# VinAIResearch/LFM

Hardware: AMD Instinct MI355X
Metric: images/sec (higher is better)
Workload: dtype f16; 1 GPU; DiT-L/2 celeb256 f8 (4x32x32 latents), batch 64/GPU, 50-step Euler (torchdiffeq grid) + f8 VAE decode to 256x256 + uint8 NHWC; 2 batches in flight on 2 HIP streams (same weights, own scratch); per_gpu_batch=64, global_batch=64, h2d_of_latents=inside the timed step, nfe=50, batches_in_flight=2

## Files before the change

### include/lfm_hip.h

```cpp
#ifndef LFM_HIP_H
#define LFM_HIP_H
#include <stddef.h>
#include <stdint.h>

#ifdef __cplusplus
extern "C" {
#endif

typedef void* lfm_stream_t;

#define LFM_OK 0
#define LFM_ERR_SHAPE (-1)
#define LFM_ERR_ALIGN (-2)
#define LFM_ERR_WORKSPACE (-3)
#define LFM_ERR_LAUNCH (-4)
#define LFM_ERR_ARG (-5)

const char* lfm_strerror(int code);
#define LFM_ABI_VERSION 4
int lfm_abi_version(void);

typedef struct lfm_dit_shape {
  int depth;
  int hidden;
  int heads;
  int patch;
  int in_ch;
  int res;
  int mlp_hidden;
  int label_rows;
} lfm_dit_shape;

typedef struct lfm_dit_weights {
  const float* pos_embed;
  const float* patch_w;
  const float* patch_b;
  const float* t_w0;
  const float* t_b0;
  const float* t_w2;
  const float* t_b2;
  const float* y_table;
  const void* ada_w;
  const float* ada_b;
  const void* qkv_w;
  const float* qkv_b;
  const void* proj_w;
  const float* proj_b;
  const void* fc1_w;
  const float* fc1_b;
  const void* fc2_w;
  const float* fc2_b;
  const float* final_w;
  const float* final_b;
  const void* patch_w16;
} lfm_dit_weights;

typedef struct lfm_dit_call {
  int batch;
  const float* x;
  const float* t;
  int t_len;
  const int64_t* y;
  int cfg;
  float cfg_scale;
  float* out;
  const float* axpy_base;
  const float* axpy_dt;
  const void* cond_table;
  const int* cond_step;
  int cond_offset;
  int cond_rows;
  int fold_ln;
  int gemm_select;
} lfm_dit_call;
#define LFM_CALL_OFF 1
#define LFM_CALL_ON 2
#define LFM_CALL_GEMM_SELECT(which) ((which) + 1)

size_t lfm_dit_workspace_bytes(const lfm_dit_shape* shape, int max_batch);

#define LFM_DIT_WS_BUFFERS 10
int lfm_dit_workspace_layout(const lfm_dit_shape* shape, int batch, size_t* offsets_out, int n);

int lfm_dit_forward(const lfm_dit_shape* shape, const lfm_dit_weights* w, void* workspace, size_t workspace_bytes,
                    const lfm_dit_call* call, lfm_stream_t stream);

#define LFM_PLAN_FOLDED_LN 1
#define LFM_PLAN_FUSED_QKV_ATTENTION 2
int lfm_dit_plan(const lfm_dit_shape* shape, const lfm_dit_call* call, int* plan_out);

size_t lfm_dit_cond_table_bytes(const lfm_dit_shape* shape, int n_times);
int lfm_dit_cond_table_build(const lfm_dit_shape* shape, const lfm_dit_weights* w, void* workspace, size_t workspace_bytes, int batch, const float* t_values,
                             int n_times, void* table, size_t table_bytes, lfm_stream_t stream);

int lfm_gemm_f16(const void* A, long lda, const void* W, long ldw, void* C, long ldc, int M, int N, int K, const float* bias,
                 int epilogue, const float* gate, long gate_stride, int tokens, lfm_stream_t stream);

int lfm_gemm_qkv_f16(const void* A, long lda, const void* W, long ldw, void* Q, void* K_out, void* Vt, int M, int D, int K,
                     const float* bias, int head_dim, int tokens, lfm_stream_t stream);

int lfm_gemm_select(int which);
int lfm_gemm_plan(int M, int N, int K, int batch, int caps);

int lfm_profile_fc1(int enable);
int lfm_profile_blocks_read(float* host_ms_out, int max_n);
#define LFM_OPT_FOLD_LN 1
#define LFM_OPT_GEMM_V6 2
#define LFM_OPT_SKINNY_GEMM 4
#define LFM_OPT_ATTENTION_STREAM 5
#define LFM_OPT_FUSED_QKV_ATTENTION 6
#define LFM_OPT_UNET_ATTENTION_STREAM 7
#define LFM_OPT_ATTENTION_TILED 8
int lfm_set_option(int key, int value);
int lfm_dit_call_settings(const lfm_dit_call* call, int* gemm_select_out, int* fold_ln_out);

int lfm_clock_probe(int blocks, int iters, unsigned long long* ticks_out, lfm_stream_t stream);

#ifdef LFM_MEASURE
int lfm_gemm_trace_read(unsigned long long* host_out, int n_per_group);
int lfm_attention_trace_read(unsigned long long* host_out, int n);
int lfm_attention_wg_trace_read(unsigned long long* host_out, int n_wg);
int lfm_dit_chk_arm(const void* workspace);
int lfm_dit_chk_read(unsigned long long* host_out, int n);
#endif
int lfm_profile_fc1_read(float* host_ms_out, int max_n);

int lfm_ln_modulate(const float* X, void* A, int M, int D, int tokens, const float* shift, const float* scale, long mod_stride,
                    lfm_stream_t stream);

int lfm_dit_attention(const void* Q, const void* K, const void* Vt, void* O, int batch, int heads, int T, lfm_stream_t stream);
int lfm_dit_attention_hd(const void* Q, const void* K, const void* Vt, void* O, int batch, int heads, int head_dim, int T,
                         lfm_stream_t stream);
int lfm_attention_plan(int batch, int heads, int head_dim, int T);

typedef struct lfm_vae_resnet {
  const float* n1_g; const float* n1_b; const void* c1_w; const float* c1_b;
  const float* n2_g; const float* n2_b; const void* c2_w; const float* c2_b;
  const void* sc_w; const float* sc_b;
  int cin, cout;
} lfm_vae_resnet;

typedef struct lfm_vae_weights {
  const float* pq_w; const float* pq_b;
  const float* cin_w; const float* cin_b;
  lfm_vae_resnet mid[2];
  const float* at_g; const float* at_b;
  const void* q_w; const float* q_b; const void* k_w; const float* k_b;
  const void* v_w; const float* v_b; const void* o_w; const float* o_b;
  lfm_vae_resnet up[4][3];
  const void* ups_w[3]; const float* ups_b[3];
  const float* no_g; const float* no_b;
  const void* cout_w; const float* cout_b;
} lfm_vae_weights;

size_t lfm_vae_workspace_bytes(int R, int chunk);

int lfm_vae_decode(const lfm_vae_weights* w, void* workspace, size_t workspace_bytes, const float* z, float* out, int N, int R,
                   int chunk, lfm_stream_t stream);

typedef struct lfm_vae_enc_weights {
  const float* cin_w; const float* cin_b;
  lfm_vae_resnet down[4][2];
  const void* ds_w[3]; const float* ds_b[3];
  lfm_vae_resnet mid[2];
  const float* at_g; const float* at_b;
  const void* q_w; const float* q_b; const void* k_w; const float* k_b;
  const void* v_w; const float* v_b; const void* o_w; const float* o_b;
  const float* no_g; const float* no_b;
  const void* cout_w; const float* cout_b;
} lfm_vae_enc_weights;

int lfm_vae_encode(const lfm_vae_enc_weights* w, void* workspace, size_t workspace_bytes, const float* x, float* moments, int N, int R,
                   int chunk, lfm_stream_t stream);

int lfm_vae_groupnorm_f16(const void* x, void* y, const float* gamma, const float* beta, void* workspace, size_t workspace_bytes, int n, int HW, int C,
                          int silu, lfm_stream_t stream);
int lfm_vae_groupnorm_plan(int n, int HW, int C, size_t workspace_bytes);
int lfm_vae_conv3x3_gn_f16(const void* in, const void* w, const float* bias, const void* resid, void* conv_out, void* y, const float* gamma,
                           const float* beta, void* workspace, size_t workspace_bytes, int n, int H, int W, int Cin, int Cout, int ups, int silu,
                           int* stat_slabs, int* stat_kernel, lfm_stream_t stream);
size_t lfm_vae_mid_attention_workspace_bytes(int n, int T);
int lfm_vae_mid_attention_f16(const void* x, void* out, const float* gn_gamma, const float* gn_beta, const void* q_w, const float* q_b,
                              const void* k_w, const float* k_b, const void* v_w, const float* v_b, const void* o_w, const float* o_b,
                              void* workspace, size_t workspace_bytes, int n, int T, lfm_stream_t stream);
int lfm_vae_conv_in_f16(const float* pq_w, const float* pq_b, const float* cin_w, const float* cin_b, const float* z, void* out, int n, int R,
                        lfm_stream_t stream);
size_t lfm_vae_downsample_workspace_bytes(int n, int Ho, int Wo, int C);
int lfm_vae_downsample_f16(const void* x, const void* w, const float* bias, void* out, void* workspace, size_t workspace_bytes, int n, int Ho, int Wo,
                           int C, lfm_stream_t stream);
size_t lfm_vae_resnets_workspace_bytes(int n, int H, int W);
int lfm_vae_resnets_f16(const lfm_vae_resnet* r, int n_res, const void* x, void* out, void* workspace, size_t workspace_bytes, int n, int H, int W,
                        int chain_stats, int* last_slabs, lfm_stream_t stream);
size_t lfm_vae_conv_moments_workspace_bytes(int n, int H, int W);
int lfm_vae_conv_moments_f32(const void* in, const void* w8, const float* b8, float* moments, void* workspace, size_t workspace_bytes, int n, int H,
                             int W, lfm_stream_t stream);

int lfm_images_to_uint8(const float* x, uint8_t* out, int N, int H, int W, lfm_stream_t stream);
int lfm_images_to_uint8_mode(const float* x, uint8_t* out, int N, int H, int W, int rounding, lfm_stream_t stream);

int lfm_conv3x3_f16(const void* in, const void* w, const float* bias, const void* resid, void* out, int N, int H, int W, int Cin, int Cout,
                    int mode, lfm_stream_t stream);
size_t lfm_conv3x3_workspace_bytes(int N, int H, int W, int Cin, int Cout);
int lfm_conv3x3_f16_ws(const void* in, const void* w, const float* bias, const void* resid, void* out, int N, int H, int W, int Cin, int Cout,
                       int mode, void* workspace, size_t workspace_bytes, lfm_stream_t stream);
int lfm_conv3x3_scaled_f16_ws(const void* in, const void* w, const float* bias, const void* resid, float scale, void* out, int N, int H, int W, int Cin,
                              int Cout, int mode, void* workspace, size_t workspace_bytes, lfm_stream_t stream);
int lfm_conv3x3_plan(int N, int H, int W, int Cin, int Cout, int mode, size_t workspace_bytes);
int lfm_conv3x3_in_f32(const float* x_nchw, const float* w, const float* bias, void* out_nhwc, int N, int H, int W, int Cin, int Cout,
                       lfm_stream_t stream);
int lfm_conv3x3_out_f32(const void* in, const void* w4, const float* bias4, float* out_nchw, int N, int H, int W, int Cin, int nch,
                        lfm_stream_t stream);
int lfm_linear_f16(const void* A, long lda, const void* W, long ldw, void* C, long ldc, int M, int N, int K, const float* bias,
                   const void* resid, lfm_stream_t stream);
int lfm_linear2_f16(const void* A1, int K1, const void* A2, int K2, const void* W, long ldw, void* C, long ldc, int M, int N, const float* bias,
                    const void* resid, lfm_stream_t stream);
int lfm_linear_scaled_f16(const void* A, long lda, const void* W, long ldw, void* C, long ldc, int M, int N, int K, const float* bias,
                          const void* resid, float scale, lfm_stream_t stream);
int lfm_linear2_scaled_f16(const void* A1, int K1, const void* A2, int K2, const void* W, long ldw, void* C, long ldc, int M, int N,
                           const float* bias, const void* resid, float scale, lfm_stream_t stream);
int lfm_linear_resid_vec_f16(const void* A, long lda, const void* W, long ldw, void* C, long ldc, int M, int N, int K, const float* bias,
                             const void* resid, const float* vec, long vec_stride, int tokens, float scale, lfm_stream_t stream);
int lfm_linear_silu_f16(const void* A, long lda, const void* W, long ldw, void* C, long ldc, int M, int N, int K, const float* bias, lfm_stream_t stream);
int lfm_gather_rows_f32(const float* table, int rows, int cols, const void* y_int64, int N, float* out, long out_stride, lfm_stream_t stream);
size_t lfm_groupnorm_scratch_bytes(int N, int C);
int lfm_groupnorm_f16(const void* x, void* y, const float* gamma, const float* beta, const float* film, long film_stride, void* scratch, int N,
                      int HW, int C, int groups, float eps, int silu, lfm_stream_t stream);
int lfm_groupnorm_plan(int N, int HW, int C, int groups);
int lfm_groupnorm2_f16(const void* xa, int Ca, const void* xb, int Cb, void* y, const float* gamma, const float* beta, const float* film,
                       long film_stride, void* scratch, int N, int HW, int groups, float eps, int silu, lfm_stream_t stream);
int lfm_avgpool2_f16(const void* x, void* y, int N, int Ho, int Wo, int C, lfm_stream_t stream);
int lfm_upsample2_f16(const void* x, void* y, int N, int Ho, int Wo, int C, lfm_stream_t stream);
int lfm_fir_down2_f16(const void* x, void* y, const float* bias, const void* resid, float scale, int N, int Ho, int Wo, int C, int pad,
                      lfm_stream_t stream);
int lfm_fir_up2_f16(const void* x, void* y, int N, int Ho, int Wo, int C, lfm_stream_t stream);
int lfm_zero_border_f16(const void* x, void* y, int N, int H, int W, int C, lfm_stream_t stream);
int lfm_zero_border_f32(const float* x, float* y, int planes, int H, int W, lfm_stream_t stream);
int lfm_concat_channels_f16(const void* a, const void* b, void* out, long pixels, int Ca, int Cb, lfm_stream_t stream);
int lfm_add_image_vec_f16(const void* x, const float* e, long e_stride, void* y, int N, int HW, int C, lfm_stream_t stream);
int lfm_attention_small_f16(const void* qkv, void* out, int N, int T, int heads, int ch, lfm_stream_t stream);
int lfm_unet_attention_plan(int N, int T, int heads, int ch);
int lfm_cross_attention_f16(const void* Q, long ldq, const void* K, const void* V, long ldkv, void* out, long ldo, int N, int Tq, int Tk, int heads,
                            int ch, lfm_stream_t stream);
int lfm_cross_attention_plan(int N, int Tq, int Tk, int heads, int ch);
int lfm_layernorm_f16(const void* x, void* y, const float* gamma, const float* beta, long M, int C, float eps, lfm_stream_t stream);
int lfm_geglu_f16(const void* h, long ldh, void* y, long M, int I, lfm_stream_t stream);
int lfm_token_embed_f16(const float* tok_emb, int vocab, const float* pos_emb, int pos_rows, const void* ids_int64, void* out, int N, int L, int D,
                        lfm_stream_t stream);
int lfm_linear_gelu_f16(const void* A, long lda, const void* W, long ldw, void* C, long ldc, int M, int N, int K, const float* bias, lfm_stream_t stream);
int lfm_label_rescale_f32(const void* labels_int64, const float* w, const float* bias, float* out, int N, int H, int W, int num_cls, int Cout, int n_stages,
                          lfm_stream_t stream);
int lfm_time_embed(const float* t, int t_len, const float* w0, const float* b0, const float* w2, const float* b2, const float* label_table,
                   const int64_t* y, int label_rows, float* scratch_h1, float* emb, void* emb_silu_f16, int N, int F, int E,
                   lfm_stream_t stream);
int lfm_song_embed(const float* t, int t_len, const float* w0, const float* b0, const float* w1, const float* b1, const float* label_table,
                   const float* label_bias, float label_scale, const int64_t* y, int label_rows, float* scratch_h1, float* emb, void* emb_f16, int N,
                   int F, int E, lfm_stream_t stream);
int lfm_fourier_embed(const float* t, int t_len, const float* freqs, const float* w0, const float* b0, const float* w1, const float* b1,
                      const float* label_table, const float* label_bias, float label_scale, const int64_t* y, int label_rows, float* scratch_h1,
                      float* emb, void* emb_f16, int N, int F, int E, lfm_stream_t stream);

int lfm_grid_advance(const float* ts, const float* dts, int* step, float* t_cur, float* t_next, float* dt_cur, lfm_stream_t stream);

int lfm_lincomb(float* out, const float* base, const float* const* k_host_ptrs, const float* coef, const float* scale, int nk, long n,
                lfm_stream_t stream);

int lfm_rk_error_norm(const float* y0, const float* y1, const float* const* k_host_ptrs, const float* e_coef, const float* dt, int nk, long n,
                      float rtol, float atol, float* scratch, float* out, lfm_stream_t stream);

#ifdef __cplusplus
}
#endif
#endif
```

### lfm_amd/csrc/dit.hip

```cpp
#include <mutex>

#include "../../include/lfm_hip.h"
#include "gemm_dispatch.h"
#include "gemm_skinny_kernel.h"
#include "gemm_sq64_kernel.h"
#include "qkv_attention_kernel.h"

typedef std::atomic<int> Opt;
static inline int opt_get(const Opt& o) { return o.load(std::memory_order_relaxed); }
static inline void opt_set(Opt& o, int v) { o.store(v, std::memory_order_relaxed); }
static struct {
  Opt gemm_sel{0}, gemm_dbg{0};
  Opt fold_ln{1};
  Opt v6{0};
  Opt skinny{1};
  Opt stagger{0};
  Opt att_stream{1};
  Opt fused_qkv{1};
  Opt att_tiled{1};
  Opt unet_att_stream{1};
} g_def;
static thread_local int tl_sel_set = 0, tl_gemm_sel = 0, tl_gemm_dbg = 0;
static thread_local int tl_fold = 0;
static inline int gemm_sel() { return tl_sel_set ? tl_gemm_sel : opt_get(g_def.gemm_sel); }
static inline int gemm_dbg() { return tl_sel_set ? tl_gemm_dbg : opt_get(g_def.gemm_dbg); }
static inline int opt_fold_ln() { return tl_fold ? (tl_fold == LFM_CALL_ON ? 1 : 0) : opt_get(g_def.fold_ln); }
int lfm_gemm_selected() { return gemm_sel(); }
int lfm_gemm_debug_flags() { return gemm_dbg(); }
int lfm_gemm_selected_v1_ok() { return gemm_sel() < 2 && !(gemm_dbg() & LFM_DBG_GEMM_NO_SPLITK); }
int lfm_gemm_prefers_v4(int M, int N, int K) {
  (void)M;
  (void)N;
  (void)K;
  if (gemm_dbg() & LFM_DBG_GEMM_NEVER_V4) return 0;
  if (gemm_dbg() & LFM_DBG_GEMM_ALWAYS_V4) return 1;
  return 0;
}
int lfm_gemm_v6_default() { return opt_get(g_def.v6); }
int lfm_stagger_ticks() { return opt_get(g_def.stagger); }
int lfm_attention_stream_enabled() { return opt_get(g_def.att_stream); }
int lfm_attention_tiled_mode() { return opt_get(g_def.att_tiled); }
int lfm_unet_attention_stream_mode() { return opt_get(g_def.unet_att_stream); }
extern "C" int lfm_gemm_plan(int M, int N, int K, int batch, int caps) { return gemm_choose(M, N, K, batch, caps); }
static inline bool gemm_select_valid(int which) {
  const int k = which & 15;
  return which >= 0 && (k == 0 || k == 1 || k == 4 || k == 5 || k == 6 || k == 7 || k == 8);
}
struct CallScope {
  int sel_set, sel, dbg, fold;
  CallScope() : sel_set(tl_sel_set), sel(tl_gemm_sel), dbg(tl_gemm_dbg), fold(tl_fold) {}
  ~CallScope() {
    tl_sel_set = sel_set;
    tl_gemm_sel = sel;
    tl_gemm_dbg = dbg;
    tl_fold = fold;
  }
};

static int call_scope_enter(const lfm_dit_call* c) {
  if (c->fold_ln < 0 || c->fold_ln > LFM_CALL_ON || c->gemm_select < 0 || (c->gemm_select && !gemm_select_valid(c->gemm_select - 1)) || c->cond_rows < 0)
    return LFM_ERR_ARG;
  if (c->fold_ln) tl_fold = c->fold_ln;
  if (c->gemm_select) {
    tl_sel_set = 1;
    tl_gemm_sel = (c->gemm_select - 1) & 15;
    tl_gemm_dbg = (c->gemm_select - 1) >> 4;
  }
  return LFM_OK;
}
extern "C" int lfm_dit_call_settings(const lfm_dit_call* call, int* gemm_select_out, int* fold_ln_out) {
  if (!call || !gemm_select_out || !fold_ln_out) return LFM_ERR_ARG;
  CallScope scope;
  const int rc = call_scope_enter(call);
  if (rc) return rc;
  *gemm_select_out = gemm_sel() | (gemm_dbg() << 4);
  *fold_ln_out = opt_fold_ln();
  return LFM_OK;
}

extern "C" int lfm_set_option(int key, int value) {
  switch (key) {
    case 1: opt_set(g_def.fold_ln, value != 0); break;
    case 2: opt_set(g_def.v6, value != 0); break;
#ifdef LFM_MEASURE
    case 3: opt_set(g_def.stagger, value > 0 ? value : 0); break;
#endif
    case 4: opt_set(g_def.skinny, value < 0 || value > 2 ? 1 : value); break;
    case 5: opt_set(g_def.att_stream, value != 0); break;
    case 6: opt_set(g_def.fused_qkv, value != 0); break;
    case 7: opt_set(g_def.unet_att_stream, value < 0 || value > 2 ? 1 : value); break;
    case 8:
      if (value < 0 || value > 2) return LFM_ERR_ARG;
      opt_set(g_def.att_tiled, value);
      break;
    default: return LFM_ERR_ARG;
  }
  return LFM_OK;
}
extern "C" int lfm_gemm_select(int which) {
  if (!gemm_select_valid(which)) return LFM_ERR_ARG;
  opt_set(g_def.gemm_sel, which & 15);
  opt_set(g_def.gemm_dbg, which >> 4);
  return LFM_OK;
}

#include "dit_kernels.h"
#include "attention_dispatch.h"
#include "solver_kernels.h"
#include "dit_measure.h"

static inline size_t align_up(size_t v, size_t a) { return (v + a - 1) / a * a; }

struct DitWs {
  float* X;
  half_t* A;
  half_t* A2;
  half_t* QKVH;
  float* temb;
  float* temb_h;
  half_t* c_half;
  float* mod;
  float* ones;
  float* ln_part;
  float* cen[2];
  half_t* amod;
  float* uvq;
  float* uvf;
  float* slab;
  size_t slab_bytes;
  size_t total;
};

struct DitDims {
  int B, T, M, D, H;
  long J, uvq_n, uvf_n;
  int KK, tiles_p, hd;
};
static inline bool dit_fold_capable(const lfm_dit_shape* s) { return (s->hidden % 256) == 0 && (s->mlp_hidden % 64) == 0; }
static DitDims dit_dims(const lfm_dit_shape* s, int B) {
  const int grid = s->res / s->patch, T = grid * grid, D = s->hidden, H = s->mlp_hidden;
  const long uv = dit_fold_capable(s) ? (long)s->depth * 2 : 0;
  return DitDims{B, T, B * T, D, H, (long)s->depth * 6 * D + 2 * D, uv * 3 * D, uv * H, s->in_ch * s->patch * s->patch, D / 256, D / s->heads};
}

static DitWs carve(const lfm_dit_shape* s, const DitDims& d, void* ws, bool sizing = false) {
  const size_t B = d.B, T = d.T, M = d.M, D = d.D, H = d.H, J = d.J;
  size_t off = 0;
  char* base = (char*)ws;
  DitWs w;
  auto take = [&](size_t bytes) {
    char* p = (char*)((uintptr_t)base + off);
    off += align_up(bytes, 256);
    return p;
  };
  w.X = (float*)take(M * D * 4);
  w.A = (half_t*)take(M * D * 2);
  const size_t qkvh = (3 * M * D > M * H ? 3 * M * D : M * H) * 2;
  w.QKVH = (half_t*)take(qkvh);
  w.temb = (float*)take(B * D * 4);
  w.temb_h = (float*)take(B * D * 4);
  w.c_half = (half_t*)take(B * D * 2);
  w.mod = (float*)take(B * J * 4);
  w.ones = (float*)take(D * 4);
  w.ln_part = (float*)take(M * ((D + 255) / 256) * 8);
  w.cen[0] = (float*)take(M * 4);
  w.cen[1] = (float*)take(M * 4);
  const bool fold_ops = dit_fold_capable(s);
  w.amod = (half_t*)take(fold_ops ? (size_t)s->depth * 4 * B * D * 2 : 0);
  w.uvq = (float*)take(fold_ops ? (size_t)s->depth * 2 * B * 3 * D * 4 : 0);
  w.uvf = (float*)take(fold_ops ? (size_t)s->depth * 2 * B * H * 4 : 0);
  w.A2 = (half_t*)take(fold_ops ? M * D * 2 : 0);
  const size_t Ms = sizing ? (M < 1024 ? M : (size_t)1024 / T * T) : M;
  w.slab_bytes = (sizing || M <= 1024) && Ms > 0 ? 4 * Ms * (H > 3 * D ? H : 3 * D) * 4 : 0;
  w.slab = w.slab_bytes ? (float*)take(w.slab_bytes) : nullptr;
  if (!base) w.slab = nullptr;
  w.total = off;
  return w;
}

static int check_shape(const lfm_dit_shape* s) {
  if (!s) return LFM_ERR_ARG;
  if (s->depth <= 0 || s->hidden <= 0 || s->heads <= 0 || s->patch <= 0 || s->in_ch <= 0 || s->res <= 0) return LFM_ERR_SHAPE;
  if (s->hidden % s->heads) return LFM_ERR_SHAPE;
  if (s->res % s->patch) return LFM_ERR_SHAPE;
  const int T = (s->res / s->patch) * (s->res / s->patch);
  if (attention_choose(1, s->heads, s->hidden / s->heads, T) < 0) return LFM_ERR_SHAPE;
  if (s->hidden % 64 || s->hidden > 256 * LN_MAXV || s->mlp_hidden % 64) return LFM_ERR_SHAPE;
  const int kk = s->patch * s->patch * s->in_ch;
  if (kk > FIN_MAXO || (kk > PE_MAXK && (kk % 64))) return LFM_ERR_SHAPE;
  if (s->label_rows <= 0) return LFM_ERR_SHAPE;
  return LFM_OK;
}

extern "C" const char* lfm_strerror(int code) {
  switch (code) {
    case LFM_OK: return "ok";
    case LFM_ERR_SHAPE: return "unsupported or inconsistent shape";
    case LFM_ERR_ALIGN: return "pointer / leading dimension alignment";
    case LFM_ERR_WORKSPACE: return "workspace too small";
    case LFM_ERR_LAUNCH: return "kernel launch failed";
    case LFM_ERR_ARG: return "bad argument";
  }
  return "unknown";
}
extern "C" int lfm_abi_version(void) { return LFM_ABI_VERSION; }

extern "C" size_t lfm_dit_workspace_bytes(const lfm_dit_shape* shape, int max_batch) {
  if (check_shape(shape) != LFM_OK || max_batch <= 0) return 0;
  return carve(shape, dit_dims(shape, max_batch), nullptr, true).total;
}

extern "C" int lfm_dit_workspace_layout(const lfm_dit_shape* shape, int batch, size_t* offsets_out, int n) {
  const int rc = check_shape(shape);
  if (rc) return rc;
  if (!offsets_out || n < 0) return LFM_ERR_ARG;
  if (batch <= 0) return LFM_ERR_SHAPE;
  const DitWs w = carve(shape, dit_dims(shape, batch), nullptr);
  const bool fold_ops = dit_fold_capable(shape);
  const void* bufs[LFM_DIT_WS_BUFFERS] = {w.X, w.A, fold_ops ? w.A2 : nullptr, w.QKVH, w.mod, w.ln_part, w.cen[0], w.cen[1], fold_ops ? w.uvq : nullptr,
                                          fold_ops ? w.uvf : nullptr};
  for (int i = 0; i < n && i < LFM_DIT_WS_BUFFERS; ++i) offsets_out[i] = (size_t)(uintptr_t)bufs[i];
  return LFM_DIT_WS_BUFFERS;
}

extern "C" int lfm_dit_attention_hd(const void* Q, const void* K, const void* Vt, void* O, int batch, int heads, int head_dim, int T,
                                    lfm_stream_t stream) {
  if (!Q || !K || !Vt || !O) return LFM_ERR_ARG;
  if (batch <= 0 || heads <= 0) return LFM_ERR_SHAPE;
  if (((uintptr_t)Q | (uintptr_t)K | (uintptr_t)Vt | (uintptr_t)O) & 15) return LFM_ERR_ALIGN;
  return attention_launch((const half_t*)Q, (const half_t*)K, (const half_t*)Vt, (half_t*)O, batch, heads, head_dim, T, (hipStream_t)stream);
}
extern "C" int lfm_attention_plan(int batch, int heads, int head_dim, int T) {
  if (batch <= 0 || heads <= 0) return LFM_ERR_SHAPE;
  return attention_choose(batch, heads, head_dim, T);
}
extern "C" int lfm_dit_attention(const void* Q, const void* K, const void* Vt, void* O, int batch, int heads, int T, lfm_stream_t stream) {
  return lfm_dit_attention_hd(Q, K, Vt, O, batch, heads, 64, T, stream);
}

static int ln_modulate_launch(const float* X, half_t* A, int M, int D, int tokens, const float* shift, const float* scale, long stride,
                              hipStream_t st) {
  if (D % 4 || D > 256 * LN_MAXV) return LFM_ERR_SHAPE;
  if (D % 8 == 0 && !(((uintptr_t)A | (uintptr_t)X) & 15) && !(gemm_dbg() & LFM_DBG_LN_STORE8)) {
    const int f = gemm_dbg();
    if (f & LFM_DBG_LN_BPERMUTE) hipLaunchKernelGGL(ln_modulate8_kernel<1>, dim3(cdiv(M, 4)), dim3(256), 0, st, X, A, M, D, tokens, shift, scale, stride);
    else if (f & LFM_DBG_LN_TWO_ROWS) hipLaunchKernelGGL(ln_modulate8_kernel<2>, dim3(cdiv(M, 8)), dim3(256), 0, st, X, A, M, D, tokens, shift, scale, stride);
    else if (f & LFM_DBG_LN_FOUR_ROWS) hipLaunchKernelGGL(ln_modulate8_kernel<4>, dim3(cdiv(M, 16)), dim3(256), 0, st, X, A, M, D, tokens, shift, scale, stride);
    else hipLaunchKernelGGL((ln_modulate8_kernel<1, true>), dim3(cdiv(M, 4)), dim3(256), 0, st, X, A, M, D, tokens, shift, scale, stride);
    LFM_CHECK_LAUNCH();
    return LFM_OK;
  }
  hipLaunchKernelGGL(ln_modulate_kernel, dim3(cdiv(M, 4 * LN_ROWS)), dim3(256), 0, st, X, A, M, D, tokens, shift, scale, stride);
  LFM_CHECK_LAUNCH();
  return LFM_OK;
}

extern "C" int lfm_ln_modulate(const float* X, void* A, int M, int D, int tokens, const float* shift, const float* scale, long mod_stride,
                               lfm_stream_t stream) {
  if (!X || !A || !shift || !scale) return LFM_ERR_ARG;
  if (M <= 0 || tokens <= 0) return LFM_ERR_SHAPE;
  return ln_modulate_launch(X, (half_t*)A, M, D, tokens, shift, scale, mod_stride, (hipStream_t)stream);
}

extern "C" int lfm_gemm_f16(const void* A, long lda, const void* W, long ldw, void* C, long ldc, int M, int N, int K, const float* bias,
                            int epilogue, const float* gate, long gate_stride, int tokens, lfm_stream_t stream) {
  if (!A || !W || !C) return LFM_ERR_ARG;
  if ((lda % 8) || (ldw % 8) || (ldc % 4) || (((uintptr_t)A | (uintptr_t)W) & 15)) return LFM_ERR_ALIGN;
  hipStream_t st = (hipStream_t)stream;
  ASrcRowMajor a{(const half_t*)A, lda, M, 0};
  if (gemm_sel() == 7 || gemm_sel() == 8) {
    const int which = gemm_sel();
    auto lat = [&](const auto& e) {
      return which == 7 ? launch_gemm_sq64((const half_t*)A, lda, (const half_t*)W, ldw, M, N, K, e, 1, st)
                        : launch_gemm_skinny((const half_t*)A, lda, (const half_t*)W, ldw, M, N, K, e, 1, st);
    };
    switch (epilogue) {
      case 0: return lat(EpiBiasF16{(half_t*)C, ldc, bias});
      case 1: return bias ? lat(EpiBiasGeluF16{(half_t*)C, ldc, bias}) : LFM_ERR_ARG;
      case 2: return lat(EpiBiasF32{(float*)C, ldc, bias});
      default: return LFM_ERR_ARG;
    }
  }
  switch (epilogue) {
    case 0: return gemm_f16_launch(a, (const half_t*)W, ldw, M, N, K, EpiBiasF16{(half_t*)C, ldc, bias}, st);
    case 1: return bias ? gemm_f16_launch(a, (const half_t*)W, ldw, M, N, K, EpiBiasGeluF16{(half_t*)C, ldc, bias}, st) : LFM_ERR_ARG;
    case 2: return launch_gemm_auto(a, (const half_t*)W, ldw, M, N, K, EpiBiasF32{(float*)C, ldc, bias}, st);
    case 3:
      if (!bias || !gate || tokens <= 0) return LFM_ERR_ARG;
      return gemm_f16_launch(a, (const half_t*)W, ldw, M, N, K, EpiGateResidF32{(float*)C, ldc, bias, gate, gate_stride, tokens}, st);
  }
  return LFM_ERR_ARG;
}

extern "C" int lfm_gemm_qkv_f16(const void* A, long lda, const void* W, long ldw, void* Q, void* Kout, void* Vt, int M, int D, int K,
                                const float* bias, int head_dim, int tokens, lfm_stream_t stream) {
  if (!A || !W || !Q || !Kout || !Vt || !bias) return LFM_ERR_ARG;
  if ((lda % 8) || (ldw % 8) || (((uintptr_t)A | (uintptr_t)W) & 15)) return LFM_ERR_ALIGN;
  if (head_dim <= 0 || tokens <= 0 || (D % head_dim) || (head_dim % 8) || (tokens % 16) || (M % tokens)) return LFM_ERR_SHAPE;
  return gemm_f16_launch(ASrcRowMajor{(const half_t*)A, lda, M, 0}, (const half_t*)W, ldw, M, 3 * D, K,
                         EpiQKV::make((half_t*)Q, (half_t*)Kout, (half_t*)Vt, bias, D, head_dim, tokens), (hipStream_t)stream);
}

static int dit_conditioning(const lfm_dit_shape* s, const lfm_dit_weights* w, const DitWs& ws, const DitDims& d, const float* t, int t_len, const int64_t* y,
                            int rows, bool want_uv, hipStream_t st) {
  const int D = d.D, H = d.H;
  const long J = d.J, mstride = rows == 1 ? 0 : J;
  hipLaunchKernelGGL(temb1_kernel, dim3(cdiv(D, 4), t_len), dim3(256), 0, st, t, w->t_w0, w->t_b0, ws.temb_h, D);
  LFM_CHECK_LAUNCH();
  hipLaunchKernelGGL(temb2_kernel, dim3(cdiv(D, 4), t_len), dim3(256), 0, st, ws.temb_h, w->t_w2, w->t_b2, ws.temb, D);
  LFM_CHECK_LAUNCH();
  hipLaunchKernelGGL(cond_kernel, dim3(cdiv((long)rows * D, 256)), dim3(256), 0, st, ws.temb, t_len, w->y_table, y, s->label_rows, ws.c_half, D, rows);
  LFM_CHECK_LAUNCH();
  int rc = launch_gemm_tn(ASrcRowMajor{ws.c_half, D, rows, 0}, (const half_t*)w->ada_w, D, rows, (int)J, D, EpiBiasF32{ws.mod, J, w->ada_b}, st);
  if (rc || !want_uv) return rc;
  if (rows == 1 && D <= 8 * 64 * LN_MAXP) {
    hipLaunchKernelGGL(uv_gemv_kernel, dim3(cdiv(3 * D, 4 * UV_ROWS), s->depth), dim3(256), 0, st, (const half_t*)w->qkv_w, w->qkv_b, ws.mod, 3 * D, D, D, 0,
                       ws.uvq);
    LFM_CHECK_LAUNCH();
    hipLaunchKernelGGL(uv_gemv_kernel, dim3(cdiv(H, 4 * UV_ROWS), s->depth), dim3(256), 0, st, (const half_t*)w->fc1_w, w->fc1_b, ws.mod, H, D, 4 * D, 3 * D,
                       ws.uvf);
    LFM_CHECK_LAUNCH();
    return LFM_OK;
  }
  const long nmod = (long)s->depth * 4 * rows * (D / 4);
  hipLaunchKernelGGL(mod_rows_f16_kernel, dim3(cdiv(nmod, 256)), dim3(256), 0, st, ws.mod, mstride, s->depth, rows, D, ws.amod);
  LFM_CHECK_LAUNCH();
  rc = launch_gemm_auto(ASrcRowMajor{ws.amod, D, 2 * rows, 0}, (const half_t*)w->qkv_w, D, 2 * rows, 3 * D, D, EpiUV{ws.uvq, 3L * D, w->qkv_b, rows, 3L * D}, st,
                        s->depth, 4L * rows * D, 3L * D * D, 2L * rows * 3 * D);
  if (rc) return rc;
  return launch_gemm_auto(ASrcRowMajor{ws.amod + 2L * rows * D, D, 2 * rows, 0}, (const half_t*)w->fc1_w, D, 2 * rows, H, D,
                          EpiUV{ws.uvf, (long)H, w->fc1_b, rows, (long)H}, st, s->depth, 4L * rows * D, (long)H * D, 2L * rows * H);
}

static inline long cond_row_floats(const DitDims& d) { return d.J + d.uvq_n + d.uvf_n; }
static int dit_cond_copy(const DitWs& ws, const DitDims& d, const float* table, const int* step, int offset, int fixed_row, int to_table, hipStream_t st,
                         int rows = 0) {
  hipLaunchKernelGGL(cond_row_copy_kernel, dim3(cdiv(cond_row_floats(d) / 4, 256)), dim3(256), 0, st, table, cond_row_floats(d), step, offset, fixed_row, ws.mod,
                     d.J, ws.uvq, d.uvq_n, ws.uvf, d.uvf_n, to_table, rows);
  LFM_CHECK_LAUNCH();
  return LFM_OK;
}

extern "C" size_t lfm_dit_cond_table_bytes(const lfm_dit_shape* shape, int n_times) {
  if (check_shape(shape) != LFM_OK || n_times <= 0) return 0;
  return (size_t)cond_row_floats(dit_dims(shape, 1)) * 4 * (size_t)n_times;
}

extern "C" int lfm_dit_cond_table_build(const lfm_dit_shape* s, const lfm_dit_weights* w, void* workspace, size_t workspace_bytes, int batch,
                                        const float* t_values, int n_times, void* table, size_t table_bytes, lfm_stream_t stream) {
  int rc = check_shape(s);
  if (rc) return rc;
  if (!w || !workspace || !t_values || !table || n_times <= 0 || batch <= 0) return LFM_ERR_ARG;
  if (table_bytes < lfm_dit_cond_table_bytes(s, n_times)) return LFM_ERR_WORKSPACE;
  const DitDims d = dit_dims(s, batch);
  const DitWs ws = carve(s, d, workspace);
  if (ws.total > workspace_bytes) return LFM_ERR_WORKSPACE;
  if (((uintptr_t)workspace & 255) || ((uintptr_t)table & 15)) return LFM_ERR_ALIGN;
  hipStream_t st = (hipStream_t)stream;
  for (int i = 0; i < n_times; ++i) {
    rc = dit_conditioning(s, w, ws, d, t_values + i, 1, nullptr, 1, dit_fold_capable(s), st);
    if (rc) return rc;
    rc = dit_cond_copy(ws, d, (const float*)table, nullptr, 0, i, 1, st, n_times);
    if (rc) return rc;
  }
  return LFM_OK;
}

enum DitLoop { DIT_LOOP_FOLDED, DIT_LOOP_LATENCY, DIT_LOOP_SEPARATE };
struct DitPlan {
  DitLoop loop;
  bool fold, w6, fused;
  bool pe_mfma, fin_mfma;
  bool sq64;
  int s_proj, s_fc2;
};
static DitPlan dit_plan(const lfm_dit_shape* s, const DitDims& d, int rows, const DitWs* ws = nullptr, const lfm_dit_weights* w = nullptr) {
  const int sel = gemm_sel(), dbg = gemm_dbg(), skinny = opt_get(g_def.skinny);
  const int D = d.D, H = d.H, T = d.T, M = d.M;
  DitPlan p{};
  p.fold = opt_fold_ln() && dit_fold_capable(s) && (M % 256 == 0) && (rows == 1 || T % 256 == 0) && (long)(M / 256) * d.tiles_p >= 192 && (sel == 0 || sel == 6) &&
           s->depth >= 1;
  p.w6 = sel == 6 || (sel == 0 && opt_get(g_def.v6));
  p.fused = p.fold && opt_get(g_def.fused_qkv) && !p.w6 && T == 256 && D == s->heads * 64 && (long)M * D < (1L << 31) && (long)3 * D * D < (1L << 31);
  p.pe_mfma = s->patch == 2 && s->in_ch == 4 && (D % 256 == 0) && D <= 1280 && (s->res % 2 == 0) && !(dbg & LFM_DBG_DIT_PATCH_ROUND1);
  p.fin_mfma = (d.KK == 16 || d.KK == 64) && (D % 32 == 0) && (T % 16 == 0) && (M % 16 == 0) && !(dbg & LFM_DBG_DIT_FINAL_ROUND1);
  p.loop = p.fold ? DIT_LOOP_FOLDED : DIT_LOOP_SEPARATE;
  if (p.fold || !ws) return p;
  auto slices = [&](bool sq, int N_, int K_) {
    const int wgs = sq ? (N_ / SQ_T) * (M / SQ_T) : N_ / SK_BN, bk = sq ? SQ_BK : SK_BK;
    int sl = 1;
    while (wgs * (sl * 2) <= 256 && (K_ % (sl * 2 * bk)) == 0 && K_ / (sl * 2) >= 2 * bk && (size_t)(sl * 2) * M * N_ * 4 <= ws->slab_bytes) sl *= 2;
    return sl;
  };
  p.sq64 = skinny == 1 && M >= SQ_T && (M % SQ_T) == 0 && gemm_sq64_ok(ws->A, D, w->qkv_w, D, M, 3 * D, D, 1) && gemm_sq64_ok(ws->A, D, w->fc1_w, D, M, H, D, 1) &&
           gemm_sq64_ok(ws->A, D, w->proj_w, D, M, D, D, slices(true, D, D)) && gemm_sq64_ok(ws->QKVH, H, w->fc2_w, H, M, D, H, slices(true, D, H));
  p.s_proj = slices(p.sq64, D, D);
  p.s_fc2 = slices(p.sq64, D, H);
  if (skinny && sel == 0 && M <= SK_ROWS && ws->slab && D <= 1024 * SPLITK_LN_MAXJ && (D % 4) == 0 && gemm_skinny_ok(ws->A, D, w->qkv_w, D, M, 3 * D, D, 1) &&
      gemm_skinny_ok(ws->A, D, w->fc1_w, D, M, H, D, 1) && gemm_skinny_ok(ws->A, D, w->proj_w, D, M, D, D, p.s_proj) &&
      gemm_skinny_ok(ws->QKVH, H, w->fc2_w, H, M, D, H, p.s_fc2))
    p.loop = DIT_LOOP_LATENCY;
  return p;
}
extern "C" int lfm_dit_plan(const lfm_dit_shape* s, const lfm_dit_call* c, int* plan_out) {
  int rc = check_shape(s);
  if (rc) return rc;
  if (!c || !plan_out) return LFM_ERR_ARG;
  const int B = c->batch;
  if (B <= 0 || (c->t_len != 1 && c->t_len != B)) return LFM_ERR_SHAPE;
  CallScope scope;
  if ((rc = call_scope_enter(c)) != LFM_OK) return rc;
  const DitPlan p = dit_plan(s, dit_dims(s, B), (c->t_len == 1 && !c->y) ? 1 : B);
  *plan_out = (p.fold ? LFM_PLAN_FOLDED_LN : 0) | (p.fused ? LFM_PLAN_FUSED_QKV_ATTENTION : 0);
  return LFM_OK;
}

struct BlockW {
  const half_t *qkv_w, *proj_w, *fc1_w, *fc2_w;
  const float *qkv_b, *proj_b, *fc1_b, *fc2_b;
  const float *shift_msa, *scale_msa, *gate_msa, *shift_mlp, *scale_mlp, *gate_mlp, *next_shift_msa, *next_scale_msa;
};
static BlockW block_weights(const lfm_dit_weights* w, const float* mod_rows, const DitDims& d, int i) {
  const size_t D = d.D, H = d.H, b = i;
  const float* mod = mod_rows + b * 6 * D;
  return BlockW{(const half_t*)w->qkv_w + b * 3 * D * D, (const half_t*)w->proj_w + b * D * D, (const half_t*)w->fc1_w + b * H * D, (const half_t*)w->fc2_w + b * D * H,
                w->qkv_b + b * 3 * D, w->proj_b + b * D, w->fc1_b + b * H, w->fc2_b + b * D,
                mod, mod + D, mod + 2 * D, mod + 3 * D, mod + 4 * D, mod + 5 * D, mod + 6 * D, mod + 7 * D};
}

struct DitCtx : DitDims {
  const lfm_dit_shape* s;
  const lfm_dit_weights* w;
  const lfm_dit_call* c;
  const void* workspace;
  DitWs ws;
  DitPlan p;
  int rows;
  long mstride;
  hipStream_t st;
  half_t *Qb, *Kb, *Vb;
  bool prof_ok, chk;
  BlockW block(int i) const { return block_weights(w, ws.mod, *this, i); }
  void checksum(const void* buf, size_t bytes, int i, int slot) const { if (chk) dit_chk(buf, bytes, i, slot, st); }
  int embed() const, blocks_folded() const, blocks_latency() const, blocks_separate() const, final_layer() const;
};

int DitCtx::embed() const {
  const int xmod = c->cfg ? B / 2 : B;
  if (p.pe_mfma) {
    const int tpb = M <= 1024 ? 1 : 2;
    hipLaunchKernelGGL(patch_embed_ln_kernel, dim3(cdiv(M, 16 * tpb)), dim3(64 * (D / 256)), 0, st, c->x, w->patch_w, w->patch_b, w->pos_embed, ws.X,
                       M, xmod, s->res, D, tpb, p.fold ? ws.A : (half_t*)nullptr, ws.mod + D, mstride, ws.ln_part, tiles_p, ws.cen[0]);
    LFM_CHECK_LAUNCH();
  } else if (KK <= PE_MAXK) {
    hipLaunchKernelGGL(patch_embed_kernel, dim3(cdiv(M, PE_TOK)), dim3(D / 4), 0, st, c->x, w->patch_w, w->patch_b, w->pos_embed, ws.X, M,
                       xmod, s->in_ch, s->res, s->patch, D);
    LFM_CHECK_LAUNCH();
  } else {
    if (!w->patch_w16) return LFM_ERR_ARG;
    hipLaunchKernelGGL(patchify_kernel, dim3(M), dim3(256), 0, st, c->x, w->pos_embed, ws.A, ws.X, ws.ones, M, xmod, s->in_ch, s->res,
                       s->patch, D);
    LFM_CHECK_LAUNCH();
    const int rc = launch_gemm_auto(ASrcRowMajor{ws.A, KK, M, 0}, (const half_t*)w->patch_w16, KK, M, D, KK,
                                    EpiGateResidF32{ws.X, D, w->patch_b, ws.ones, 0, T}, st);
    if (rc) return rc;
  }
  if (p.fold && !p.pe_mfma) {
    hipLaunchKernelGGL(ln_center_mod_kernel, dim3(cdiv(M, 4)), dim3(256), 0, st, ws.X, ws.A, M, D, T, ws.mod + D, mstride, ws.ln_part, tiles_p,
                       ws.cen[0]);
    LFM_CHECK_LAUNCH();
  }
  return LFM_OK;
}

int DitCtx::blocks_folded() const {
  const long uvs_q = rows == 1 ? 0 : 3 * D, uvs_f = rows == 1 ? 0 : H;
  int rc, cen_cur = 0;
  auto rowstat_src = [&]() {
    RowStatSrc r{ws.ln_part, ws.cen[cen_cur], ws.cen[cen_cur ^ 1], tiles_p, 1.0f / (float)D, 1e-6f};
    cen_cur ^= 1;
    return r;
  };
  auto launch_fold = [&](const ASrcRowMajor& a, const half_t* Wp, long ldw_, int M_, int N_, int K_, const auto& e) {
    return p.w6 ? launch_gemm256w_tn(a, Wp, ldw_, M_, N_, K_, e, st) : launch_gemm256h_tn(a, Wp, ldw_, M_, N_, K_, e, st);
  };
  half_t *Ob = p.fused ? ws.A2 : ws.A, *A1b = p.fused ? ws.A : ws.A2;
  for (int i = 0; i < s->depth; ++i) {
    const BlockW b = block(i);
    const float *uq = ws.uvq + (long)i * 2 * rows * 3 * D, *uf = ws.uvf + (long)i * 2 * rows * H;
    if (p.fused) {
      const QkvAttnArgs e_qa{uq, uq + (long)rows * 3 * D, uvs_q, rowstat_src(), Ob, D, s->heads, 0.125f * 1.4426950408889634f, nullptr, 0};
      if ((rc = launch_qkv_attention(ws.A, D, b.qkv_w, D, M, D, s->heads, D, e_qa, st))) return rc;
    } else {
      const EpiQKVMod e_qkv{{}, Qb, Kb, Vb, uq, uq + (long)rows * 3 * D, uvs_q, D, hd, T, EpiQKV::log2_or_neg(T), rowstat_src(), nullptr, 0};
      if ((rc = launch_fold(ASrcRowMajor{ws.A, D, M, 0}, b.qkv_w, D, M, 3 * D, D, e_qkv))) return rc;
      checksum(ws.QKVH, (size_t)3 * M * D * 2, i, 0);
      if ((rc = attention_launch(Qb, Kb, Vb, Ob, B, s->heads, hd, T, st))) return rc;
    }
    checksum(Ob, (size_t)M * D * 2, i, 1);
    const EpiGateResidMod e_proj{ws.X, D, b.proj_b, b.gate_msa, mstride, T, A1b, b.scale_mlp, mstride, ws.cen[cen_cur], ws.ln_part, tiles_p};
    if ((rc = launch_fold(ASrcRowMajor{Ob, D, M, 0}, b.proj_w, D, M, D, D, e_proj))) return rc;
    checksum(ws.X, (size_t)M * D * 4, i, 2);
    checksum(A1b, (size_t)M * D * 2, i, 3);
    checksum(ws.ln_part, (size_t)M * tiles_p * 8, i, 4);
    const bool prof = prof_fc1_begin(prof_ok, st);
#if defined(LFM_MEASURE) && defined(LFM_EXP_DUMP)
    const EpiModGeluF16 e_fc1{ws.QKVH, H, uf, uf + (long)rows * H, uvs_f, T, rowstat_src(), nullptr, 0,
                              (g_dbg && workspace == g_dbg_ws) ? g_dbg + (long)i * g_dbg_stride : (float*)nullptr};
#else
    const EpiModGeluF16 e_fc1{ws.QKVH, H, uf, uf + (long)rows * H, uvs_f, T, rowstat_src(), nullptr, 0};
#endif
    if ((rc = launch_fold(ASrcRowMajor{A1b, D, M, 0}, b.fc1_w, D, M, H, D, e_fc1))) return rc;
    prof_fc1_end(prof, st);
    checksum(ws.QKVH, (size_t)M * H * 2, i, 5);
    const ASrcRowMajor a_fc2{ws.QKVH, H, M, 0};
    const EpiGateResidF32 e_fc2{ws.X, D, b.fc2_b, b.gate_mlp, mstride, T};
    const EpiGateResidMod e_fc2_mod{e_fc2.X, D, e_fc2.bias, e_fc2.gate, mstride, T, ws.A, b.next_scale_msa, mstride, ws.cen[cen_cur], ws.ln_part, tiles_p};
    if ((rc = i + 1 < s->depth ? launch_fold(a_fc2, b.fc2_w, H, M, D, H, e_fc2_mod) : launch_fold(a_fc2, b.fc2_w, H, M, D, H, e_fc2))) return rc;
    checksum(ws.X, (size_t)M * D * 4, i, 6);
    checksum(ws.A, (size_t)M * D * 2, i, 7);
  }
  return LFM_OK;
}

int DitCtx::blocks_latency() const {
  auto lat_gemm = [&](const half_t* A_, const half_t* W_, int N_, int K_, const auto& epi_, int S_) {
    return p.sq64 ? launch_gemm_sq64(A_, (long)K_, W_, (long)K_, M, N_, K_, epi_, S_, st) : launch_gemm_skinny(A_, (long)K_, W_, (long)K_, M, N_, K_, epi_, S_, st);
  };
  auto finish = [&](int S_, const EpiGateResidF32& e, half_t* A_out, const float* shift, const float* scale) {
    hipLaunchKernelGGL(splitk_finish_resid_ln_kernel, dim3(M), dim3(256), 0, st, ws.slab, S_, (long)M * D, D, e.X, e.ldx, e.bias, e.gate, e.gate_stride, e.tokens, A_out,
                       shift, scale, mstride);
    LFM_CHECK_LAUNCH();
    return LFM_OK;
  };
  const EpiSlabF32 e_slab{ws.slab, (long)D, (long)M * D};
  int rc = ln_modulate_launch(ws.X, ws.A, M, D, T, block(0).shift_msa, block(0).scale_msa, mstride, st);
  if (rc) return rc;
  for (int i = 0; i < s->depth; ++i) {
    const BlockW b = block(i);
    if ((rc = lat_gemm(ws.A, b.qkv_w, 3 * D, D, EpiQKV::make(Qb, Kb, Vb, b.qkv_b, D, hd, T), 1))) return rc;
    if ((rc = attention_launch(Qb, Kb, Vb, ws.A, B, s->heads, hd, T, st))) return rc;
    if ((rc = lat_gemm(ws.A, b.proj_w, D, D, e_slab, p.s_proj))) return rc;
    if ((rc = finish(p.s_proj, EpiGateResidF32{ws.X, D, b.proj_b, b.gate_msa, mstride, T}, ws.A, b.shift_mlp, b.scale_mlp))) return rc;
    const bool prof = prof_fc1_begin(prof_ok, st);
    if ((rc = lat_gemm(ws.A, b.fc1_w, H, D, EpiBiasGeluF16{ws.QKVH, H, b.fc1_b}, 1))) return rc;
    prof_fc1_end(prof, st);
    if ((rc = lat_gemm(ws.QKVH, b.fc2_w, D, H, e_slab, p.s_fc2))) return rc;
    if ((rc = finish(p.s_fc2, EpiGateResidF32{ws.X, D, b.fc2_b, b.gate_mlp, mstride, T}, i + 1 < s->depth ? ws.A : nullptr, b.next_shift_msa, b.next_scale_msa))) return rc;
  }
  return LFM_OK;
}

int DitCtx::blocks_separate() const {
  auto linear = [&](const half_t* W_, int N_, const auto& epi_) {
    const int rc = launch_gemm_splitk(ws.A, D, W_, D, M, N_, D, epi_, ws.slab, ws.slab_bytes, st);
    return rc == 1 ? launch_gemm_auto(ASrcRowMajor{ws.A, D, M, 0}, W_, D, M, N_, D, epi_, st) : rc;
  };
  int rc;
  bool a_ready = false;
  for (int i = 0; i < s->depth; ++i) {
    const BlockW b = block(i);
    if (!a_ready && (rc = ln_modulate_launch(ws.X, ws.A, M, D, T, b.shift_msa, b.scale_msa, mstride, st))) return rc;
    a_ready = false;
    if ((rc = linear(b.qkv_w, 3 * D, EpiQKV::make(Qb, Kb, Vb, b.qkv_b, D, hd, T)))) return rc;
    if ((rc = attention_launch(Qb, Kb, Vb, ws.A, B, s->heads, hd, T, st))) return rc;
    const EpiGateResidF32 e_proj{ws.X, D, b.proj_b, b.gate_msa, mstride, T};
    rc = launch_gemm_splitk_resid_ln(ws.A, D, b.proj_w, D, M, D, D, e_proj, ws.A, b.shift_mlp, b.scale_mlp, mstride, ws.slab, ws.slab_bytes, st);
    if (rc == 1) {
      if ((rc = launch_gemm_auto(ASrcRowMajor{ws.A, D, M, 0}, b.proj_w, D, M, D, D, e_proj, st))) return rc;
      rc = ln_modulate_launch(ws.X, ws.A, M, D, T, b.shift_mlp, b.scale_mlp, mstride, st);
    }
    if (rc) return rc;
    const bool prof = prof_fc1_begin(prof_ok, st);
    if ((rc = linear(b.fc1_w, H, EpiBiasGeluF16{ws.QKVH, H, b.fc1_b}))) return rc;
    prof_fc1_end(prof, st);
    const EpiGateResidF32 e_fc2{ws.X, D, b.fc2_b, b.gate_mlp, mstride, T};
    const bool more = i + 1 < s->depth;
    rc = launch_gemm_splitk_resid_ln(ws.QKVH, H, b.fc2_w, H, M, D, H, e_fc2, more ? ws.A : (half_t*)nullptr, b.next_shift_msa, b.next_scale_msa, mstride, ws.slab,
                                     ws.slab_bytes, st);
    if (rc == LFM_OK) a_ready = more;
    if (rc == 1) rc = launch_gemm_auto(ASrcRowMajor{ws.QKVH, H, M, 0}, b.fc2_w, H, M, D, H, e_fc2, st);
    if (rc) return rc;
  }
  return LFM_OK;
}

int DitCtx::final_layer() const {
  const bool cfg = c->cfg != 0;
  const float* fmod = ws.mod + (long)s->depth * 6 * D;
  const int Mh = cfg ? M / 2 : M;
  auto kernel = p.fin_mfma ? (cfg ? (KK == 16 ? final_layer_mfma_kernel<true, 1> : final_layer_mfma_kernel<true, 4>)
                                  : (KK == 16 ? final_layer_mfma_kernel<false, 1> : final_layer_mfma_kernel<false, 4>))
                           : (cfg ? final_layer_kernel<true> : final_layer_kernel<false>);
  const long blocks = p.fin_mfma ? (cfg ? Mh / 8 : M / 16) : cdiv(Mh, cfg ? 8 : 16);
  hipLaunchKernelGGL(kernel, dim3((unsigned)blocks), dim3(256), 0, st, ws.X, M, D, T, fmod, fmod + D, mstride, w->final_w, w->final_b, s->in_ch, s->res, s->patch,
                     cfg ? c->cfg_scale : 1.0f, c->out, c->axpy_base, c->axpy_dt);
  LFM_CHECK_LAUNCH();
  return LFM_OK;
}

extern "C" int lfm_dit_forward(const lfm_dit_shape* s, const lfm_dit_weights* w, void* workspace, size_t workspace_bytes,
                               const lfm_dit_call* c, lfm_stream_t stream) {
  int rc = check_shape(s);
  if (rc) return rc;
  if (!w || !workspace || !c || !c->x || !c->t || !c->out) return LFM_ERR_ARG;
  const int B = c->batch;
  if (B <= 0 || (c->t_len != 1 && c->t_len != B)) return LFM_ERR_SHAPE;
  if (c->cfg && (B & 1)) return LFM_ERR_SHAPE;
  if (c->axpy_base && !c->axpy_dt) return LFM_ERR_ARG;
  const DitDims d = dit_dims(s, B);
  const DitWs ws = carve(s, d, workspace);
  if (ws.total > workspace_bytes) return LFM_ERR_WORKSPACE;
  if ((uintptr_t)workspace & 255) return LFM_ERR_ALIGN;
  hipStream_t st = (hipStream_t)stream;
  CallScope scope;
  if ((rc = call_scope_enter(c)) != LFM_OK) return rc;
  const bool prof_ok = prof_claim(st);
  const int rows = (c->t_len == 1 && !c->y) ? 1 : B;
  const bool tab = c->cond_table != nullptr;
  if (tab && (rows != 1 || !c->cond_step)) return LFM_ERR_ARG;
  DitCtx x{d, s, w, c, workspace, ws, dit_plan(s, d, rows, &ws, w), rows,  rows == 1 ? 0 : d.J, st,
            ws.QKVH, ws.QKVH + (size_t)d.M * d.D, ws.QKVH + (size_t)2 * d.M * d.D, prof_ok,  false};

  if (tab) rc = dit_cond_copy(ws, d, (const float*)c->cond_table, c->cond_step, c->cond_offset, 0, 0, st, c->cond_rows);
  else rc = dit_conditioning(s, w, ws, d, c->t, c->t_len, c->y, rows, x.p.fold, st);
  if (rc) return rc;
  if ((rc = x.embed()) != LFM_OK) return rc;
#ifdef LFM_MEASURE
  x.chk = g_chk && workspace == g_chk_ws;
  if (x.chk) (void)hipMemsetAsync(g_chk, 0, DIT_CHK_SLOTS * 8, st);
#endif
  const bool prof_blk = prof_ok && g_prof_blk_count < LFM_PROF_BLK_MAX;
  if (prof_blk) (void)hipEventRecord(g_prof_blk_ev[2 * g_prof_blk_count], st);
  switch (x.p.loop) {
    case DIT_LOOP_FOLDED: rc = x.blocks_folded(); break;
    case DIT_LOOP_LATENCY: rc = x.blocks_latency(); break;
    case DIT_LOOP_SEPARATE: rc = x.blocks_separate(); break;
  }
  if (rc) return rc;
  if (prof_blk) (void)hipEventRecord(g_prof_blk_ev[2 * g_prof_blk_count++ + 1], st);
  return x.final_layer();
}
```

### lfm_amd/csrc/dit_kernels.h

```cpp
#pragma once

__global__ __launch_bounds__(256) void temb1_kernel(const float* __restrict__ t, const float* __restrict__ w0, const float* __restrict__ b0,
                                                    float* __restrict__ h1, int D) {
  const int r = blockIdx.y, lane = threadIdx.x & 63;
  const int j = blockIdx.x * 4 + (threadIdx.x >> 6);
  if (j >= D) return;
  const float tv = t[r];
  const float* w = w0 + (long)j * 256;
  float s = 0.f;
#pragma unroll
  for (int k = lane; k < 256; k += 64) {
    const int i = k & 127;
    const float a = tv * expf(-9.210340371976184f * (float)i / 128.0f);
    s += w[k] * (k < 128 ? cosf(a) : sinf(a));
  }
  s = wave_sum(s);
  if (lane == 0) h1[(long)r * D + j] = silu_f(s + b0[j]);
}
__global__ __launch_bounds__(256) void temb2_kernel(const float* __restrict__ h1, const float* __restrict__ w2, const float* __restrict__ b2,
                                                    float* __restrict__ temb, int D) {
  const int r = blockIdx.y, lane = threadIdx.x & 63;
  const int j = blockIdx.x * 4 + (threadIdx.x >> 6);
  if (j >= D) return;
  const float* w = w2 + (long)j * D;
  const float* h = h1 + (long)r * D;
  float s = 0.f;
  for (int k = lane; k < D; k += 64) s += w[k] * h[k];
  s = wave_sum(s);
  if (lane == 0) temb[(long)r * D + j] = s + b2[j];
}

__global__ void cond_kernel(const float* __restrict__ temb, int t_len, const float* __restrict__ y_table, const int64_t* __restrict__ y,
                            int label_rows, half_t* __restrict__ c_half, int D, int rows) {
  const long i = (long)blockIdx.x * blockDim.x + threadIdx.x;
  if (i >= (long)rows * D) return;
  const int r = (int)(i / D), j = (int)(i - (long)r * D);
  const long yr = y ? (long)y[r] : (long)(label_rows - 1);
  if (yr < 0 || yr >= label_rows) {
    c_half[i] = (half_t)__builtin_nanf("");
    return;
  }
  const float v = temb[(t_len == 1 ? 0 : (long)r * D) + j] + y_table[yr * D + j];
  c_half[i] = (half_t)silu_f(v);
}

#define PE_TOK 16
#define PE_MAXK 16
__global__ __launch_bounds__(320) void patch_embed_kernel(const float* __restrict__ x, const float* __restrict__ w, const float* __restrict__ b,
                                                          const float* __restrict__ pos, float* __restrict__ X, int M, int xmod, int C, int R,
                                                          int p, int D) {
  __shared__ float xs[PE_TOK][PE_MAXK];
  const int grid = R / p, T = grid * grid, KK = C * p * p;
  const long m_begin = (long)blockIdx.x * PE_TOK;
  for (int e = threadIdx.x; e < PE_TOK * PE_MAXK; e += blockDim.x) {
    const int tt = e / PE_MAXK, k = e % PE_MAXK;
    const long m = m_begin + tt;
    float v = 0.f;
    if (m < M && k < KK) {
      const int tok = (int)(m % T), n = (int)(m / T) % xmod;
      const int c = k / (p * p), pp = (k / p) % p, q = k % p;
      v = x[(((long)n * C + c) * R + (tok / grid) * p + pp) * R + (tok % grid) * p + q];
    }
    xs[tt][k] = v;
  }
  const int j = threadIdx.x * 4;
  float wr[4][PE_MAXK];
#pragma unroll
  for (int i = 0; i < 4; ++i)
#pragma unroll
    for (int k = 0; k < PE_MAXK; ++k) wr[i][k] = (k < KK) ? w[(long)(j + i) * KK + k] : 0.f;
  const f32x4 bias = *(const f32x4*)(b + j);
  f32x4 pv[PE_TOK];
#pragma unroll
  for (int tt = 0; tt < PE_TOK; ++tt) {
    const long m = (m_begin + tt < M) ? m_begin + tt : M - 1;
    pv[tt] = *(const f32x4*)(pos + (long)(m % T) * D + j);
  }
  __syncthreads();
#pragma unroll
  for (int tt = 0; tt < PE_TOK; ++tt) {
    const long m = m_begin + tt;
    if (m >= M) break;
    f32x4 acc = bias + pv[tt];
#pragma unroll
    for (int k = 0; k < PE_MAXK; ++k) {
      const float xv = xs[tt][k];
      acc.x += wr[0][k] * xv;
      acc.y += wr[1][k] * xv;
      acc.z += wr[2][k] * xv;
      acc.w += wr[3][k] * xv;
    }
    *(f32x4*)(X + m * D + j) = acc;
  }
}

__global__ __launch_bounds__(320) void patch_embed_ln_kernel(const float* __restrict__ x, const float* __restrict__ w, const float* __restrict__ b,
                                                             const float* __restrict__ pos, float* __restrict__ X, int M, int xmod, int R, int D,
                                                             int tiles_per_block, half_t* __restrict__ A, const float* __restrict__ scale,
                                                             long mod_stride, float* __restrict__ part, int tiles_p, float* __restrict__ cen) {
  typedef half_t half4v __attribute__((ext_vector_type(4)));
  __shared__ float red[2][5][16];
  const int lane = threadIdx.x & 63, wv = threadIdx.x >> 6, a = lane & 15, q = lane >> 4;
  const int grid = R >> 1, T = grid * grid;
  half4v wh[8][2], wl[8][2];
  f32x4 bias[8][2];
#pragma unroll
  for (int pr = 0; pr < 8; ++pr)
#pragma unroll
    for (int e = 0; e < 2; ++e) {
      const int n = 256 * wv + 32 * pr + 8 * (a >> 2) + 4 * e + (a & 3);
      const f32x4 wf = *(const f32x4*)(w + (long)n * 16 + 4 * q);
      const float wa[4] = {wf.x, wf.y, wf.z, wf.w};
#pragma unroll
      for (int i = 0; i < 4; ++i) {
        wh[pr][e][i] = (half_t)wa[i];
        wl[pr][e][i] = (half_t)(wa[i] - (float)wh[pr][e][i]);
      }
      bias[pr][e] = *(const f32x4*)(b + 256 * wv + 32 * pr + 8 * q + 4 * e);
    }
  for (int it = 0; it < tiles_per_block; ++it) {
    const long tile = (long)blockIdx.x * tiles_per_block + it;
    if (tile * 16 >= M) break;
    const long m = tile * 16 + a < M ? tile * 16 + a : M - 1;
    const int tok = (int)(m % T), n_img = (int)(m / T) % xmod;
    const float* xp = x + (((long)n_img * 4 + q) * R + (tok / grid) * 2) * R + (tok % grid) * 2;
    const f32x2 r0 = *(const f32x2*)xp, r1 = *(const f32x2*)(xp + R);
    const float xa[4] = {r0.x, r0.y, r1.x, r1.y};
    half4v xh, xl;
#pragma unroll
    for (int i = 0; i < 4; ++i) {
      xh[i] = (half_t)xa[i];
      xl[i] = (half_t)(xa[i] - (float)xh[i]);
    }
    f32x4 val[8][2];
    float sx = 0.f;
    const float* prow = pos + (long)tok * D + 256 * wv + 8 * q;
    float* xrow = X + m * D + 256 * wv + 8 * q;
    const bool live = tile * 16 + a < M;
#pragma unroll
    for (int pr = 0; pr < 8; ++pr)
#pragma unroll
      for (int e = 0; e < 2; ++e) {
        f32x4_t acc = {0.f, 0.f, 0.f, 0.f};
        acc = __builtin_amdgcn_mfma_f32_16x16x16f16(wh[pr][e], xh, acc, 0, 0, 0);
        acc = __builtin_amdgcn_mfma_f32_16x16x16f16(wl[pr][e], xh, acc, 0, 0, 0);
        acc = __builtin_amdgcn_mfma_f32_16x16x16f16(wh[pr][e], xl, acc, 0, 0, 0);
        const f32x4 v = (f32x4){acc[0], acc[1], acc[2], acc[3]} + bias[pr][e] + *(const f32x4*)(prow + 32 * pr + 4 * e);
        val[pr][e] = v;
        if (live) *(f32x4*)(xrow + 32 * pr + 4 * e) = v;
        sx += (v.x + v.y) + (v.z + v.w);
      }
    if (!A) continue;
    sx += __shfl_xor(sx, 16, 64);
    sx += __shfl_xor(sx, 32, 64);
    if (q == 0) red[0][wv][a] = sx;
    __syncthreads();
    float sum = 0.f;
    for (int i = 0; i < (int)(blockDim.x >> 6); ++i) sum += red[0][i][a];
    const float mean = sum / (float)D;
    const float* srow = scale + (m / T) * mod_stride + 256 * wv + 8 * q;
    half_t* arow = A + m * D + 256 * wv + 8 * q;
    float sq = 0.f;
#pragma unroll
    for (int pr = 0; pr < 8; ++pr) {
      const f32x4 d0 = val[pr][0] - mean, d1 = val[pr][1] - mean;
      sq += (d0.x * d0.x + d0.y * d0.y) + (d0.z * d0.z + d0.w * d0.w) + (d1.x * d1.x + d1.y * d1.y) + (d1.z * d1.z + d1.w * d1.w);
      const f32x4 o0 = d0 * (1.0f + *(const f32x4*)(srow + 32 * pr)), o1 = d1 * (1.0f + *(const f32x4*)(srow + 32 * pr + 4));
      const half8_t h = {(half_t)o0.x, (half_t)o0.y, (half_t)o0.z, (half_t)o0.w, (half_t)o1.x, (half_t)o1.y, (half_t)o1.z, (half_t)o1.w};
      if (live) *(half8_t*)(arow + 32 * pr) = h;
    }
    sq += __shfl_xor(sq, 16, 64);
    sq += __shfl_xor(sq, 32, 64);
    if (q == 0) red[1][wv][a] = sq;
    __syncthreads();
    if (wv == 0 && q == 0 && live) {
      float qs = 0.f;
      for (int i = 0; i < (int)(blockDim.x >> 6); ++i) qs += red[1][i][a];
      float* pp = part + m * tiles_p * 2;
      pp[0] = sum;
      pp[1] = qs;
      for (int t2 = 1; t2 < tiles_p; ++t2) {
        pp[2 * t2] = 0.f;
        pp[2 * t2 + 1] = 0.f;
      }
      cen[m] = mean;
    }
  }
}

__global__ __launch_bounds__(256) void patchify_kernel(const float* __restrict__ x, const float* __restrict__ pos, half_t* __restrict__ Ap,
                                                       float* __restrict__ X, float* __restrict__ ones, int M, int xmod, int C, int R, int p, int D) {
  const int grid = R / p, T = grid * grid, KK = C * p * p;
  const long m = blockIdx.x;
  const int tok = (int)(m % T), n = (int)(m / T) % xmod;
  for (int k = threadIdx.x; k < KK; k += 256) {
    const int c = k / (p * p), pp = (k / p) % p, q = k % p;
    Ap[m * KK + k] = (half_t)x[(((long)n * C + c) * R + (tok / grid) * p + pp) * R + (tok % grid) * p + q];
  }
  for (int j = threadIdx.x; j < D; j += 256) X[m * D + j] = pos[(long)tok * D + j];
  if (m == 0)
    for (int j = threadIdx.x; j < D; j += 256) ones[j] = 1.0f;
}

#define LN_MAXV 5
#define LN_ROWS 2
__global__ __launch_bounds__(256) void ln_modulate_kernel(const float* __restrict__ X, half_t* __restrict__ A, int M, int D, int tokens,
                                                          const float* __restrict__ shift, const float* __restrict__ scale, long mod_stride) {
  const int lane = threadIdx.x & 63;
  const long m0 = ((long)blockIdx.x * 4 + (threadIdx.x >> 6)) * LN_ROWS;
  if (m0 >= M) return;
  const int nv = D >> 2;
  f32x4 v[LN_ROWS][LN_MAXV];
  float s[LN_ROWS];
#pragma unroll
  for (int r = 0; r < LN_ROWS; ++r) {
    const long m = (m0 + r < M) ? m0 + r : M - 1;
    const f32x4* xr = (const f32x4*)(X + m * D);
    s[r] = 0.f;
#pragma unroll
    for (int i = 0; i < LN_MAXV; ++i) {
      const int c = lane + 64 * i;
      if (c < nv) {
        v[r][i] = xr[c];
        s[r] += v[r][i].x + v[r][i].y + v[r][i].z + v[r][i].w;
      }
    }
  }
#pragma unroll
  for (int r = 0; r < LN_ROWS; ++r) {
    const long m = m0 + r;
    if (m >= M) break;
    const float mean = wave_sum(s[r]) / (float)D;
    float q = 0.f;
#pragma unroll
    for (int i = 0; i < LN_MAXV; ++i) {
      const int c = lane + 64 * i;
      if (c < nv) {
        v[r][i] -= mean;
        q += v[r][i].x * v[r][i].x + v[r][i].y * v[r][i].y + v[r][i].z * v[r][i].z + v[r][i].w * v[r][i].w;
      }
    }
    const float rstd = rsqrtf(wave_sum(q) / (float)D + 1e-6f);
    const long mo = (m / tokens) * mod_stride;
    const f32x4* sh = (const f32x4*)(shift + mo);
    const f32x4* sc = (const f32x4*)(scale + mo);
    half4_t* ar = (half4_t*)(A + m * D);
#pragma unroll
    for (int i = 0; i < LN_MAXV; ++i) {
      const int c = lane + 64 * i;
      if (c < nv) {
        const f32x4 o = v[r][i] * rstd * (1.0f + sc[c]) + sh[c];
        half4_t h = {(half_t)o.x, (half_t)o.y, (half_t)o.z, (half_t)o.w};
        ar[c] = h;
      }
    }
  }
}

#define LN_MAXP 3
template <int NR, bool DPP = false>
__global__ __launch_bounds__(256) void ln_modulate8_kernel(const float* __restrict__ X, half_t* __restrict__ A, int M, int D, int tokens,
                                                           const float* __restrict__ shift, const float* __restrict__ scale, long mod_stride) {
  const int lane = threadIdx.x & 63;
  const long m0 = ((long)blockIdx.x * 4 + (threadIdx.x >> 6)) * NR;
  if (m0 >= M) return;
  const int np = D >> 3;
  f32x4 v[NR][LN_MAXP][2];
  float s[NR];
#pragma unroll
  for (int r = 0; r < NR; ++r) {
    const long m = (m0 + r < M) ? m0 + r : M - 1;
    const f32x4* xr = (const f32x4*)(X + m * D);
    s[r] = 0.f;
#pragma unroll
    for (int i = 0; i < LN_MAXP; ++i) {
      const int c = lane + 64 * i;
      if (c < np) {
        v[r][i][0] = xr[2 * c];
        v[r][i][1] = xr[2 * c + 1];
        const f32x4 t = v[r][i][0] + v[r][i][1];
        s[r] += (t.x + t.y) + (t.z + t.w);
      }
    }
  }
#pragma unroll
  for (int r = 0; r < NR; ++r) {
    const long m = m0 + r;
    if (m >= M) break;
    const float mean = (DPP ? wave_sum_dpp(s[r]) : wave_sum(s[r])) / (float)D;
    float q = 0.f;
#pragma unroll
    for (int i = 0; i < LN_MAXP; ++i) {
      if (lane + 64 * i < np) {
#pragma unroll
        for (int h = 0; h < 2; ++h) {
          v[r][i][h] -= mean;
          const f32x4 t = v[r][i][h] * v[r][i][h];
          q += (t.x + t.y) + (t.z + t.w);
        }
      }
    }
    const float rstd = rsqrtf((DPP ? wave_sum_dpp(q) : wave_sum(q)) / (float)D + 1e-6f);
    const long mo = (m / tokens) * mod_stride;
    const f32x4* sh = (const f32x4*)(shift + mo);
    const f32x4* sc = (const f32x4*)(scale + mo);
    half8_t* ar = (half8_t*)(A + m * D);
#pragma unroll
    for (int i = 0; i < LN_MAXP; ++i) {
      const int c = lane + 64 * i;
      if (c < np) {
        const f32x4 lo = v[r][i][0] * rstd * (1.0f + sc[2 * c]) + sh[2 * c];
        const f32x4 hi = v[r][i][1] * rstd * (1.0f + sc[2 * c + 1]) + sh[2 * c + 1];
        half8_t h = {(half_t)lo.x, (half_t)lo.y, (half_t)lo.z, (half_t)lo.w, (half_t)hi.x, (half_t)hi.y, (half_t)hi.z, (half_t)hi.w};
        ar[c] = h;
      }
    }
  }
}

__global__ __launch_bounds__(256) void ln_center_mod_kernel(const float* __restrict__ X, half_t* __restrict__ A, int M, int D, int tokens,
                                                            const float* __restrict__ scale, long mod_stride, float* __restrict__ part, int tiles_p,
                                                            float* __restrict__ cen) {
  const int lane = threadIdx.x & 63;
  const long m = (long)blockIdx.x * 4 + (threadIdx.x >> 6);
  if (m >= M) return;
  const int np = D >> 3;
  f32x4 v[LN_MAXP][2];
  const f32x4* xr = (const f32x4*)(X + m * D);
  float s = 0.f;
#pragma unroll
  for (int i = 0; i < LN_MAXP; ++i) {
    const int c = lane + 64 * i;
    if (c < np) {
      v[i][0] = xr[2 * c];
      v[i][1] = xr[2 * c + 1];
      const f32x4 t = v[i][0] + v[i][1];
      s += (t.x + t.y) + (t.z + t.w);
    }
  }
  const float sum = wave_sum_dpp(s), mean = sum / (float)D;
  float q = 0.f;
#pragma unroll
  for (int i = 0; i < LN_MAXP; ++i) {
    if (lane + 64 * i < np) {
#pragma unroll
      for (int h = 0; h < 2; ++h) {
        v[i][h] -= mean;
        const f32x4 t = v[i][h] * v[i][h];
        q += (t.x + t.y) + (t.z + t.w);
      }
    }
  }
  const float qs = wave_sum_dpp(q);
  const f32x4* sc = (const f32x4*)(scale + (m / tokens) * mod_stride);
  half8_t* ar = (half8_t*)(A + m * D);
#pragma unroll
  for (int i = 0; i < LN_MAXP; ++i) {
    const int c = lane + 64 * i;
    if (c < np) {
      const f32x4 lo = v[i][0] * (1.0f + sc[2 * c]), hi = v[i][1] * (1.0f + sc[2 * c + 1]);
      half8_t h = {(half_t)lo.x, (half_t)lo.y, (half_t)lo.z, (half_t)lo.w, (half_t)hi.x, (half_t)hi.y, (half_t)hi.z, (half_t)hi.w};
      ar[c] = h;
    }
  }
  if (lane < tiles_p) *(f32x2*)(part + (m * tiles_p + lane) * 2) = lane == 0 ? (f32x2){sum, qs} : (f32x2){0.f, 0.f};
  if (lane == 0) cen[m] = mean;
}

__global__ __launch_bounds__(256) void mod_rows_f16_kernel(const float* __restrict__ mod, long mod_stride, int depth, int R, int D,
                                                           half_t* __restrict__ Amod) {
  const long idx = (long)blockIdx.x * 256 + threadIdx.x;
  const int d4 = D >> 2;
  const long total = (long)depth * 4 * R * d4;
  if (idx >= total) return;
  const int k = (int)(idx % d4) * 4;
  long t = idx / d4;
  const int r = (int)(t % R);
  t /= R;
  const int h = (int)(t & 1), b = (int)((t >> 1) & 1), i = (int)(t >> 2);
  const float* src = mod + (long)r * mod_stride + (long)i * 6 * D + (b ? 3 * D : 0) + (h ? 0 : D) + k;
  f32x4 v = *(const f32x4*)src;
  if (!h) v += 1.0f;
  half4_t o = {(half_t)v.x, (half_t)v.y, (half_t)v.z, (half_t)v.w};
  *(half4_t*)(Amod + idx * 4) = o;
}

#define UV_ROWS 8
__global__ __launch_bounds__(256) void uv_gemv_kernel(const half_t* __restrict__ W, const float* __restrict__ bias, const float* __restrict__ mod,
                                                      int N, int D, int scale_off, int shift_off, float* __restrict__ out) {
  const int lane = threadIdx.x & 63, i = blockIdx.y;
  const int n0 = (blockIdx.x * 4 + (threadIdx.x >> 6)) * UV_ROWS;
  if (n0 >= N) return;
  const int nch = D >> 3;
  const float* sc = mod + (long)i * 6 * D + scale_off;
  const float* sh = mod + (long)i * 6 * D + shift_off;
  f32x4 au[LN_MAXP][2], av[LN_MAXP][2];
#pragma unroll
  for (int j = 0; j < LN_MAXP; ++j) {
    const int c = lane + 64 * j;
    if (c < nch) {
      au[j][0] = *(const f32x4*)(sc + 8 * c) + 1.0f;
      au[j][1] = *(const f32x4*)(sc + 8 * c + 4) + 1.0f;
      av[j][0] = *(const f32x4*)(sh + 8 * c);
      av[j][1] = *(const f32x4*)(sh + 8 * c + 4);
    }
  }
  const half_t* wb = W + ((long)i * N + n0) * D;
  half8_t wv[UV_ROWS][LN_MAXP];
#pragma unroll
  for (int r = 0; r < UV_ROWS; ++r)
#pragma unroll
    for (int j = 0; j < LN_MAXP; ++j) {
      const int c = lane + 64 * j;
      if (c < nch && n0 + r < N) wv[r][j] = *(const half8_t*)(wb + (long)r * D + 8 * c);
    }
  float* ob = out + (long)i * 2 * N;
#pragma unroll
  for (int r = 0; r < UV_ROWS; ++r) {
    float u = 0.f, v = 0.f;
#pragma unroll
    for (int j = 0; j < LN_MAXP; ++j) {
      if (lane + 64 * j < nch && n0 + r < N) {
        const half8_t h = wv[r][j];
        const f32x4 w0 = {(float)h[0], (float)h[1], (float)h[2], (float)h[3]}, w1 = {(float)h[4], (float)h[5], (float)h[6], (float)h[7]};
        const f32x4 pu = au[j][0] * w0 + au[j][1] * w1, pv = av[j][0] * w0 + av[j][1] * w1;
        u += (pu.x + pu.y) + (pu.z + pu.w);
        v += (pv.x + pv.y) + (pv.z + pv.w);
      }
    }
    u = wave_sum_dpp(u);
    v = wave_sum_dpp(v);
    if (lane == 0 && n0 + r < N) {
      ob[n0 + r] = u;
      ob[N + n0 + r] = v + bias[(long)i * N + n0 + r];
    }
  }
}

#define FIN_MAXO 256
template <bool CFG>
__global__ __launch_bounds__(256) void final_layer_kernel(const float* __restrict__ X, int M, int D, int tokens, const float* __restrict__ shift,
                                                          const float* __restrict__ scale, long mod_stride, const float* __restrict__ Wf,
                                                          const float* __restrict__ bf, int C, int R, int p, float cfg_scale,
                                                          float* out, const float* base, const float* __restrict__ dt_ptr) {
  const int lane = threadIdx.x & 63;
  const long wg = (long)blockIdx.x * 4 + (threadIdx.x >> 6);
  const int Mh = CFG ? M / 2 : M;
  const long mfirst = CFG ? wg * 2 : wg * 4;
  if (mfirst >= Mh) return;
  const int nv = D >> 2, NO = p * p * C;
  long mrow[4];
#pragma unroll
  for (int r = 0; r < 4; ++r) {
    long m = CFG ? mfirst + (r & 1) + (long)(r >> 1) * Mh : mfirst + r;
    mrow[r] = m < M ? m : M - 1;
  }
  f32x4 v[4][LN_MAXV];
#pragma unroll
  for (int r = 0; r < 4; ++r) {
    const f32x4* xr = (const f32x4*)(X + mrow[r] * D);
#pragma unroll
    for (int i = 0; i < LN_MAXV; ++i) {
      const int c = lane + 64 * i;
      if (c < nv) v[r][i] = xr[c];
    }
  }
#pragma unroll
  for (int r = 0; r < 4; ++r) {
    float s = 0.f;
#pragma unroll
    for (int i = 0; i < LN_MAXV; ++i)
      if (lane + 64 * i < nv) s += v[r][i].x + v[r][i].y + v[r][i].z + v[r][i].w;
    const float mean = wave_sum(s) / (float)D;
    float q = 0.f;
#pragma unroll
    for (int i = 0; i < LN_MAXV; ++i)
      if (lane + 64 * i < nv) {
        v[r][i] -= mean;
        q += v[r][i].x * v[r][i].x + v[r][i].y * v[r][i].y + v[r][i].z * v[r][i].z + v[r][i].w * v[r][i].w;
      }
    const float rstd = rsqrtf(wave_sum(q) / (float)D + 1e-6f);
    const long mo = (mrow[r] / tokens) * mod_stride;
    const f32x4* sh = (const f32x4*)(shift + mo);
    const f32x4* sc = (const f32x4*)(scale + mo);
#pragma unroll
    for (int i = 0; i < LN_MAXV; ++i) {
      const int c = lane + 64 * i;
      if (c < nv) v[r][i] = v[r][i] * rstd * (1.0f + sc[c]) + sh[c];
    }
  }
  const int r = lane >> 4, ol = lane & 15;
  const long m = CFG ? mfirst + (r & 1) + (long)(r >> 1) * Mh : mfirst + r;
  for (int o0 = 0; o0 < NO; o0 += 16) {
    float part[64];
#pragma unroll
    for (int o = 0; o < 16; ++o) {
      f32x4 w4[LN_MAXV];
#pragma unroll
      for (int i = 0; i < LN_MAXV; ++i) {
        const int c = lane + 64 * i;
        w4[i] = (o0 + o < NO && c < nv) ? ((const f32x4*)(Wf + (long)(o0 + o) * D))[c] : (f32x4){0.f, 0.f, 0.f, 0.f};
      }
#pragma unroll
      for (int rr = 0; rr < 4; ++rr) {
        float a = 0.f;
#pragma unroll
        for (int i = 0; i < LN_MAXV; ++i)
          if (lane + 64 * i < nv) a += v[rr][i].x * w4[i].x + v[rr][i].y * w4[i].y + v[rr][i].z * w4[i].z + v[rr][i].w * w4[i].w;
        part[rr * 16 + o] = a;
      }
    }
#pragma unroll
    for (int s = 0; s < 6; ++s) {
      const int half_w = 32 >> s, mask = 32 >> s;
      const bool upper = (lane & mask) != 0;
#pragma unroll
      for (int k = 0; k < half_w; ++k) {
        const float keep = upper ? part[k + half_w] : part[k];
        const float send = upper ? part[k] : part[k + half_w];
        part[k] = keep + __shfl_xor(send, mask, 64);
      }
    }
    const int o = o0 + ol;
    float val = part[0] + (o < NO ? bf[o] : 0.f);
    if (CFG) {
      const float other = xhalf(val);
      const float cond = r < 2 ? val : other, uncond = r < 2 ? other : val;
      val = uncond + cfg_scale * (cond - uncond);
    }
    if (o < NO && m < M && (CFG || m < Mh)) {
      const int grid = R / p;
      const int n = (int)(m / tokens), tok = (int)(m % tokens);
      const int pp = o / (p * C), qq = (o / C) % p, c = o % C;
      const long off = (((long)n * C + c) * R + (tok / grid) * p + pp) * R + (tok % grid) * p + qq;
      if (base) out[off] = base[off] + (*dt_ptr) * val;
      else out[off] = val;
    }
  }
}

template <bool CFG, int NT>
__global__ __launch_bounds__(256) void final_layer_mfma_kernel(const float* __restrict__ X, int M, int D, int tokens, const float* __restrict__ shift,
                                                               const float* __restrict__ scale, long mod_stride, const float* __restrict__ Wf,
                                                               const float* __restrict__ bf, int C, int R, int p, float cfg_scale, float* out,
                                                               const float* base, const float* __restrict__ dt_ptr) {
  __shared__ float st_s[4][16][3];
  __shared__ float acc_s[4][NT][64][4];
  const int lane = threadIdx.x & 63, wv = threadIdx.x >> 6, a = lane & 15, q = lane >> 4;
  const long tile = blockIdx.x;
  const int Mh = CFG ? M / 2 : M;
  const long m = CFG ? tile * 8 + (a & 7) + (a >> 3) * (long)Mh : tile * 16 + a;
  const float* xr = X + m * D + 8 * q;
  const int nks = D >> 5;
  float cn = 0.f, mu = 0.f, m2 = 0.f;
#pragma unroll 4
  for (int ks = wv; ks < nks; ks += 4) {
    const f32x4 x0 = *(const f32x4*)(xr + 32 * ks), x1 = *(const f32x4*)(xr + 32 * ks + 4);
    const float m8 = (((x0.x + x0.y) + (x0.z + x0.w)) + ((x1.x + x1.y) + (x1.z + x1.w))) * 0.125f;
    const f32x4 d0 = x0 - m8, d1 = x1 - m8;
    const float q8 = ((d0.x * d0.x + d0.y * d0.y) + (d0.z * d0.z + d0.w * d0.w)) + ((d1.x * d1.x + d1.y * d1.y) + (d1.z * d1.z + d1.w * d1.w));
    const float dl = m8 - mu, nn = cn + 8.f, f = 8.f / nn;
    mu += dl * f;
    m2 += q8 + dl * dl * (cn * f);
    cn = nn;
  }
#pragma unroll
  for (int mask = 16; mask <= 32; mask <<= 1) {
    const float dl = __shfl_xor(mu, mask, 64) - mu;
    m2 = (m2 + __shfl_xor(m2, mask, 64)) + dl * dl * (0.5f * cn);
    mu += 0.5f * dl;
    cn += cn;
  }
  if (q == 0) {
    st_s[wv][a][0] = cn;
    st_s[wv][a][1] = mu;
    st_s[wv][a][2] = m2;
  }
  __syncthreads();
  cn = st_s[0][a][0], mu = st_s[0][a][1], m2 = st_s[0][a][2];
#pragma unroll
  for (int w = 1; w < 4; ++w) {
    const float nb = st_s[w][a][0], dl = st_s[w][a][1] - mu, nn = cn + nb, f = nb / nn;
    mu += dl * f;
    m2 += st_s[w][a][2] + dl * dl * (cn * f);
    cn = nn;
  }
  const float mean = mu;
  const float rstd = rsqrtf(m2 / (float)D + 1e-6f);
  const long mo = (m / tokens) * mod_stride + 8 * q;
  f32x4_t acc[NT];
#pragma unroll
  for (int t = 0; t < NT; ++t) acc[t] = (f32x4_t){0.f, 0.f, 0.f, 0.f};
  auto split = [](const f32x4& lo4, const f32x4& hi4, half8_t& h, half8_t& l) {
    const float v[8] = {lo4.x, lo4.y, lo4.z, lo4.w, hi4.x, hi4.y, hi4.z, hi4.w};
#pragma unroll
    for (int e = 0; e < 8; ++e) {
      h[e] = (half_t)v[e];
      l[e] = (half_t)(v[e] - (float)h[e]);
    }
  };
#pragma unroll 2
  for (int ks = wv; ks < nks; ks += 4) {
    const f32x4 x0 = *(const f32x4*)(xr + 32 * ks), x1 = *(const f32x4*)(xr + 32 * ks + 4);
    const f32x4 s0 = *(const f32x4*)(scale + mo + 32 * ks), s1 = *(const f32x4*)(scale + mo + 32 * ks + 4);
    const f32x4 h0 = *(const f32x4*)(shift + mo + 32 * ks), h1 = *(const f32x4*)(shift + mo + 32 * ks + 4);
    const f32x4 a0 = (x0 - mean) * rstd * (1.0f + s0) + h0, a1 = (x1 - mean) * rstd * (1.0f + s1) + h1;
    half8_t ah, al;
    split(a0, a1, ah, al);
#pragma unroll
    for (int t = 0; t < NT; ++t) {
      const float* wr = Wf + (long)(t * 16 + a) * D + 32 * ks + 8 * q;
      half8_t wh, wl;
      split(*(const f32x4*)wr, *(const f32x4*)(wr + 4), wh, wl);
      acc[t] = __builtin_amdgcn_mfma_f32_16x16x32_f16(ah, wh, acc[t], 0, 0, 0);
      acc[t] = __builtin_amdgcn_mfma_f32_16x16x32_f16(al, wh, acc[t], 0, 0, 0);
      acc[t] = __builtin_amdgcn_mfma_f32_16x16x32_f16(ah, wl, acc[t], 0, 0, 0);
    }
  }
#pragma unroll
  for (int t = 0; t < NT; ++t) *(f32x4_t*)acc_s[wv][t][lane] = acc[t];
  __syncthreads();
  if (wv != 0) return;
  const float dt = base ? *dt_ptr : 0.f;
  const int grid = R / p;
#pragma unroll
  for (int t = 0; t < NT; ++t) {
    const f32x4_t tot = (*(const f32x4_t*)acc_s[0][t][lane] + *(const f32x4_t*)acc_s[1][t][lane]) +
                        (*(const f32x4_t*)acc_s[2][t][lane] + *(const f32x4_t*)acc_s[3][t][lane]);
    const int o = t * 16 + a;
    const float bo = bf[o];
    const int pp = o / (p * C), qq = (o / C) % p, c = o % C;
#pragma unroll
    for (int r = 0; r < 4; ++r) {
      const int row = 4 * q + r;
      float val = tot[r] + bo;
      if (CFG) {
        const float other = xhalf(val);
        const float cond = row < 8 ? val : other, uncond = row < 8 ? other : val;
        val = uncond + cfg_scale * (cond - uncond);
      }
      const long mr = CFG ? tile * 8 + (row & 7) + (row >> 3) * (long)Mh : tile * 16 + row;
      const int n = (int)(mr / tokens), tok = (int)(mr % tokens);
      const long off = (((long)n * C + c) * R + (tok / grid) * p + pp) * R + (tok % grid) * p + qq;
      out[off] = base ? base[off] + dt * val : val;
    }
  }
}

__global__ __launch_bounds__(256) void cond_row_copy_kernel(const float* __restrict__ table, long row_floats, const int* __restrict__ step, int offset,
                                                            int fixed_row, float* __restrict__ mod, long nmod, float* __restrict__ uvq, long nq,
                                                            float* __restrict__ uvf, long nf, int to_table, int rows) {
  const long i = ((long)blockIdx.x * 256 + threadIdx.x) * 4;
  if (i >= nmod + nq + nf) return;
  const long row = step ? (long)(*step + offset) : (long)fixed_row;
  float* ws = i < nmod ? mod + i : (i < nmod + nq ? uvq + (i - nmod) : uvf + (i - nmod - nq));
  if (rows > 0 && (row < 0 || row >= rows)) {
    if (!to_table) *(f32x4*)ws = (f32x4){__builtin_nanf(""), __builtin_nanf(""), __builtin_nanf(""), __builtin_nanf("")};
    return;
  }
  float* tb = (float*)table + row * row_floats + i;
  if (to_table) *(f32x4*)tb = *(const f32x4*)ws;
  else *(f32x4*)ws = *(const f32x4*)tb;
}
```

### lfm_amd/hip.py

```python
import ctypes as C
import math
import os

import torch

_HERE = os.path.dirname(os.path.abspath(__file__))
LIB_PATH = os.path.join(_HERE, "_lib", "liblfm_hip.so")
_lib = None


class LfmHipError(RuntimeError):
    pass


class DitShape(C.Structure):
    _fields_ = [(n, C.c_int) for n in ("depth", "hidden", "heads", "patch", "in_ch", "res", "mlp_hidden", "label_rows")]


_DIT_WEIGHT_FIELDS = ("pos_embed", "patch_w", "patch_b", "t_w0", "t_b0", "t_w2", "t_b2", "y_table", "ada_w", "ada_b",
                      "qkv_w", "qkv_b", "proj_w", "proj_b", "fc1_w", "fc1_b", "fc2_w", "fc2_b", "final_w", "final_b", "patch_w16")


class DitWeights(C.Structure):
    _fields_ = [(n, C.c_void_p) for n in _DIT_WEIGHT_FIELDS]


class DitCall(C.Structure):
    _fields_ = [("batch", C.c_int), ("x", C.c_void_p), ("t", C.c_void_p), ("t_len", C.c_int), ("y", C.c_void_p),
                ("cfg", C.c_int), ("cfg_scale", C.c_float), ("out", C.c_void_p), ("axpy_base", C.c_void_p), ("axpy_dt", C.c_void_p),
                ("cond_table", C.c_void_p), ("cond_step", C.c_void_p), ("cond_offset", C.c_int),
                ("cond_rows", C.c_int), ("fold_ln", C.c_int), ("gemm_select", C.c_int)]


class VaeResnet(C.Structure):
    _fields_ = [(n, C.c_void_p) for n in ("n1_g", "n1_b", "c1_w", "c1_b", "n2_g", "n2_b", "c2_w", "c2_b", "sc_w", "sc_b")] + [
        ("cin", C.c_int), ("cout", C.c_int)]


ABI_VERSION = 4
CALL_OFF, CALL_ON = 1, 2


def call_gemm_select(which):
    return int(which) + 1


def lib():
    global _lib
    if _lib is not None:
        return _lib
    from . import _build

    override = os.environ.get("LFM_HIP_LIBRARY")
    if override:
        if not os.path.exists(override):
            raise LfmHipError(f"LFM_HIP_LIBRARY={override} does not exist")
        path = override
    else:
        path = LIB_PATH
    if not override and (os.path.exists(_build.HIPCC) or not os.path.exists(LIB_PATH)):
        try:
            _build.build()
        except Exception as e:
            if not os.path.exists(LIB_PATH):
                raise LfmHipError(f"liblfm_hip.so is missing and could not be built: {e}") from e
            raise LfmHipError(f"liblfm_hip.so is stale and could not be rebuilt: {e}") from e
    try:
        L = C.CDLL(path)
    except OSError as e:
        raise LfmHipError(f"cannot load {path}: {e}") from e
    L.lfm_strerror.restype = C.c_char_p
    L.lfm_strerror.argtypes = [C.c_int]
    L.lfm_abi_version.restype = C.c_int
    if L.lfm_abi_version() != ABI_VERSION:
        raise LfmHipError(f"{path} has ABI {L.lfm_abi_version()}, this package binds ABI {ABI_VERSION}: rebuild it (python -m lfm_amd._build --force)")
    L.lfm_dit_workspace_bytes.restype = C.c_size_t
    L.lfm_dit_workspace_bytes.argtypes = [C.POINTER(DitShape), C.c_int]
    L.lfm_dit_workspace_layout.restype = C.c_int
    L.lfm_dit_workspace_layout.argtypes = [C.POINTER(DitShape), C.c_int, C.POINTER(C.c_size_t), C.c_int]
    L.lfm_dit_forward.restype = C.c_int
    L.lfm_dit_forward.argtypes = [C.POINTER(DitShape), C.POINTER(DitWeights), C.c_void_p, C.c_size_t, C.POINTER(DitCall), C.c_void_p]
    L.lfm_gemm_f16.restype = C.c_int
    L.lfm_gemm_f16.argtypes = [C.c_void_p, C.c_long, C.c_void_p, C.c_long, C.c_void_p, C.c_long, C.c_int, C.c_int, C.c_int,
                               C.c_void_p, C.c_int, C.c_void_p, C.c_long, C.c_int, C.c_void_p]
    L.lfm_dit_cond_table_bytes.restype = C.c_size_t
    L.lfm_dit_cond_table_bytes.argtypes = [C.c_void_p, C.c_int]
    L.lfm_dit_cond_table_build.restype = C.c_int
    L.lfm_dit_cond_table_build.argtypes = [C.c_void_p, C.c_void_p, C.c_void_p, C.c_size_t, C.c_int, C.c_void_p, C.c_int, C.c_void_p, C.c_size_t, C.c_void_p]
    L.lfm_clock_probe.restype = C.c_int
    L.lfm_clock_probe.argtypes = [C.c_int, C.c_int, C.c_void_p, C.c_void_p]
    L.lfm_gemm_select.restype = C.c_int
    L.lfm_gemm_select.argtypes = [C.c_int]
    L.lfm_gemm_qkv_f16.restype = C.c_int
    L.lfm_gemm_qkv_f16.argtypes = [C.c_void_p, C.c_long, C.c_void_p, C.c_long, C.c_void_p, C.c_void_p, C.c_void_p, C.c_int, C.c_int, C.c_int,
                                   C.c_void_p, C.c_int, C.c_int, C.c_void_p]
    if hasattr(L, "lfm_gemm_trace_read"):
        L.lfm_gemm_trace_read.restype = C.c_int
        L.lfm_gemm_trace_read.argtypes = [C.POINTER(C.c_ulonglong), C.c_int]
        L.lfm_attention_trace_read.restype = C.c_int
        L.lfm_attention_trace_read.argtypes = [C.POINTER(C.c_ulonglong), C.c_int]
    L.lfm_profile_fc1.restype = C.c_int
    L.lfm_profile_fc1.argtypes = [C.c_int]
    L.lfm_profile_fc1_read.restype = C.c_int
    L.lfm_profile_fc1_read.argtypes = [C.POINTER(C.c_float), C.c_int]
    L.lfm_profile_blocks_read.restype = C.c_int
    L.lfm_profile_blocks_read.argtypes = [C.POINTER(C.c_float), C.c_int]
    L.lfm_ln_modulate.restype = C.c_int
    L.lfm_ln_modulate.argtypes = [C.c_void_p, C.c_void_p, C.c_int, C.c_int, C.c_int, C.c_void_p, C.c_void_p, C.c_long, C.c_void_p]
    L.lfm_dit_attention.restype = C.c_int
    L.lfm_dit_attention.argtypes = [C.c_void_p, C.c_void_p, C.c_void_p, C.c_void_p, C.c_int, C.c_int, C.c_int, C.c_void_p]
    L.lfm_set_option.restype = C.c_int
    L.lfm_set_option.argtypes = [C.c_int, C.c_int]
    L.lfm_dit_call_settings.restype = C.c_int
    L.lfm_dit_call_settings.argtypes = [C.POINTER(DitCall), C.POINTER(C.c_int), C.POINTER(C.c_int)]
    L.lfm_dit_plan.restype = C.c_int
    L.lfm_dit_plan.argtypes = [C.POINTER(DitShape), C.POINTER(DitCall), C.POINTER(C.c_int)]
    L.lfm_gemm_plan.restype = C.c_int
    L.lfm_gemm_plan.argtypes = [C.c_int] * 5
    L.lfm_attention_plan.restype = C.c_int
    L.lfm_attention_plan.argtypes = [C.c_int] * 4
    L.lfm_dit_attention_hd.restype = C.c_int
    L.lfm_dit_attention_hd.argtypes = [C.c_void_p, C.c_void_p, C.c_void_p, C.c_void_p, C.c_int, C.c_int, C.c_int, C.c_int, C.c_void_p]
    L.lfm_grid_advance.restype = C.c_int
    L.lfm_grid_advance.argtypes = [C.c_void_p] * 7
    L.lfm_lincomb.restype = C.c_int
    L.lfm_lincomb.argtypes = [C.c_void_p, C.c_void_p, C.POINTER(C.c_void_p), C.c_void_p, C.c_void_p, C.c_int, C.c_long, C.c_void_p]
    L.lfm_rk_error_norm.restype = C.c_int
    L.lfm_rk_error_norm.argtypes = [C.c_void_p, C.c_void_p, C.POINTER(C.c_void_p), C.c_void_p, C.c_void_p, C.c_int, C.c_long, C.c_float, C.c_float,
                                    C.c_void_p, C.c_void_p, C.c_void_p]
    L.lfm_vae_workspace_bytes.restype = C.c_size_t
    L.lfm_vae_workspace_bytes.argtypes = [C.c_int, C.c_int]
    L.lfm_vae_decode.restype = C.c_int
    L.lfm_vae_decode.argtypes = [C.c_void_p, C.c_void_p, C.c_size_t, C.c_void_p, C.c_void_p, C.c_int, C.c_int, C.c_int, C.c_void_p]
    L.lfm_vae_encode.restype = C.c_int
    L.lfm_vae_encode.argtypes = [C.c_void_p, C.c_void_p, C.c_size_t, C.c_void_p, C.c_void_p, C.c_int, C.c_int, C.c_int, C.c_void_p]
    L.lfm_images_to_uint8.restype = C.c_int
    L.lfm_images_to_uint8.argtypes = [C.c_void_p, C.c_void_p, C.c_int, C.c_int, C.c_int, C.c_void_p]
    L.lfm_images_to_uint8_mode.restype = C.c_int
    L.lfm_images_to_uint8_mode.argtypes = [C.c_void_p, C.c_void_p, C.c_int, C.c_int, C.c_int, C.c_int, C.c_void_p]
    V, I, LG, F = C.c_void_p, C.c_int, C.c_long, C.c_float
    L.lfm_conv3x3_f16.restype = I
    L.lfm_conv3x3_f16.argtypes = [V, V, V, V, V, I, I, I, I, I, I, V]
    L.lfm_conv3x3_workspace_bytes.restype = C.c_size_t
    L.lfm_conv3x3_workspace_bytes.argtypes = [I, I, I, I, I]
    L.lfm_conv3x3_f16_ws.restype = I
    L.lfm_conv3x3_f16_ws.argtypes = [V, V, V, V, V, I, I, I, I, I, I, V, C.c_size_t, V]
    L.lfm_conv3x3_in_f32.restype = I
    L.lfm_conv3x3_in_f32.argtypes = [V, V, V, V, I, I, I, I, I, V]
    L.lfm_conv3x3_out_f32.restype = I
    L.lfm_conv3x3_out_f32.argtypes = [V, V, V, V, I, I, I, I, I, V]
    L.lfm_linear_f16.restype = I
    L.lfm_linear_f16.argtypes = [V, LG, V, LG, V, LG, I, I, I, V, V, V]
    L.lfm_groupnorm_scratch_bytes.restype = C.c_size_t
    L.lfm_groupnorm_scratch_bytes.argtypes = [I, I]
    L.lfm_groupnorm_f16.restype = I
    L.lfm_groupnorm_f16.argtypes = [V, V, V, V, V, LG, V, I, I, I, I, F, I, V]
    L.lfm_groupnorm2_f16.restype = I
    L.lfm_groupnorm2_f16.argtypes = [V, I, V, I, V, V, V, V, LG, V, I, I, I, F, I, V]
    if hasattr(L, "lfm_groupnorm_plan"):
        L.lfm_groupnorm_plan.restype = I
        L.lfm_groupnorm_plan.argtypes = [I, I, I, I]
        L.lfm_vae_groupnorm_plan.restype = I
        L.lfm_vae_groupnorm_plan.argtypes = [I, I, I, C.c_size_t]
    L.lfm_linear2_f16.restype = I
    L.lfm_linear2_f16.argtypes = [V, I, V, I, V, LG, V, LG, I, I, V, V, V]
    L.lfm_avgpool2_f16.restype = I
    L.lfm_avgpool2_f16.argtypes = [V, V, I, I, I, I, V]
    L.lfm_upsample2_f16.restype = I
    L.lfm_upsample2_f16.argtypes = [V, V, I, I, I, I, V]
    L.lfm_concat_channels_f16.restype = I
    L.lfm_concat_channels_f16.argtypes = [V, V, V, LG, I, I, V]
    L.lfm_add_image_vec_f16.restype = I
    L.lfm_add_image_vec_f16.argtypes = [V, V, LG, V, I, I, I, V]
    L.lfm_attention_small_f16.restype = I
    L.lfm_attention_small_f16.argtypes = [V, V, I, I, I, I, V]
    L.lfm_unet_attention_plan.restype = I
    L.lfm_unet_attention_plan.argtypes = [I, I, I, I]
    L.lfm_cross_attention_f16.restype = I
    L.lfm_cross_attention_f16.argtypes = [V, LG, V, V, LG, V, LG, I, I, I, I, I, V]
    L.lfm_cross_attention_plan.restype = I
    L.lfm_cross_attention_plan.argtypes = [I, I, I, I, I]
    L.lfm_layernorm_f16.restype = I
    L.lfm_layernorm_f16.argtypes = [V, V, V, V, LG, I, F, V]
    L.lfm_geglu_f16.restype = I
    L.lfm_geglu_f16.argtypes = [V, LG, V, LG, I, V]
    L.lfm_time_embed.restype = I
    L.lfm_time_embed.argtypes = [V, I, V, V, V, V, V, V, I, V, V, V, I, I, I, V]
    L.lfm_conv3x3_scaled_f16_ws.restype = I
    L.lfm_conv3x3_scaled_f16_ws.argtypes = [V, V, V, V, F, V, I, I, I, I, I, I, V, C.c_size_t, V]
    L.lfm_conv3x3_plan.restype = I
    L.lfm_conv3x3_plan.argtypes = [I, I, I, I, I, I, C.c_size_t]
    L.lfm_linear_scaled_f16.restype = I
    L.lfm_linear_scaled_f16.argtypes = [V, LG, V, LG, V, LG, I, I, I, V, V, F, V]
    L.lfm_linear2_scaled_f16.restype = I
    L.lfm_linear2_scaled_f16.argtypes = [V, I, V, I, V, LG, V, LG, I, I, V, V, F, V]
    L.lfm_linear_resid_vec_f16.restype = I
    L.lfm_linear_resid_vec_f16.argtypes = [V, LG, V, LG, V, LG, I, I, I, V, V, V, LG, I, F, V]
    L.lfm_linear_silu_f16.restype = I
    L.lfm_linear_silu_f16.argtypes = [V, LG, V, LG, V, LG, I, I, I, V, V]
    L.lfm_linear_gelu_f16.restype = I
    L.lfm_linear_gelu_f16.argtypes = [V, LG, V, LG, V, LG, I, I, I, V, V]
    L.lfm_token_embed_f16.restype = I
    L.lfm_token_embed_f16.argtypes = [V, I, V, I, V, V, I, I, I, V]
    L.lfm_gather_rows_f32.restype = I
    L.lfm_gather_rows_f32.argtypes = [V, I, I, V, I, V, LG, V]
    L.lfm_label_rescale_f32.restype = I
    L.lfm_label_rescale_f32.argtypes = [V, V, V, V, I, I, I, I, I, I, V]
    L.lfm_song_embed.restype = I
    L.lfm_song_embed.argtypes = [V, I, V, V, V, V, V, V, F, V, I, V, V, V, I, I, I, V]
    L.lfm_fourier_embed.restype = I
    L.lfm_fourier_embed.argtypes = [V, I, V, V, V, V, V, V, V, F, V, I, V, V, V, I, I, I, V]
    L.lfm_fir_down2_f16.restype = I
    L.lfm_fir_down2_f16.argtypes = [V, V, V, V, F, I, I, I, I, I, V]
    L.lfm_fir_up2_f16.restype = I
    L.lfm_fir_up2_f16.argtypes = [V, V, I, I, I, I, V]
    L.lfm_zero_border_f16.restype = I
    L.lfm_zero_border_f16.argtypes = [V, V, I, I, I, I, V]
    L.lfm_zero_border_f32.restype = I
    L.lfm_zero_border_f32.argtypes = [V, V, I, I, I, V]
    L.lfm_vae_groupnorm_f16.restype = I
    L.lfm_vae_groupnorm_f16.argtypes = [V, V, V, V, V, C.c_size_t, I, I, I, I, V]
    L.lfm_vae_conv3x3_gn_f16.restype = I
    L.lfm_vae_conv3x3_gn_f16.argtypes = [V, V, V, V, V, V, V, V, V, C.c_size_t, I, I, I, I, I, I, I, C.POINTER(C.c_int), C.POINTER(C.c_int), V]
    L.lfm_vae_mid_attention_workspace_bytes.restype = C.c_size_t
    L.lfm_vae_mid_attention_workspace_bytes.argtypes = [I, I]
    L.lfm_vae_mid_attention_f16.restype = I
    L.lfm_vae_mid_attention_f16.argtypes = [V] * 13 + [C.c_size_t, I, I, V]
    L.lfm_vae_conv_in_f16.restype = I
    L.lfm_vae_conv_in_f16.argtypes = [V] * 6 + [I, I, V]
    L.lfm_vae_downsample_workspace_bytes.restype = C.c_size_t
    L.lfm_vae_downsample_workspace_bytes.argtypes = [I, I, I, I]
    L.lfm_vae_downsample_f16.restype = I
    L.lfm_vae_downsample_f16.argtypes = [V] * 5 + [C.c_size_t, I, I, I, I, V]
    L.lfm_vae_resnets_workspace_bytes.restype = C.c_size_t
    L.lfm_vae_resnets_workspace_bytes.argtypes = [I, I, I]
    L.lfm_vae_resnets_f16.restype = I
    L.lfm_vae_resnets_f16.argtypes = [C.POINTER(VaeResnet), I, V, V, V, C.c_size_t, I, I, I, I, C.POINTER(C.c_int), V]
    L.lfm_vae_conv_moments_workspace_bytes.restype = C.c_size_t
    L.lfm_vae_conv_moments_workspace_bytes.argtypes = [I, I, I]
    L.lfm_vae_conv_moments_f32.restype = I
    L.lfm_vae_conv_moments_f32.argtypes = [V] * 5 + [C.c_size_t, I, I, I, V]
    _lib = L
    return L


def check(rc, what):
    if rc != 0:
        raise LfmHipError(f"{what} failed: {lib().lfm_strerror(rc).decode()} (code {rc})")


def stream_ptr(device=None):
    return C.c_void_p(torch.cuda.current_stream(device).cuda_stream)


def ptr(t):
    return C.c_void_p(t.data_ptr()) if t is not None else C.c_void_p(0)


def check_labels(y, rows, what, noun="label", table="the embedding table",
                 hint=" (classifier-free guidance needs a model built with label_dropout > 0: its null class is row num_classes)"):
    if y is None or y.numel() == 0:
        return
    if y.is_cuda and torch.cuda.is_current_stream_capturing():
        return
    key = (y._version, y.numel(), rows)
    if getattr(y, "_lfm_labels_ok", None) == key:
        return
    lo, hi = (int(v) for v in torch.stack([y.min(), y.max()]).tolist())
    if lo < 0 or hi >= rows:
        raise IndexError(f"{what}: {noun} {hi if hi >= rows else lo} is outside {table} [0, {rows}){hint}")
    try:
        y._lfm_labels_ok = key
    except Exception:
        pass


def require_gpu(t, what):
    if not t.is_cuda:
        raise LfmHipError(f"{what}: tensor is on {t.device}; the LFM hot path only runs on an MI355X (no CPU fallback)")


def gemm_select(which):
    check(lib().lfm_gemm_select(int(which)), "lfm_gemm_select")


def gemm_f16(A, W, bias=None, epilogue=0, out=None, gate=None, gate_stride=0, tokens=1):
    require_gpu(A, "gemm_f16")
    M, K = A.shape
    N = W.shape[0]
    if out is None:
        out = torch.empty(M, N, device=A.device, dtype=torch.float32 if epilogue in (2, 3) else torch.float16)
    check(lib().lfm_gemm_f16(ptr(A), A.stride(0), ptr(W), W.stride(0), ptr(out), out.stride(0), M, N, K, ptr(bias), epilogue,
                             ptr(gate), gate_stride, tokens, stream_ptr()), "lfm_gemm_f16")
    return out


def gemm_qkv_f16(A, W, bias, head_dim, tokens):
    require_gpu(A, "gemm_qkv_f16")
    M, K = A.shape
    D = W.shape[0] // 3
    Q = torch.empty(M, D, device=A.device, dtype=torch.float16)
    Kt = torch.empty_like(Q)
    Vt = torch.empty(M // tokens, D // head_dim, head_dim, tokens, device=A.device, dtype=torch.float16)
    check(lib().lfm_gemm_qkv_f16(ptr(A), A.stride(0), ptr(W), W.stride(0), ptr(Q), ptr(Kt), ptr(Vt), M, D, K, ptr(bias), head_dim, tokens,
                                 stream_ptr()), "lfm_gemm_qkv_f16")
    return Q, Kt, Vt


def ln_modulate(X, shift, scale, tokens, mod_stride):
    require_gpu(X, "ln_modulate")
    M, D = X.shape
    A = torch.empty(M, D, device=X.device, dtype=torch.float16)
    check(lib().lfm_ln_modulate(ptr(X), ptr(A), M, D, tokens, ptr(shift), ptr(scale), mod_stride, stream_ptr()), "lfm_ln_modulate")
    return A


DBG_GEMM_NO_EPILOGUE = 4
DBG_GEMM_SETPRIO = 8
DBG_GEMM_GM8 = 32
DBG_GEMM_GM2 = 64
DBG_GEMM_NO_XCD_REMAP = 128
DBG_GEMM_GM4 = 256
DBG_GEMM_NO_SPLITK = 512
DBG_GEMM_STORE8 = 1024
DBG_GEMM_PARITY_PRIO = 2048
DBG_GEMM_NEVER_V4 = 4096
DBG_GEMM_ALWAYS_V4 = 8192
DBG_GEMM_SPLITK128 = 65536
DBG_GEMM_ABL_SHIFT = 21
DBG_GEMM_ABL_MASK = 15
DBG_GEMM_OPT_SHIFT = 25
DBG_GEMM_OPT_MASK = 3
DBG_TRACE_GEMM = 2
DBG_TRACE_NO_STORES = 131072
DBG_TRACE_COL_SHIFT = 21
DBG_TRACE_COL_MASK = 15
DBG_ATT_WIDE = 256
DBG_ATT_MODE_SHIFT = 25
DBG_ATT_MODE_MASK = 3
DBG_QKV_TRACE = 2
DBG_QKV_NO_VT_WRITES = 262144
DBG_QKV_NO_QK_WRITES = 524288
DBG_QKV_PER_ITEM = 4194304
DBG_QKV_NO_KEY_LOOP = 33554432
DBG_QKV_TWO_KTILES = 67108864
DBG_LN_STORE8 = 32768
DBG_LN_BPERMUTE = 65536
DBG_LN_FOUR_ROWS = 262144
DBG_LN_TWO_ROWS = 524288
DBG_DIT_FINAL_ROUND1 = 1048576
DBG_DIT_PATCH_ROUND1 = 2097152
DBG_CONV_IMPLICIT_GEMM = 8388608
DBG_CONV_HALO_SMALL = 16777216
DBG_VAE_SEPARATE_STATS = 4194304
DBG_UNET_CONV_IN_SCALAR = 1
DBG_UNET_ATT_VALU = 16
DBG_UNET_GN_ROWS = 16384

OPT_FOLD_LN = 1
OPT_SKINNY_GEMM = 4
OPT_ATTENTION_STREAM = 5
OPT_FUSED_QKV_ATTENTION = 6
OPT_UNET_ATTENTION_STREAM = 7
OPT_ATTENTION_TILED = 8
OPT_GEMM_V6 = 2


def effective_clock_mhz(device=None, iters=20000):
    dev = torch.device(device or "cuda:0")
    n = torch.cuda.get_device_properties(dev).multi_processor_count
    ticks = torch.zeros(n, dtype=torch.int64, device=dev)
    for it in (200, iters):
        e0, e1 = torch.cuda.Event(enable_timing=True), torch.cuda.Event(enable_timing=True)
        e0.record(torch.cuda.current_stream(dev))
        check(lib().lfm_clock_probe(n, it, ptr(ticks), stream_ptr(dev)), "lfm_clock_probe")
        e1.record(torch.cuda.current_stream(dev))
        torch.cuda.synchronize(dev)
    ms = e0.elapsed_time(e1)
    return 2.0 * float(ticks.max()) / (ms * 1e3)


PLAN_FOLDED_LN, PLAN_FUSED_QKV_ATTENTION = 1, 2


def dit_plan(shape, batch, t_len=1, labels=False, fold_ln=0, gemm_select=0):
    call = DitCall()
    call.batch, call.t_len, call.y = int(batch), int(t_len), (1 if labels else None)
    call.fold_ln, call.gemm_select = fold_ln, gemm_select
    plan = C.c_int(-1)
    check(lib().lfm_dit_plan(C.byref(shape), C.byref(call), C.byref(plan)), "lfm_dit_plan")
    return plan.value


DIT_WS_BUFFERS = ("X", "A", "A2", "QKVH", "mod", "ln_part", "cen0", "cen1", "uvq", "uvf")


def dit_workspace_layout(shape, batch):
    offs = (C.c_size_t * len(DIT_WS_BUFFERS))()
    rc = lib().lfm_dit_workspace_layout(C.byref(shape), int(batch), offs, len(DIT_WS_BUFFERS))
    if rc < 0:
        check(rc, "lfm_dit_workspace_layout")
    assert rc == len(DIT_WS_BUFFERS), rc
    return dict(zip(DIT_WS_BUFFERS, (int(o) for o in offs)))


GEMM_CAP_V6, GEMM_CAP_FITS = 1, 2


def gemm_plan(M, N, K, batch=1, caps=GEMM_CAP_V6 | GEMM_CAP_FITS):
    return lib().lfm_gemm_plan(int(M), int(N), int(K), int(batch), int(caps))


def attention_plan(batch, heads, head_dim, T):
    return lib().lfm_attention_plan(int(batch), int(heads), int(head_dim), int(T))


DIT_RESIDENT_TOKENS = (16, 64, 128, 256, 1024)


def dit_tokens_served(tokens):
    tokens = int(tokens)
    if tokens in DIT_RESIDENT_TOKENS:
        return True
    side = math.isqrt(tokens) if tokens > 0 else 0
    return side * side == tokens and side % 4 == 0 and 144 <= tokens <= 3600


CONV_PLAN_HALO, CONV_PLAN_SPLITK, CONV_PLAN_GEMM = 1, 2, 3


def conv3x3_plan(N, H, W, Cin, Cout, mode=0, workspace_bytes=0):
    return lib().lfm_conv3x3_plan(int(N), int(H), int(W), int(Cin), int(Cout), int(mode), int(workspace_bytes))


GN_STATS_FUSED, GN_STATS_ROWS, GN_STATS_GROUPS4, GN_STATS_GROUPS1 = 1, 2, 3, 4
GN_APPLY_FUSED, GN_APPLY_OCTET, GN_APPLY_CHUNK = 1, 2, 3


def groupnorm_plan(N, HW, C, groups):
    plan = lib().lfm_groupnorm_plan(int(N), int(HW), int(C), int(groups))
    return plan if plan < 0 else (plan & 15, plan >> 4)


def vae_groupnorm_plan(n, HW, C, workspace_bytes):
    return lib().lfm_vae_groupnorm_plan(int(n), int(HW), int(C), int(workspace_bytes))


def unet_attention_plan(N, T, heads, ch):
    return lib().lfm_unet_attention_plan(int(N), int(T), int(heads), int(ch))


def unet_attention(qkv, out, N, T, heads, ch):
    if unet_attention_plan(N, T, heads, ch) < 0:
        raise LfmHipError(f"UNet attention: no kernel serves T = {T} tokens x {ch} channels per head (limit: channels per head % 16 == 0 and <= 256 for any "
                          f"token count; other widths only while min(T, 64) * (T + 1) * 4 + 4 * T * (ch + 2) <= {160 * 1024} bytes of LDS)")
    check(lib().lfm_attention_small_f16(ptr(qkv), ptr(out), N, T, heads, ch, stream_ptr(qkv.device)), "lfm_attention_small_f16")
    return out


def cross_attention_plan(N, Tq, Tk, heads, ch):
    return lib().lfm_cross_attention_plan(int(N), int(Tq), int(Tk), int(heads), int(ch))


def cross_attention(Q, K, V, N, Tq, Tk, heads, ch, out=None):
    require_gpu(Q, "cross_attention")
    if cross_attention_plan(N, Tq, Tk, heads, ch) < 0:
        raise LfmHipError(f"cross-attention: no kernel serves {Tq} queries x {Tk} keys x {ch} channels per head (limit: channels per head % 16 == 0 and "
                          "<= 256, any positive token counts)")
    if out is None:
        out = torch.empty(N * Tq, heads * ch, dtype=torch.float16, device=Q.device)
    C_ = heads * ch
    for name, t, rows in (("Q", Q, N * Tq), ("K", K, N * Tk), ("V", V, N * Tk), ("out", out, N * Tq)):
        if t.dtype != torch.float16 or tuple(t.shape) != (rows, C_) or t.stride(1) != 1 or t.device != Q.device:
            raise LfmHipError(f"cross-attention: {name} must be fp16 [{rows}, {C_}] with unit column stride on {Q.device}, got {t.dtype} {tuple(t.shape)} "
                              f"strides {t.stride()} on {t.device}")
    if K.stride(0) != V.stride(0):
        raise LfmHipError(f"cross-attention: K and V must share a row stride (two column slices of one buffer), got {K.stride(0)} and {V.stride(0)}")
    check(lib().lfm_cross_attention_f16(ptr(Q), Q.stride(0), ptr(K), ptr(V), K.stride(0), ptr(out), out.stride(0), N, Tq, Tk, heads, ch,
                                        stream_ptr(Q.device)), "lfm_cross_attention_f16")
    return out


def layernorm(x, gamma, beta, eps=1e-5, out=None):
    require_gpu(x, "layernorm")
    M, C = x.shape
    if C % 8:
        raise LfmHipError(f"layernorm: {C} channels (limit: channels % 8 == 0)")
    if out is None:
        out = torch.empty(M, C, dtype=torch.float16, device=x.device)
    for name, t in (("x", x), ("out", out)):
        if t.dtype != torch.float16 or tuple(t.shape) != (M, C) or t.stride() != (C, 1) or t.device != x.device:
            raise LfmHipError(f"layernorm: {name} must be dense fp16 [{M}, {C}] on {x.device}, got {t.dtype} {tuple(t.shape)} strides {t.stride()} on {t.device}")
    for name, t in (("gamma", gamma), ("beta", beta)):
        if t.dtype != torch.float32 or tuple(t.shape) != (C,) or t.stride() != (1,) or t.device != x.device:
            raise LfmHipError(f"layernorm: {name} must be dense fp32 [{C}] on {x.device}, got {t.dtype} {tuple(t.shape)} on {t.device}")
    check(lib().lfm_layernorm_f16(ptr(x), ptr(out), ptr(gamma), ptr(beta), M, C, float(eps), stream_ptr(x.device)), "lfm_layernorm_f16")
    return out


def geglu(h, out=None):
    require_gpu(h, "geglu")
    M, I2 = h.shape
    if I2 % 16:
        raise LfmHipError(f"geglu: {I2} columns (limit: half of them % 8 == 0)")
    if out is None:
        out = torch.empty(M, I2 // 2, dtype=torch.float16, device=h.device)
    if h.dtype != torch.float16 or h.stride(1) != 1:
        raise LfmHipError(f"geglu: h must be fp16 with unit column stride, got {h.dtype} strides {h.stride()}")
    if out.dtype != torch.float16 or tuple(out.shape) != (M, I2 // 2) or out.stride() != (I2 // 2, 1) or out.device != h.device:
        raise LfmHipError(f"geglu: out must be dense fp16 [{M}, {I2 // 2}] on {h.device}, got {out.dtype} {tuple(out.shape)} strides {out.stride()} on {out.device}")
    check(lib().lfm_geglu_f16(ptr(h), h.stride(0), ptr(out), M, I2 // 2, stream_ptr(h.device)), "lfm_geglu_f16")
    return out


def linear_resid_vec(x, w, bias, resid, vec, tokens, scale=1.0, out=None):
    require_gpu(x, "linear_resid_vec")
    M, K = x.shape
    N = w.shape[0]
    if out is None:
        out = torch.empty(M, N, dtype=torch.float16, device=x.device)
    if vec is not None and (vec.dtype != torch.float32 or tuple(vec.shape) != (M // tokens, N) or vec.stride(1) != 1):
        raise LfmHipError(f"linear_resid_vec: vec must be fp32 [{M // tokens}, {N}] with unit column stride, got {vec.dtype} {tuple(vec.shape)} strides {vec.stride()}")
    check(lib().lfm_linear_resid_vec_f16(ptr(x), x.stride(0), ptr(w), w.stride(0), ptr(out), out.stride(0), M, N, K, ptr(bias), ptr(resid), ptr(vec),
                                         vec.stride(0) if vec is not None else 0, int(tokens), float(scale), stream_ptr(x.device)), "lfm_linear_resid_vec_f16")
    return out


def linear_silu(x, w, bias, out=None):
    require_gpu(x, "linear_silu")
    M, K = x.shape
    N = w.shape[0]
    if out is None:
        out = torch.empty(M, N, dtype=torch.float16, device=x.device)
    check(lib().lfm_linear_silu_f16(ptr(x), x.stride(0), ptr(w), w.stride(0), ptr(out), out.stride(0), M, N, K, ptr(bias), stream_ptr(x.device)),
          "lfm_linear_silu_f16")
    return out


def linear_gelu(x, w, bias, out=None):
    require_gpu(x, "linear_gelu")
    M, K = x.shape
    N = w.shape[0]
    if out is None:
        out = torch.empty(M, N, dtype=torch.float16, device=x.device)
    check(lib().lfm_linear_gelu_f16(ptr(x), x.stride(0), ptr(w), w.stride(0), ptr(out), out.stride(0), M, N, K, ptr(bias), stream_ptr(x.device)),
          "lfm_linear_gelu_f16")
    return out


def token_embed(tok_emb, pos_emb, ids, out=None):
    require_gpu(tok_emb, "token_embed")
    vocab, D = tok_emb.shape
    N, L = ids.shape
    for name, t in (("tok_emb", tok_emb), ("pos_emb", pos_emb)):
        if t.dtype != torch.float32 or t.dim() != 2 or t.shape[1] != D or not t.is_contiguous() or t.device != tok_emb.device:
            raise LfmHipError(f"token_embed: {name} must be dense fp32 [rows, {D}] on {tok_emb.device}, got {t.dtype} {tuple(t.shape)} on {t.device}")
    if ids.dtype != torch.int64 or not ids.is_contiguous() or ids.device != tok_emb.device:
        raise LfmHipError(f"token_embed: ids must be contiguous int64 on {tok_emb.device}, got {ids.dtype} on {ids.device}")
    if out is None:
        out = torch.empty(N * L, D, dtype=torch.float16, device=tok_emb.device)
    if out.dtype != torch.float16 or tuple(out.shape) != (N * L, D) or not out.is_contiguous():
        raise LfmHipError(f"token_embed: out must be dense fp16 [{N * L}, {D}], got {out.dtype} {tuple(out.shape)} strides {out.stride()}")
    check(lib().lfm_token_embed_f16(ptr(tok_emb), vocab, ptr(pos_emb), pos_emb.shape[0], ptr(ids), ptr(out), N, L, D, stream_ptr(tok_emb.device)),
          "lfm_token_embed_f16")
    return out


def gather_rows(table, y, out=None):
    require_gpu(table, "gather_rows")
    rows, cols = table.shape
    if table.dtype != torch.float32 or not table.is_contiguous() or y.dtype != torch.int64 or not y.is_contiguous() or y.device != table.device:
        raise LfmHipError(f"gather_rows: table must be dense fp32 and y contiguous int64 on {table.device}, got {table.dtype} / {y.dtype} on {y.device}")
    if out is None:
        out = torch.empty(y.numel(), cols, device=table.device)
    check(lib().lfm_gather_rows_f32(ptr(table), rows, cols, ptr(y), y.numel(), ptr(out), out.stride(0), stream_ptr(table.device)), "lfm_gather_rows_f32")
    return out


LABEL_RESCALE_MAX_STAGES, LABEL_RESCALE_MAX_COUT, LABEL_RESCALE_TABLE_BYTES = 4, 8, 65536


def label_rescale_serves(num_cls, cout, n_stages):
    return 1 <= n_stages <= LABEL_RESCALE_MAX_STAGES and 1 <= cout <= LABEL_RESCALE_MAX_COUT and num_cls >= 1 and num_cls * cout * 4 <= LABEL_RESCALE_TABLE_BYTES


def label_rescale(labels, w, bias, n_stages, out=None):
    require_gpu(labels, "label_rescale")
    if labels.dtype != torch.int64 or labels.dim() != 3 or not labels.is_contiguous():
        raise LfmHipError(f"label_rescale: labels must be contiguous int64 [N, H, W], got {labels.dtype} {tuple(labels.shape)} strides {labels.stride()}")
    N, H, W = labels.shape
    if w.dtype != torch.float32 or w.dim() != 2 or not w.is_contiguous() or w.device != labels.device:
        raise LfmHipError(f"label_rescale: w must be dense fp32 [Cout, num_cls] on {labels.device}, got {w.dtype} {tuple(w.shape)} on {w.device}")
    cout, num_cls = w.shape
    if bias is not None and (bias.dtype != torch.float32 or tuple(bias.shape) != (cout,) or not bias.is_contiguous() or bias.device != labels.device):
        raise LfmHipError(f"label_rescale: bias must be dense fp32 [{cout}] on {labels.device}, got {bias.dtype} {tuple(bias.shape)} on {bias.device}")
    shape = (N, cout, H >> n_stages, W >> n_stages)
    if out is None:
        out = torch.empty(shape, dtype=torch.float32, device=labels.device)
    if out.dtype != torch.float32 or tuple(out.shape) != shape or not out.is_contiguous() or out.device != labels.device:
        raise LfmHipError(f"label_rescale: out must be dense fp32 {shape} on {labels.device}, got {out.dtype} {tuple(out.shape)} strides {out.stride()}")
    check(lib().lfm_label_rescale_f32(ptr(labels), ptr(w), ptr(bias), ptr(out), N, H, W, num_cls, cout, int(n_stages), stream_ptr(labels.device)),
          "lfm_label_rescale_f32")
    return out


def fir_down2(x, N, Ho, Wo, C, pad=1, bias=None, resid=None, scale=1.0, out=None):
    require_gpu(x, "fir_down2")
    if out is None:
        out = torch.empty(N * Ho * Wo, C, dtype=torch.float16, device=x.device)
    check(lib().lfm_fir_down2_f16(ptr(x), ptr(out), ptr(bias), ptr(resid), float(scale), N, Ho, Wo, C, pad, stream_ptr(x.device)), "lfm_fir_down2_f16")
    return out


def fir_up2(x, N, Ho, Wo, C, out=None):
    require_gpu(x, "fir_up2")
    if out is None:
        out = torch.empty(N * Ho * Wo, C, dtype=torch.float16, device=x.device)
    check(lib().lfm_fir_up2_f16(ptr(x), ptr(out), N, Ho, Wo, C, stream_ptr(x.device)), "lfm_fir_up2_f16")
    return out


def zero_border(x, N, H, W, C):
    require_gpu(x, "zero_border")
    if x.dtype == torch.float32:
        out = torch.empty(N, C, H + 2, W + 2, device=x.device)
        check(lib().lfm_zero_border_f32(ptr(x), ptr(out), N * C, H, W, stream_ptr(x.device)), "lfm_zero_border_f32")
    else:
        out = torch.empty(N * (H + 2) * (W + 2), C, dtype=torch.float16, device=x.device)
        check(lib().lfm_zero_border_f16(ptr(x), ptr(out), N, H, W, C, stream_ptr(x.device)), "lfm_zero_border_f16")
    return out


def set_option(key, value):
    check(lib().lfm_set_option(int(key), int(value)), "lfm_set_option")


def vt_token_perm(T, device=None):
    i = torch.arange(T, device=device)
    return (i & ~12) | ((i & 4) << 1) | ((i & 8) >> 1)


def dit_attention(Q, K, Vt, batch, heads, T, head_dim=64):
    require_gpu(Q, "dit_attention")
    O = torch.empty_like(Q)
    check(lib().lfm_dit_attention_hd(ptr(Q), ptr(K), ptr(Vt), ptr(O), batch, heads, head_dim, T, stream_ptr()), "lfm_dit_attention_hd")
    return O


def rk_error_norm(y0, y1, ks, e_coef, dt, rtol, atol, scratch, out):
    require_gpu(y0, "rk_error_norm")
    arr = (C.c_void_p * len(ks))(*[k.data_ptr() for k in ks])
    check(lib().lfm_rk_error_norm(ptr(y0), ptr(y1), arr, ptr(e_coef), ptr(dt), len(ks), y0.numel(), float(rtol), float(atol), ptr(scratch), ptr(out),
                                  stream_ptr(y0.device)), "lfm_rk_error_norm")
    return out


def lincomb(out, base, ks, coef, scale=None):
    require_gpu(out, "lincomb")
    arr = (C.c_void_p * len(ks))(*[k.data_ptr() for k in ks])
    check(lib().lfm_lincomb(ptr(out), ptr(base), arr, ptr(coef), ptr(scale), len(ks), out.numel(), stream_ptr(out.device)), "lfm_lincomb")
    return out
```

### lfm_amd/models/DiT.py

```python
import ctypes as C
import math

import numpy as np
import torch
import torch.nn as nn

from .. import hip
from ._unet_host import PackedModule


class _Attention(nn.Module):
    def __init__(self, dim, num_heads):
        super().__init__()
        self.num_heads = num_heads
        self.qkv = nn.Linear(dim, dim * 3, bias=True)
        self.proj = nn.Linear(dim, dim)


class _Mlp(nn.Module):
    def __init__(self, dim, hidden):
        super().__init__()
        self.fc1 = nn.Linear(dim, hidden)
        self.fc2 = nn.Linear(hidden, dim)


class _PatchEmbed(nn.Module):
    def __init__(self, img, patch, in_chans, dim):
        super().__init__()
        self.patch_size = (patch, patch)
        self.num_patches = (img // patch) ** 2
        self.proj = nn.Conv2d(in_chans, dim, kernel_size=patch, stride=patch, bias=True)


class TimestepEmbedder(nn.Module):
    def __init__(self, hidden_size, frequency_embedding_size=256):
        super().__init__()
        self.mlp = nn.Sequential(nn.Linear(frequency_embedding_size, hidden_size), nn.SiLU(), nn.Linear(hidden_size, hidden_size))
        self.frequency_embedding_size = frequency_embedding_size


class LabelEmbedder(nn.Module):
    def __init__(self, num_classes, hidden_size, dropout_prob):
        super().__init__()
        self.in_channels = num_classes + (dropout_prob > 0)
        self.embedding_table = nn.Embedding(self.in_channels, hidden_size)
        self.num_classes = num_classes
        self.dropout_prob = dropout_prob

    def get_in_channels(self):
        return self.in_channels


class DiTBlock(nn.Module):
    def __init__(self, hidden_size, num_heads, mlp_ratio=4.0):
        super().__init__()
        self.attn = _Attention(hidden_size, num_heads)
        self.mlp = _Mlp(hidden_size, int(hidden_size * mlp_ratio))
        self.adaLN_modulation = nn.Sequential(nn.SiLU(), nn.Linear(hidden_size, 6 * hidden_size, bias=True))


class FinalLayer(nn.Module):
    def __init__(self, hidden_size, patch_size, out_channels):
        super().__init__()
        self.linear = nn.Linear(hidden_size, patch_size * patch_size * out_channels, bias=True)
        self.adaLN_modulation = nn.Sequential(nn.SiLU(), nn.Linear(hidden_size, 2 * hidden_size, bias=True))


def get_2d_sincos_pos_embed(embed_dim, grid_size):
    pos = np.arange(grid_size, dtype=np.float64)
    col, row = np.meshgrid(pos, pos)

    def one(dim, p):
        omega = 1.0 / 10000 ** (np.arange(dim // 2, dtype=np.float64) / (dim / 2.0))
        out = p.reshape(-1)[:, None] * omega[None]
        return np.concatenate([np.sin(out), np.cos(out)], axis=1)

    return np.concatenate([one(embed_dim // 2, col), one(embed_dim // 2, row)], axis=1)


class DiT(PackedModule):
    _scratch_attrs = ("_ws",)

    def __init__(self, img_resolution=32, patch_size=2, in_channels=4, hidden_size=1152, depth=28, num_heads=16,
                 mlp_ratio=4.0, label_dropout=0.1, num_classes=1000, learn_sigma=False):
        super().__init__()
        self._init_host_state()
        if learn_sigma:
            raise NotImplementedError("learn_sigma=True is never used by the LFM sampling path")
        tokens = (img_resolution // patch_size) ** 2 if patch_size and img_resolution % patch_size == 0 else 0
        kk = patch_size * patch_size * in_channels
        if hidden_size % num_heads or hidden_size // num_heads not in (64, 72):
            raise NotImplementedError(f"DiT with head_dim {hidden_size / num_heads:g}: the attention kernels are built for head_dim 64 "
                                      "(DiT-S / B / L) and 72 (DiT-XL: 1152 / 16)")
        if not hip.dit_tokens_served(tokens) or (kk > 16 and kk % 64) or kk > 256 or hidden_size % 64 or hidden_size > 1280:
            raise NotImplementedError(f"DiT shape not built: {tokens} tokens (need 16 / 64 / 128 / 256 / 1024 or a square grid whose side is a multiple of 4, "
                                      f"144 to 3600 tokens), patch inputs {kk} (need <= 16 or a multiple of 64 up to 256), hidden {hidden_size} (multiple of 64, "
                                      "<= 1280)")
        self.learn_sigma = learn_sigma
        self.in_channels = in_channels
        self.out_channels = in_channels
        self.patch_size = patch_size
        self.num_heads = num_heads
        self.num_classes = num_classes
        self.img_resolution = img_resolution
        self.hidden_size = hidden_size
        self.depth = depth
        self.mlp_hidden = int(hidden_size * mlp_ratio)

        self.x_embedder = _PatchEmbed(img_resolution, patch_size, in_channels, hidden_size)
        self.t_embedder = TimestepEmbedder(hidden_size)
        self.y_embedder = LabelEmbedder(num_classes, hidden_size, label_dropout)
        self.pos_embed = nn.Parameter(torch.zeros(1, self.x_embedder.num_patches, hidden_size), requires_grad=False)
        self.blocks = nn.ModuleList([DiTBlock(hidden_size, num_heads, mlp_ratio=mlp_ratio) for _ in range(depth)])
        self.final_layer = FinalLayer(hidden_size, patch_size, self.out_channels)
        self.initialize_weights()

    def initialize_weights(self):
        for m in self.modules():
            if isinstance(m, nn.Linear):
                nn.init.xavier_uniform_(m.weight)
                nn.init.zeros_(m.bias)
        grid = int(self.x_embedder.num_patches ** 0.5)
        self.pos_embed.data.copy_(torch.from_numpy(get_2d_sincos_pos_embed(self.hidden_size, grid)).float().unsqueeze(0))
        w = self.x_embedder.proj.weight.data
        nn.init.xavier_uniform_(w.view(w.shape[0], -1))
        nn.init.zeros_(self.x_embedder.proj.bias)
        nn.init.normal_(self.y_embedder.embedding_table.weight, std=0.02)
        nn.init.normal_(self.t_embedder.mlp[0].weight, std=0.02)
        nn.init.normal_(self.t_embedder.mlp[2].weight, std=0.02)
        for blk in self.blocks:
            nn.init.zeros_(blk.adaLN_modulation[-1].weight)
            nn.init.zeros_(blk.adaLN_modulation[-1].bias)
        nn.init.zeros_(self.final_layer.adaLN_modulation[-1].weight)
        nn.init.zeros_(self.final_layer.adaLN_modulation[-1].bias)
        nn.init.zeros_(self.final_layer.linear.weight)
        nn.init.zeros_(self.final_layer.linear.bias)

    def shape_struct(self):
        return hip.DitShape(self.depth, self.hidden_size, self.num_heads, self.patch_size, self.in_channels, self.img_resolution,
                            self.mlp_hidden, self.y_embedder.get_in_channels())

    @torch.no_grad()
    def _pack(self):
        dev = self.pos_embed.device
        hip.require_gpu(self.pos_embed, "DiT")
        f32 = lambda t: t.detach().to(dev, torch.float32).contiguous()
        f16 = lambda t: t.detach().to(dev, torch.float16).contiguous()
        B = self.blocks
        keep = {
            "pos_embed": f32(self.pos_embed[0]),
            "patch_w": f32(self.x_embedder.proj.weight.reshape(self.hidden_size, -1)),
            "patch_b": f32(self.x_embedder.proj.bias),
            "t_w0": f32(self.t_embedder.mlp[0].weight), "t_b0": f32(self.t_embedder.mlp[0].bias),
            "t_w2": f32(self.t_embedder.mlp[2].weight), "t_b2": f32(self.t_embedder.mlp[2].bias),
            "y_table": f32(self.y_embedder.embedding_table.weight),
            "ada_w": f16(torch.cat([b.adaLN_modulation[1].weight for b in B] + [self.final_layer.adaLN_modulation[1].weight], 0)),
            "ada_b": f32(torch.cat([b.adaLN_modulation[1].bias for b in B] + [self.final_layer.adaLN_modulation[1].bias], 0)),
            "qkv_w": f16(torch.stack([b.attn.qkv.weight for b in B])), "qkv_b": f32(torch.stack([b.attn.qkv.bias for b in B])),
            "proj_w": f16(torch.stack([b.attn.proj.weight for b in B])), "proj_b": f32(torch.stack([b.attn.proj.bias for b in B])),
            "fc1_w": f16(torch.stack([b.mlp.fc1.weight for b in B])), "fc1_b": f32(torch.stack([b.mlp.fc1.bias for b in B])),
            "fc2_w": f16(torch.stack([b.mlp.fc2.weight for b in B])), "fc2_b": f32(torch.stack([b.mlp.fc2.bias for b in B])),
            "final_w": f32(self.final_layer.linear.weight), "final_b": f32(self.final_layer.linear.bias),
            "patch_w16": f16(self.x_embedder.proj.weight.reshape(self.hidden_size, -1)),
        }
        w = hip.DitWeights(**{k: v.data_ptr() for k, v in keep.items()})
        self._packed = (w, keep, self.shape_struct())
        self._gen += 1
        return self._packed

    def _workspace(self, batch, device):
        if self._ws is None or self._ws[0] < batch or self._ws[1].device != device:
            shape = self.shape_struct()
            nbytes = hip.lib().lfm_dit_workspace_bytes(C.byref(shape), batch)
            if nbytes == 0:
                raise hip.LfmHipError(f"DiT shape not supported by the HIP path: {self.extra_repr()}")
            self._ws = (batch, torch.empty(nbytes, dtype=torch.uint8, device=device))
            self._gen += 1
        return self._ws[1]

    def extra_repr(self):
        return (f"depth={self.depth}, hidden={self.hidden_size}, heads={self.num_heads}, patch={self.patch_size}, "
                f"res={self.img_resolution}, in_ch={self.in_channels}")

    @torch.no_grad()
    def cond_table(self, ts, batch):
        hip.require_gpu(ts, "DiT.cond_table")
        w, _, shape = self._packed or self._pack()
        ts = ts.detach().to(torch.float32).contiguous()
        n = ts.numel()
        nbytes = hip.lib().lfm_dit_cond_table_bytes(C.byref(shape), n)
        if nbytes == 0:
            raise hip.LfmHipError("lfm_dit_cond_table_bytes refused the shape")
        table = torch.empty(nbytes, dtype=torch.uint8, device=ts.device)
        ws = self._workspace(batch, ts.device)
        rc = hip.lib().lfm_dit_cond_table_build(C.byref(shape), C.byref(w), hip.ptr(ws), ws.numel(), batch, hip.ptr(ts), n, hip.ptr(table), nbytes,
                                                hip.stream_ptr(ts.device))
        hip.check(rc, "lfm_dit_cond_table_build")
        return table

    @torch.no_grad()
    def _run(self, t, x, y, cfg, cfg_scale, out=None, axpy_base=None, axpy_dt=None, cond=None, fold_ln=0, gemm_select=0):
        hip.require_gpu(x, "DiT.forward")
        if self.training:
            raise hip.LfmHipError("the HIP DiT is inference-only: call .eval() (label dropout / autograd are training features)")
        if x.dim() != 4 or x.shape[1] != self.in_channels or x.shape[2] != self.img_resolution or x.shape[3] != self.img_resolution:
            raise ValueError(f"x must be [N,{self.in_channels},{self.img_resolution},{self.img_resolution}], got {tuple(x.shape)}")
        packed = self._packed or self._pack()
        w, _, shape = packed
        N = x.shape[0]
        x = x.contiguous().float()
        t = torch.as_tensor(t, device=x.device).float().reshape(-1).contiguous()
        if t.numel() not in (1, N):
            raise ValueError(f"t must have 1 or {N} elements, got {t.numel()}")
        if cond is not None and (y is not None or t.numel() != 1):
            raise ValueError("a per-grid conditioning table serves evaluations with ONE shared conditioning row (scalar t, no labels)")
        if y is not None:
            y = y.to(device=x.device, dtype=torch.long).contiguous()
            if y.numel() != N:
                raise ValueError(f"y must have {N} elements")
            hip.check_labels(y, self.y_embedder.get_in_channels(), "DiT")
        if out is None:
            out = torch.empty_like(x)
        ws = self._workspace(N, x.device)
        call = hip.DitCall(N, x.data_ptr(), t.data_ptr(), t.numel(), y.data_ptr() if y is not None else None, 1 if cfg else 0,
                           float(cfg_scale), out.data_ptr(), axpy_base.data_ptr() if axpy_base is not None else None,
                           axpy_dt.data_ptr() if axpy_dt is not None else None,
                           cond[0].data_ptr() if cond is not None else None, cond[1].data_ptr() if cond is not None else None,
                           int(cond[2]) if cond is not None else 0,
                           int(cond[3]) if cond is not None and len(cond) > 3 else 0,
                           int(fold_ln), int(gemm_select))
        rc = hip.lib().lfm_dit_forward(C.byref(shape), C.byref(w), hip.ptr(ws), ws.numel(), C.byref(call), hip.stream_ptr(x.device))
        hip.check(rc, "lfm_dit_forward")
        return out

    def forward(self, t, x, y=None, **kwargs):
        return self._run(t, x, y, False, 1.0)

    def forward_with_cfg(self, t, x, y=None, cfg_scale=1.0, **kwargs):
        if x.shape[0] % 2:
            raise ValueError("forward_with_cfg needs an even batch (cond | uncond)")
        return self._run(t, x, y, True, cfg_scale)


def _cfg(depth, hidden, patch, heads):
    return lambda **kw: DiT(depth=depth, hidden_size=hidden, patch_size=patch, num_heads=heads, **kw)


DiT_models = {
    "DiT-XL/2": _cfg(28, 1152, 2, 16), "DiT-XL/4": _cfg(28, 1152, 4, 16), "DiT-XL/8": _cfg(28, 1152, 8, 16),
    "DiT-L/2": _cfg(24, 1024, 2, 16), "DiT-L/4": _cfg(24, 1024, 4, 16), "DiT-L/8": _cfg(24, 1024, 8, 16),
    "DiT-B/2": _cfg(12, 768, 2, 12), "DiT-B/4": _cfg(12, 768, 4, 12), "DiT-B/8": _cfg(12, 768, 8, 12),
    "DiT-S/2": _cfg(12, 384, 2, 6), "DiT-S/4": _cfg(12, 384, 4, 6), "DiT-S/8": _cfg(12, 384, 8, 6),
}
_ = math
```

### lfm_amd/solvers.py

```python
import math

import os

import torch

from . import hip


class _SolverCache(dict):

    def __deepcopy__(self, memo):
        return _SolverCache()

    def __reduce__(self):
        return (_SolverCache, ())

ADAPTIVE_SOLVER = ["dopri5", "dopri8", "adaptive_heun", "bosh3"]
FIXER_SOLVER = ["euler", "rk4", "midpoint", "stochastic"]


def fixed_grid(t, step_size):
    niters = torch.ceil((t[-1] - t[0]) / step_size + 1).item()
    grid = torch.arange(0, niters, dtype=t.dtype, device=t.device) * step_size + t[0]
    grid[-1] = t[-1]
    return grid


def _euler_step(f, t0, dt, t1, y0):
    return dt * f(t0, y0)


def _midpoint_step(f, t0, dt, t1, y0):
    half = 0.5 * dt
    return dt * f(t0 + half, y0 + f(t0, y0) * half)


def _rk4_step(f, t0, dt, t1, y0):
    k1 = f(t0, y0)
    k2 = f(t0 + dt / 3, y0 + dt * k1 / 3)
    k3 = f(t0 + dt * 2 / 3, y0 + dt * (k2 - k1 / 3))
    k4 = f(t1, y0 + dt * (k1 - k2 + k3))
    return (k1 + 3 * (k2 + k3) + k4) * dt * 0.125


_STEP = {"euler": _euler_step, "midpoint": _midpoint_step, "rk4": _rk4_step}

_DP_A = (1 / 5, 3 / 10, 4 / 5, 8 / 9, 1.0, 1.0)
_DP_B = ((1 / 5,), (3 / 40, 9 / 40), (44 / 45, -56 / 15, 32 / 9), (19372 / 6561, -25360 / 2187, 64448 / 6561, -212 / 729),
         (9017 / 3168, -355 / 33, 46732 / 5247, 49 / 176, -5103 / 18656), (35 / 384, 0.0, 500 / 1113, 125 / 192, -2187 / 6784, 11 / 84))
_DP_E = (35 / 384 - 1951 / 21600, 0.0, 500 / 1113 - 22642 / 50085, 125 / 192 - 451 / 720, -2187 / 6784 + 12231 / 42400,
         11 / 84 - 649 / 6300, -1.0 / 60.0)
_DP_MID = (6025192743 / 30085553152 / 2, 0.0, 51252292925 / 65400821598 / 2, -2691868925 / 45128329728 / 2,
           187940372067 / 1594534317056 / 2, -1776094331 / 19743644256 / 2, 11237099 / 235043384 / 2)


def _rms(x):
    return x.pow(2).mean().sqrt()


def _comb(ks, coefs, dt):
    acc = None
    for k, c in zip(ks, coefs):
        if c != 0:
            term = k * (c * dt)
            acc = term if acc is None else acc + term
    return acc


_BS_A = (1 / 2, 3 / 4, 1.0)
_BS_B = ((1 / 2,), (0.0, 3 / 4), (2 / 9, 1 / 3, 4 / 9))
_BS_E = (2 / 9 - 7 / 24, 1 / 3 - 1 / 4, 4 / 9 - 1 / 3, -1 / 8)
_BS_MID = (0.0, 0.5, 0.0, 0.0)
_AH_A = (1.0,)
_AH_B = ((1.0,),)
_AH_SOL = (0.5, 0.5)
_AH_E = (0.5, -0.5)
_AH_MID = (0.5, 0.0)


_D8_A = (1 / 18, 1 / 12, 1 / 8, 5 / 16, 3 / 8, 59 / 400, 93 / 200, 5490023248 / 9719169821, 13 / 20, 1201146811 / 1299019798, 1.0, 1.0, 1.0)
_D8_SOL = (14005451 / 335480064, 0.0, 0.0, 0.0, 0.0, -59238493 / 1068277825, 181606767 / 758867731, 561292985 / 797845732,
           -1041891430 / 1371343529, 760417239 / 1151165299, 118820643 / 751138087, -528747749 / 2220607170, 1 / 4)
_D8_EMB = (13451932 / 455176623, 0.0, 0.0, 0.0, 0.0, -808719846 / 976000145, 1757004468 / 5645159321, 656045339 / 265891186,
           -3867574721 / 1518517206, 465885868 / 322736535, 53011238 / 667516719, 2 / 45, 0.0)
_D8_B = (
    (1 / 18,),
    (1 / 48, 1 / 16),
    (1 / 32, 0.0, 3 / 32),
    (5 / 16, 0.0, -75 / 64, 75 / 64),
    (3 / 80, 0.0, 0.0, 3 / 16, 3 / 20),
    (29443841 / 614563906, 0.0, 0.0, 77736538 / 692538347, -28693883 / 1125000000, 23124283 / 1800000000),
    (16016141 / 946692911, 0.0, 0.0, 61564180 / 158732637, 22789713 / 633445777, 545815736 / 2771057229, -180193667 / 1043307555),
    (39632708 / 573591083, 0.0, 0.0, -433636366 / 683701615, -421739975 / 2616292301, 100302831 / 723423059, 790204164 / 839813087,
     800635310 / 3783071287),
    (246121993 / 1340847787, 0.0, 0.0, -37695042795 / 15268766246, -309121744 / 1061227803, -12992083 / 490766935, 6005943493 / 2108947869,
     393006217 / 1396673457, 123872331 / 1001029789),
    (-1028468189 / 846180014, 0.0, 0.0, 8478235783 / 508512852, 1311729495 / 1432422823, -10304129995 / 1701304382, -48777925059 / 3047939560,
     15336726248 / 1032824649, -45442868181 / 3398467696, 3065993473 / 597172653),
    (185892177 / 718116043, 0.0, 0.0, -3185094517 / 667107341, -477755414 / 1098053517, -703635378 / 230739211, 5731566787 / 1027545527,
     5232866602 / 850066563, -4093664535 / 808688257, 3962137247 / 1805957418, 65686358 / 487910083),
    (403863854 / 491063109, 0.0, 0.0, -5068492393 / 434740067, -411421997 / 543043805, 652783627 / 914296604, 11173962825 / 925320556,
     -13158990841 / 6184727034, 3936647629 / 1978049680, -160528059 / 685178525, 248638103 / 1413531060, 0.0),
    _D8_SOL,
)
_D8_E = tuple(a - b for a, b in zip(_D8_SOL, _D8_EMB)) + (0.0,)
_D8_MID = (0.04075652697815933, 0.0, 0.0, 0.0, 0.0, 0.14575312352778258, 0.2349319583967853, 0.07730057792519462, 0.015741038709153957,
           -0.015256809590672644, 3.823380238289129e-05, 0.0007353502512138821, 0.0, 0.0)


class Dopri5:

    A, B, SOL, E, MID, ORDER = _DP_A, _DP_B, None, _DP_E, _DP_MID, 5

    def __init__(self, f, y0, t0, rtol, atol, max_num_steps=2 ** 31 - 1):
        self.f, self.rtol, self.atol, self.max_num_steps = f, rtol, atol, max_num_steps
        self.nfe_steps = 0
        self.accepted = 0
        self._dev = bool(y0.is_cuda and y0.dtype == torch.float32 and y0.is_contiguous() and y0.numel() % 4 == 0 and len(self.E) <= 8
                         and float(rtol) == rtol and float(atol) == atol)
        self._y_like = y0
        if self._dev:
            dv = y0.device
            self._cB = [torch.tensor(b, dtype=torch.float32, device=dv) for b in self.B]
            self._cE = torch.tensor(self.E, dtype=torch.float32, device=dv)
            self._cSOL = None if self.SOL is None else torch.tensor(self.SOL, dtype=torch.float32, device=dv)
            self._scratch = torch.empty(1024, dtype=torch.float32, device=dv)
            self._ratio = torch.empty(1, dtype=torch.float32, device=dv)
        f0 = self._stage(f(t0, y0))
        self.y0, self.f0 = y0, f0
        self.t0 = self.t1 = t0
        self._t0_h = self._t1_h = float(t0)
        self.dt = self._initial_step(t0, y0, f0, order=self.ORDER - 1)
        self._last = None
        self.coef = [y0] * 5

    @property
    def dt(self):
        return self._dt

    @dt.setter
    def dt(self, value):
        self._dt, self._dt_h = value, float(value)

    def _initial_step(self, t0, y0, f0, order=4):
        scale = self.atol + y0.abs() * self.rtol
        d0, d1 = _rms(y0 / scale), _rms(f0 / scale)
        h0 = torch.full_like(d0, 1e-6) if (d0 < 1e-5 or d1 < 1e-5) else 0.01 * d0 / d1
        f1 = self.f(t0.to(y0.dtype) + h0, y0 + h0 * f0)
        d2 = _rms((f1 - f0) / scale) / h0
        if d1 <= 1e-15 and d2 <= 1e-15:
            h1 = torch.max(torch.full_like(h0, 1e-6), h0 * 1e-3)
        else:
            h1 = (0.01 / torch.max(d1, d2)) ** (1.0 / (order + 1))
        return torch.min(100 * h0, h1).to(t0.dtype)

    def _stage(self, k):
        if not self._dev:
            return k
        y0 = self.y0 if hasattr(self, "y0") else None
        ref = y0 if y0 is not None else self._y_like
        if torch.is_tensor(k) and k.shape == ref.shape and k.device == ref.device:
            if k.dtype != ref.dtype or not k.is_contiguous():
                k = k.to(ref.dtype).contiguous()
            return k
        self._dev = False
        return k

    def _lin(self, base, ks, coef_dev, coef_host, dty):
        if self._dev and len(ks) <= 8:
            out = torch.empty_like(base)
            hip.lincomb(out, base, ks, coef_dev[: len(ks)], dty)
            return out
        return base + _comb(ks, coef_host, dty)

    def _step(self):
        y0, f0, t0, dt = self.y0, self.f0, self.t1, self.dt
        t1 = t0 + dt
        t0y, dty, t1y = t0.to(y0.dtype), dt.to(y0.dtype), t1.to(y0.dtype)
        k = [f0]
        yi = y0
        for i, (a, b) in enumerate(zip(self.A, self.B)):
            yi = self._lin(y0, k, self._cB[i] if self._dev else None, b, dty)
            k.append(self._stage(self.f(t1y if a == 1.0 else t0y + a * dty, yi)))
        y1 = yi if self.SOL is None else self._lin(y0, k, self._cSOL if self._dev else None, self.SOL, dty)
        f1 = k[-1]
        if self._dev:
            hip.rk_error_norm(y0, y1, k, self._cE, dty, self.rtol, self.atol, self._scratch, self._ratio)
            ratio_h = float(self._ratio)
        else:
            err = _comb(k, self.E, dty)
            tol = self.atol + self.rtol * torch.max(y0.abs(), y1.abs())
            ratio_h = float(_rms(err / tol))
        self.nfe_steps += 1
        if ratio_h <= 1:
            self._last = (y0, y1, f0, f1, k, dty)
            self.coef = None
            self.t0, self.t1, self.y0, self.f0 = t0, t1, y1, f1
            self._t0_h, self._t1_h = self._t1_h, self._t1_h + self._dt_h
            self.accepted += 1
        if ratio_h == 0:
            factor = 10.0
        else:
            factor = min(10.0, max(0.9 / ratio_h ** (1.0 / self.ORDER), 1.0 if ratio_h < 1 else 0.2))
        self._dt, self._dt_h = dt * factor, self._dt_h * factor

    def _fit(self):
        if self.coef is None:
            y0, y1, f0, f1, k, dty = self._last
            y_mid = y0 + _comb(k, self.MID, dty)
            a = 2 * dty * (f1 - f0) - 8 * (y1 + y0) + 16 * y_mid
            b = dty * (5 * f0 - 3 * f1) + 18 * y0 + 14 * y1 - 32 * y_mid
            c = dty * (f1 - 4 * f0) - 11 * y0 - 5 * y1 + 16 * y_mid
            self.coef = [y0, dty * f0, c, b, a]
        return self.coef

    def advance(self, t_next):
        n = 0
        t_next_h = float(t_next)
        while t_next_h > self._t1_h:
            assert n < self.max_num_steps
            self._step()
            n += 1
        coef = self._fit()
        x = ((t_next - self.t0) / (self.t1 - self.t0)).to(coef[0].dtype)
        total = coef[0] + x * coef[1]
        xp = x
        for c in coef[2:]:
            xp = xp * x
            total = total + xp * c
        return total


class Bosh3(Dopri5):
    A, B, SOL, E, MID, ORDER = _BS_A, _BS_B, None, _BS_E, _BS_MID, 3


class AdaptiveHeun(Dopri5):
    A, B, SOL, E, MID, ORDER = _AH_A, _AH_B, _AH_SOL, _AH_E, _AH_MID, 2


class Dopri8(Dopri5):
    A, B, SOL, E, MID, ORDER = _D8_A, _D8_B, None, _D8_E, _D8_MID, 8


_ADAPTIVE = {"dopri5": Dopri5, "dopri8": Dopri8, "bosh3": Bosh3, "adaptive_heun": AdaptiveHeun}


def _perturbed(f):

    def g(t, y, perturb=0):
        t = t.to(y.dtype)
        if perturb > 0:
            t = torch.nextafter(t, t + 1)
        elif perturb < 0:
            t = torch.nextafter(t, t - 1)
        return f(t, y)

    return g


def _euler_step_p(f, t0, dt, t1, y0):
    return dt * f(t0, y0, perturb=1)


def _midpoint_step_p(f, t0, dt, t1, y0):
    half = 0.5 * dt
    return dt * f(t0 + half, y0 + f(t0, y0, perturb=1) * half)


def _rk4_step_p(f, t0, dt, t1, y0):
    k1 = f(t0, y0, perturb=1)
    k2 = f(t0 + dt / 3, y0 + dt * k1 / 3)
    k3 = f(t0 + dt * 2 / 3, y0 + dt * (k2 - k1 / 3))
    k4 = f(t1, y0 + dt * (k1 - k2 + k3), perturb=-1)
    return (k1 + 3 * (k2 + k3) + k4) * dt * 0.125


_STEP_P = {"euler": _euler_step_p, "midpoint": _midpoint_step_p, "rk4": _rk4_step_p}


@torch.no_grad()
def odeint(func, y0, t, *, rtol=1e-7, atol=1e-9, method=None, options=None, stats=None):
    method = method or "dopri5"
    options = dict(options or {})
    t = t.detach().clone()
    f = func
    if len(t) > 1 and bool(t[0] > t[1]):
        t = -t
        f = lambda s, y, _f=func: -_f(-s, y)
    g = lambda s, y, _f=f: _f(s.to(y.dtype), y)
    if method in _STEP:
        if "step_size" not in options:
            raise ValueError("fixed-grid solvers need options['step_size']")
        grid = fixed_grid(t, options["step_size"])
        step = _STEP[method]
        if options.get("perturb"):
            g, step = _perturbed(g), _STEP_P[method]
        sol, j = [y0], 1
        tl = t.tolist()
        gl = grid.tolist()
        for i in range(len(gl) - 1):
            t0, t1 = grid[i], grid[i + 1]
            y1 = y0 + step(g, t0, t1 - t0, t1, y0)
            while j < len(tl) and gl[i + 1] >= tl[j]:
                if tl[j] == gl[i + 1]:
                    sol.append(y1)
                elif tl[j] == gl[i]:
                    sol.append(y0)
                else:
                    sol.append(y0 + (t[j] - t0) / (t1 - t0) * (y1 - y0))
                j += 1
            y0 = y1
        return torch.stack(sol, 0)
    if method in _ADAPTIVE:
        t = t.to(torch.float64)
        solver = _ADAPTIVE[method](g, y0, t[0], rtol, atol)
        sol = [y0] + [solver.advance(t[j]) for j in range(1, len(t))]
        if stats is not None:
            stats.update(steps=solver.nfe_steps, accepted=solver.accepted, nfe=2 + len(solver.A) * solver.nfe_steps)
        return torch.stack(sol, 0)
    raise NotImplementedError(f"method {method!r}: euler / midpoint / rk4 / dopri5 / dopri8 / bosh3 / adaptive_heun are built")


def torchdiffeq_euler_grid(step_size, device=None):
    s = fixed_grid(torch.tensor([-1.0, -0.0]), step_size)
    ts = -s
    dts = -(s[1:] - s[:-1])
    return ts.to(device), dts.to(device)


def fused_fixed_grid_available(model, x):
    from .models.DiT import DiT
    from .models.EDM import DhariwalUNet, SongUNet
    from .models.unet import UNetModel

    inner = getattr(model, "model", None) if type(model).__name__ == "WrapperCondFlow" else model
    return isinstance(inner, (DiT, UNetModel, DhariwalUNet, SongUNet)) and x.is_cuda and not inner.training


class GraphedFixedGrid:

    def __init__(self, model, batch, y=None, cfg_scale=1.0, use_cfg=False, graph=True, resolution=None):
        from .models.DiT import DiT
        from .models.EDM import DhariwalUNet

        self.is_dit = isinstance(model, DiT)
        dev = next(model.parameters()).device
        C = model.in_channels
        R = model.img_resolution if self.is_dit else (resolution or model.image_size)
        self.host_cfg = bool(use_cfg) and isinstance(model, DhariwalUNet)
        if use_cfg and not self.is_dit and not self.host_cfg:
            raise NotImplementedError(f"classifier-free guidance needs forward_with_cfg, which {type(model).__name__} does not have")
        self.model, self.batch, self.dev = model, batch, dev
        self.y = None if y is None else y.to(dev, torch.long).clone()
        self.use_cfg, self.cfg_scale = bool(use_cfg), float(cfg_scale)
        self.x = torch.zeros(batch, C, R, R, device=dev)
        self.d1 = torch.zeros_like(self.x)
        self.d2 = torch.zeros_like(self.x)
        self.xp = torch.zeros_like(self.x)
        self.step = torch.zeros(1, dtype=torch.int32, device=dev)
        self.tcur = torch.zeros(1, device=dev)
        self.tnext = torch.zeros(1, device=dev)
        self.dt = torch.zeros(1, device=dev)
        self.c1 = torch.ones(1, device=dev)
        self.c2 = torch.full((2,), 0.5, device=dev)
        self.max_intervals = 4096
        self.ts = torch.zeros(self.max_intervals + 1, device=dev)
        self.dts = torch.zeros(self.max_intervals, device=dev)
        self.n_intervals = 0
        self.use_graph = graph
        self.graphs = {}
        self._graph_gen = -1
        self.use_cond_table = self.is_dit and self.y is None and not self.use_cfg and os.environ.get("LFM_COND_TABLE", "1") != "0"
        self.cond_buf = None
        self._cond_rows = 0
        self._cond_key = None
        self._grid_host = ()

    def set_grid(self, ts, dts):
        n = dts.numel()
        if ts.numel() != n + 1 or n < 1 or n > self.max_intervals:
            raise ValueError(f"grid with {ts.numel()} times / {n} steps (max {self.max_intervals} intervals)")
        self.ts[: n + 1].copy_(ts.to(torch.float32))
        self.dts[:n].copy_(dts.to(torch.float32))
        self.n_intervals = n
        if self.use_cond_table:
            self._grid_host = tuple(float(v) for v in ts.detach().cpu().tolist())
            self._refresh_cond()

    def _refresh_cond(self):
        if not self.use_cond_table or self.n_intervals < 1:
            return
        n = self.n_intervals
        if self._cond_key == (self._grid_host, getattr(self.model, "_gen", 0)):
            return
        import ctypes as _C
        shape = self.model.shape_struct()
        if hip.lib().lfm_dit_cond_table_bytes(_C.byref(shape), n + 1) > self.COND_TABLE_MAX_BYTES:
            if self._cond_rows:
                self.graphs.clear()
            self._cond_rows = 0
            self._cond_key = (self._grid_host, getattr(self.model, "_gen", 0))
            return
        table = self.model.cond_table(self.ts[: n + 1], self.batch)
        if self.cond_buf is None or self.cond_buf.numel() < table.numel():
            self.cond_buf = table
            self.graphs.clear()
        else:
            self.cond_buf[: table.numel()].copy_(table)
        if self._cond_rows != n + 1:
            self.graphs.clear()
        self._cond_rows = n + 1
        self._cond_key = (self._grid_host, getattr(self.model, "_gen", 0))

    def _cond(self, offset):
        return (self.cond_buf, self.step, offset, self._cond_rows) if self._cond_active() else None

    COND_TABLE_MAX_BYTES = 1 << 30

    def _cond_active(self):
        return self.use_cond_table and self.cond_buf is not None and self._cond_rows > 0

    def _advance(self):
        hip.check(hip.lib().lfm_grid_advance(hip.ptr(self.ts), hip.ptr(self.dts), hip.ptr(self.step), hip.ptr(self.tcur), hip.ptr(self.tnext),
                                             hip.ptr(self.dt), hip.stream_ptr(self.dev)), "lfm_grid_advance")

    def _velocity(self, t, x, out=None, grid_offset=None):
        if self.is_dit:
            return self.model._run(t, x, self.y, self.use_cfg, self.cfg_scale, out=out, cond=None if grid_offset is None else self._cond(grid_offset))
        if self.host_cfg:
            v = self.model.forward_with_cfg(t, x, self.y, cfg_scale=self.cfg_scale)
        else:
            v = self.model(t, x, self.y)
        if out is not None:
            out.copy_(v)
            return out
        return v

    def _euler(self):
        self._advance()
        if self.is_dit:
            self.model._run(self.tcur, self.x, self.y, self.use_cfg, self.cfg_scale, out=self.x, axpy_base=self.x, axpy_dt=self.dt, cond=self._cond(-1))
        else:
            hip.lincomb(self.x, self.x, [self._velocity(self.tcur, self.x)], self.c1, self.dt)

    def _heun(self):
        self._advance()
        d1 = self._velocity(self.tcur, self.x, out=self.d1, grid_offset=-1)
        hip.lincomb(self.xp, self.x, [d1], self.c1, self.dt)
        d2 = self._velocity(self.tnext, self.xp, out=self.d2, grid_offset=0)
        hip.lincomb(self.x, self.x, [d1, d2], self.c2, self.dt)

    def _get(self, kind):
        fn = self._euler if kind == "euler" else self._heun
        if not self.use_graph:
            return fn
        if self._graph_gen != getattr(self.model, "_gen", 0):
            self.graphs.clear()
        if kind not in self.graphs:
            side = torch.cuda.Stream(self.dev)
            side.wait_stream(torch.cuda.current_stream(self.dev))
            with torch.cuda.stream(side):
                saved = (self.x.clone(), self.step.clone())
                fn()
                self.x.copy_(saved[0])
                self.step.copy_(saved[1])
            torch.cuda.current_stream(self.dev).wait_stream(side)
            g = torch.cuda.CUDAGraph()
            with torch.cuda.graph(g, capture_error_mode="thread_local"):
                fn()
            self.x.copy_(saved[0])
            self.step.copy_(saved[1])
            self.graphs[kind] = g
            self._graph_gen = getattr(self.model, "_gen", 0)
        return self.graphs[kind].replay

    @torch.no_grad()
    def run(self, x0, heun_limit=0):
        assert self.n_intervals > 0, "set_grid first"
        n = self.n_intervals
        self._refresh_cond()
        self.x.copy_(x0)
        self.step.zero_()
        n_heun = max(0, min(n, heun_limit - 1)) if heun_limit else 0
        self.last_plan = {"heun": n_heun, "euler": n - n_heun, "nfe": 2 * n_heun + (n - n_heun)}
        if n_heun:
            h = self._get("heun")
            for _ in range(n_heun):
                h()
        if n - n_heun:
            e = self._get("euler")
            for _ in range(n - n_heun):
                e()
        return self.x




def _label_rows(model):
    if hasattr(model, "y_embedder"):
        return model.y_embedder.get_in_channels()
    return getattr(model, "num_classes", None)


def _fused(model, x, model_kwargs):
    y = model_kwargs.get("y")
    cfg_scale = float(model_kwargs.get("cfg_scale", 1.0))
    use_cfg = cfg_scale > 1.0
    if y is not None and _label_rows(model):
        hip.check_labels(y, _label_rows(model), type(model).__name__)
    per_model = model.__dict__.setdefault("_fused_solvers", _SolverCache())
    key = (tuple(x.shape), use_cfg, cfg_scale, y is not None, x.device)
    fg = per_model.get(key)
    if fg is None:
        if len(per_model) > 8:
            per_model.clear()
        fg = GraphedFixedGrid(model, x.shape[0], y=y, cfg_scale=cfg_scale, use_cfg=use_cfg, resolution=x.shape[-1])
        per_model[key] = fg
    elif y is not None:
        fg.y.copy_(y)
    return fg


def concurrency_twin(module):
    import copy

    if hasattr(module, "_pack") and getattr(module, "_packed", None) is None and any(p.is_cuda for p in module.parameters()):
        module._pack()
    t = copy.copy(module)
    t.__dict__.pop("_fused_solvers", None)
    for scratch in ("_ws", "_scratch", "_conv_ws", "_film_all"):
        if scratch in t.__dict__:
            setattr(t, scratch, None)
    return t


def sample_fixed_grid_fused(model, x, sigmas, model_kwargs, heun_limit=0):
    fg = _fused(model, x, model_kwargs)
    sig = sigmas.to(torch.float32)
    fg.set_grid(sig, sig[1:] - sig[:-1])
    return fg.run(x, heun_limit=heun_limit).clone()


def sample_torchdiffeq_euler_fused(model, x, step_size, model_kwargs):
    fg = _fused(model, x, model_kwargs)
    ts, dts = torchdiffeq_euler_grid(step_size)
    fg.set_grid(ts, dts)
    return fg.run(x).clone()


_ = math
```

Before: 122.2 images/sec.

## Chain Euler steps by fusing final layer with next step's patch embed

Adds a seam kernel that fuses the DiT final layer and Euler update with the next step's patch embedding plus folded LayerNorm. Consecutive Euler steps then skip a separate embed launch and the round trip of the latent through global memory. The solver runs first, middle and last step variants, each captured in its own graph, and reads the next conditioning row from the table. This adds code complexity. The fused kernel also reloads the patch-embed weight fragments in every block, which may raise register pressure.

```diff
diff --git a/include/lfm_hip.h b/include/lfm_hip.h
--- a/include/lfm_hip.h
+++ b/include/lfm_hip.h
@@ -87,7 +87,17 @@
 
 #define LFM_PLAN_FOLDED_LN 1
 #define LFM_PLAN_FUSED_QKV_ATTENTION 2
+#define LFM_PLAN_CHAINED 4
 int lfm_dit_plan(const lfm_dit_shape* shape, const lfm_dit_call* call, int* plan_out);
+
+typedef struct lfm_dit_chain {
+  int flags;
+} lfm_dit_chain;
+#define LFM_CHAIN_EMBEDDED 1
+#define LFM_CHAIN_SEAM 2
+#define LFM_CHAIN_EMBED_ONLY 4
+int lfm_dit_forward_chained(const lfm_dit_shape* shape, const lfm_dit_weights* w, void* workspace, size_t workspace_bytes, const lfm_dit_call* call,
+                            const lfm_dit_chain* chain, lfm_stream_t stream);
 
 size_t lfm_dit_cond_table_bytes(const lfm_dit_shape* shape, int n_times);
 int lfm_dit_cond_table_build(const lfm_dit_shape* shape, const lfm_dit_weights* w, void* workspace, size_t workspace_bytes, int batch, const float* t_values,
diff --git a/lfm_amd/csrc/dit.hip b/lfm_amd/csrc/dit.hip
--- a/lfm_amd/csrc/dit.hip
+++ b/lfm_amd/csrc/dit.hip
@@ -402,6 +402,9 @@
     p.loop = DIT_LOOP_LATENCY;
   return p;
 }
+static bool dit_chain_ok(const DitPlan& p, const lfm_dit_shape* s, const DitDims& d, int rows, const lfm_dit_call* c) {
+  return p.fold && p.pe_mfma && p.fin_mfma && d.KK == 16 && s->patch == 2 && d.D <= 1024 && rows == 1 && !c->cfg && c->cond_table && c->axpy_base;
+}
 extern "C" int lfm_dit_plan(const lfm_dit_shape* s, const lfm_dit_call* c, int* plan_out) {
   int rc = check_shape(s);
   if (rc) return rc;
@@ -410,8 +413,10 @@
   if (B <= 0 || (c->t_len != 1 && c->t_len != B)) return LFM_ERR_SHAPE;
   CallScope scope;
   if ((rc = call_scope_enter(c)) != LFM_OK) return rc;
-  const DitPlan p = dit_plan(s, dit_dims(s, B), (c->t_len == 1 && !c->y) ? 1 : B);
-  *plan_out = (p.fold ? LFM_PLAN_FOLDED_LN : 0) | (p.fused ? LFM_PLAN_FUSED_QKV_ATTENTION : 0);
+  const DitDims d = dit_dims(s, B);
+  const int rows = (c->t_len == 1 && !c->y) ? 1 : B;
+  const DitPlan p = dit_plan(s, d, rows);
+  *plan_out = (p.fold ? LFM_PLAN_FOLDED_LN : 0) | (p.fused ? LFM_PLAN_FUSED_QKV_ATTENTION : 0) | (dit_chain_ok(p, s, d, rows, c) ? LFM_PLAN_CHAINED : 0);
   return LFM_OK;
 }
 
@@ -442,7 +447,7 @@
   bool prof_ok, chk;
   BlockW block(int i) const { return block_weights(w, ws.mod, *this, i); }
   void checksum(const void* buf, size_t bytes, int i, int slot) const { if (chk) dit_chk(buf, bytes, i, slot, st); }
-  int embed() const, blocks_folded() const, blocks_latency() const, blocks_separate() const, final_layer() const;
+  int embed() const, blocks_folded() const, blocks_latency() const, blocks_separate() const, final_layer() const, seam() const;
 };
 
 int DitCtx::embed() const {
@@ -599,8 +604,17 @@
   return LFM_OK;
 }
 
-extern "C" int lfm_dit_forward(const lfm_dit_shape* s, const lfm_dit_weights* w, void* workspace, size_t workspace_bytes,
-                               const lfm_dit_call* c, lfm_stream_t stream) {
+int DitCtx::seam() const {
+  const float* fmod = ws.mod + (long)s->depth * 6 * D;
+  hipLaunchKernelGGL(dit_seam_kernel, dim3((unsigned)(M / 16)), dim3(256), 0, st, ws.X, M, D, T, fmod, fmod + D, w->final_w, w->final_b, s->res, c->out, c->axpy_dt,
+                     w->patch_w, w->patch_b, w->pos_embed, ws.A, (const float*)c->cond_table, cond_row_floats(*this), c->cond_step, c->cond_offset + 1, c->cond_rows,
+                     (long)D, ws.ln_part, tiles_p, ws.cen[0]);
+  LFM_CHECK_LAUNCH();
+  return LFM_OK;
+}
+
+static int dit_forward(const lfm_dit_shape* s, const lfm_dit_weights* w, void* workspace, size_t workspace_bytes, const lfm_dit_call* c, int chain,
+                       lfm_stream_t stream) {
   int rc = check_shape(s);
   if (rc) return rc;
   if (!w || !workspace || !c || !c->x || !c->t || !c->out) return LFM_ERR_ARG;
@@ -619,13 +633,17 @@
   const int rows = (c->t_len == 1 && !c->y) ? 1 : B;
   const bool tab = c->cond_table != nullptr;
   if (tab && (rows != 1 || !c->cond_step)) return LFM_ERR_ARG;
+  if (chain & ~(LFM_CHAIN_EMBEDDED | LFM_CHAIN_SEAM | LFM_CHAIN_EMBED_ONLY)) return LFM_ERR_ARG;
+  if ((chain & LFM_CHAIN_EMBED_ONLY) && (chain & (LFM_CHAIN_EMBEDDED | LFM_CHAIN_SEAM))) return LFM_ERR_ARG;
   DitCtx x{d, s, w, c, workspace, ws, dit_plan(s, d, rows, &ws, w), rows,  rows == 1 ? 0 : d.J, st,
             ws.QKVH, ws.QKVH + (size_t)d.M * d.D, ws.QKVH + (size_t)2 * d.M * d.D, prof_ok,  false};
+  if ((chain & (LFM_CHAIN_EMBEDDED | LFM_CHAIN_SEAM)) && (!dit_chain_ok(x.p, s, d, rows, c) || c->out != c->axpy_base)) return LFM_ERR_ARG;
 
   if (tab) rc = dit_cond_copy(ws, d, (const float*)c->cond_table, c->cond_step, c->cond_offset, 0, 0, st, c->cond_rows);
   else rc = dit_conditioning(s, w, ws, d, c->t, c->t_len, c->y, rows, x.p.fold, st);
   if (rc) return rc;
-  if ((rc = x.embed()) != LFM_OK) return rc;
+  if (!(chain & LFM_CHAIN_EMBEDDED) && (rc = x.embed()) != LFM_OK) return rc;
+  if (chain & LFM_CHAIN_EMBED_ONLY) return LFM_OK;
 #ifdef LFM_MEASURE
   x.chk = g_chk && workspace == g_chk_ws;
   if (x.chk) (void)hipMemsetAsync(g_chk, 0, DIT_CHK_SLOTS * 8, st);
@@ -639,5 +657,14 @@
   }
   if (rc) return rc;
   if (prof_blk) (void)hipEventRecord(g_prof_blk_ev[2 * g_prof_blk_count++ + 1], st);
-  return x.final_layer();
-}
+  return (chain & LFM_CHAIN_SEAM) ? x.seam() : x.final_layer();
+}
+extern "C" int lfm_dit_forward(const lfm_dit_shape* s, const lfm_dit_weights* w, void* workspace, size_t workspace_bytes,
+                               const lfm_dit_call* c, lfm_stream_t stream) {
+  return dit_forward(s, w, workspace, workspace_bytes, c, 0, stream);
+}
+extern "C" int lfm_dit_forward_chained(const lfm_dit_shape* s, const lfm_dit_weights* w, void* workspace, size_t workspace_bytes, const lfm_dit_call* c,
+                                       const lfm_dit_chain* chain, lfm_stream_t stream) {
+  if (!chain) return LFM_ERR_ARG;
+  return dit_forward(s, w, workspace, workspace_bytes, c, chain->flags, stream);
+}
diff --git a/lfm_amd/csrc/dit_kernels.h b/lfm_amd/csrc/dit_kernels.h
--- a/lfm_amd/csrc/dit_kernels.h
+++ b/lfm_amd/csrc/dit_kernels.h
@@ -94,30 +94,104 @@
   }
 }
 
+typedef half_t pe_half4v __attribute__((ext_vector_type(4)));
+struct PeFrag {
+  pe_half4v wh[8][2], wl[8][2];
+  f32x4 bias[8][2];
+};
+__device__ __forceinline__ void patch_embed_load_frag(PeFrag& f, const float* __restrict__ w, const float* __restrict__ b, int wv, int a, int q) {
+#pragma unroll
+  for (int pr = 0; pr < 8; ++pr)
+#pragma unroll
+    for (int e = 0; e < 2; ++e) {
+      const int n = 256 * wv + 32 * pr + 8 * (a >> 2) + 4 * e + (a & 3);
+      const f32x4 wf = *(const f32x4*)(w + (long)n * 16 + 4 * q);
+      const float wa[4] = {wf.x, wf.y, wf.z, wf.w};
+#pragma unroll
+      for (int i = 0; i < 4; ++i) {
+        f.wh[pr][e][i] = (half_t)wa[i];
+        f.wl[pr][e][i] = (half_t)(wa[i] - (float)f.wh[pr][e][i]);
+      }
+      f.bias[pr][e] = *(const f32x4*)(b + 256 * wv + 32 * pr + 8 * q + 4 * e);
+    }
+}
+__device__ __forceinline__ void patch_embed_ln_tile(const PeFrag& f, const float (&xa)[4], const float* __restrict__ pos, float* __restrict__ X, long m,
+                                                    bool live, int tok, int D, half_t* __restrict__ A, const float* __restrict__ srow_base,
+                                                    float* __restrict__ part, int tiles_p, float* __restrict__ cen, float (*red)[5][16], int wv, int nw,
+                                                    bool act, bool poison, int a, int q) {
+  pe_half4v xh, xl;
+#pragma unroll
+  for (int i = 0; i < 4; ++i) {
+    xh[i] = (half_t)xa[i];
+    xl[i] = (half_t)(xa[i] - (float)xh[i]);
+  }
+  f32x4 val[8][2];
+  float sx = 0.f;
+  const float* prow = pos + (long)tok * D + 256 * wv + 8 * q;
+  float* xrow = X + m * D + 256 * wv + 8 * q;
+  const bool wr = live && act;
+#pragma unroll
+  for (int pr = 0; pr < 8; ++pr)
+#pragma unroll
+    for (int e = 0; e < 2; ++e) {
+      f32x4_t acc = {0.f, 0.f, 0.f, 0.f};
+      acc = __builtin_amdgcn_mfma_f32_16x16x16f16(f.wh[pr][e], xh, acc, 0, 0, 0);
+      acc = __builtin_amdgcn_mfma_f32_16x16x16f16(f.wl[pr][e], xh, acc, 0, 0, 0);
+      acc = __builtin_amdgcn_mfma_f32_16x16x16f16(f.wh[pr][e], xl, acc, 0, 0, 0);
+      const f32x4 v = (f32x4){acc[0], acc[1], acc[2], acc[3]} + f.bias[pr][e] + *(const f32x4*)(prow + 32 * pr + 4 * e);
+      val[pr][e] = v;
+      if (wr) *(f32x4*)(xrow + 32 * pr + 4 * e) = v;
+      sx += (v.x + v.y) + (v.z + v.w);
+    }
+  if (!A) return;
+  sx += __shfl_xor(sx, 16, 64);
+  sx += __shfl_xor(sx, 32, 64);
+  if (q == 0 && act) red[0][wv][a] = sx;
+  __syncthreads();
+  float sum = 0.f;
+  for (int i = 0; i < nw; ++i) sum += red[0][i][a];
+  const float mean = sum / (float)D;
+  const float* srow = srow_base + 256 * wv + 8 * q;
+  half_t* arow = A + m * D + 256 * wv + 8 * q;
+  float sq = 0.f;
+#pragma unroll
+  for (int pr = 0; pr < 8; ++pr) {
+    const f32x4 d0 = val[pr][0] - mean, d1 = val[pr][1] - mean;
+    sq += (d0.x * d0.x + d0.y * d0.y) + (d0.z * d0.z + d0.w * d0.w) + (d1.x * d1.x + d1.y * d1.y) + (d1.z * d1.z + d1.w * d1.w);
+    const f32x4 o0 = d0 * (1.0f + *(const f32x4*)(srow + 32 * pr)), o1 = d1 * (1.0f + *(const f32x4*)(srow + 32 * pr + 4));
+    half8_t h = {(half_t)o0.x, (half_t)o0.y, (half_t)o0.z, (half_t)o0.w, (half_t)o1.x, (half_t)o1.y, (half_t)o1.z, (half_t)o1.w};
+    if (poison) {
+      const half_t nan_h = (half_t)__builtin_nanf("");
+      h = (half8_t){nan_h, nan_h, nan_h, nan_h, nan_h, nan_h, nan_h, nan_h};
+    }
+    if (wr) *(half8_t*)(arow + 32 * pr) = h;
+  }
+  sq += __shfl_xor(sq, 16, 64);
+  sq += __shfl_xor(sq, 32, 64);
+  if (q == 0 && act) red[1][wv][a] = sq;
+  __syncthreads();
+  if (wv == 0 && q == 0 && wr) {
+    float qs = 0.f;
+    for (int i = 0; i < nw; ++i) qs += red[1][i][a];
+    float* pp = part + m * tiles_p * 2;
+    pp[0] = sum;
+    pp[1] = qs;
+    for (int t2 = 1; t2 < tiles_p; ++t2) {
+      pp[2 * t2] = 0.f;
+      pp[2 * t2 + 1] = 0.f;
+    }
+    cen[m] = mean;
+  }
+}
 __global__ __launch_bounds__(320) void patch_embed_ln_kernel(const float* __restrict__ x, const float* __restrict__ w, const float* __restrict__ b,
                                                              const float* __restrict__ pos, float* __restrict__ X, int M, int xmod, int R, int D,
                                                              int tiles_per_block, half_t* __restrict__ A, const float* __restrict__ scale,
                                                              long mod_stride, float* __restrict__ part, int tiles_p, float* __restrict__ cen) {
-  typedef half_t half4v __attribute__((ext_vector_type(4)));
   __shared__ float red[2][5][16];
   const int lane = threadIdx.x & 63, wv = threadIdx.x >> 6, a = lane & 15, q = lane >> 4;
   const int grid = R >> 1, T = grid * grid;
-  half4v wh[8][2], wl[8][2];
-  f32x4 bias[8][2];
-#pragma unroll
-  for (int pr = 0; pr < 8; ++pr)
-#pragma unroll
-    for (int e = 0; e < 2; ++e) {
-      const int n = 256 * wv + 32 * pr + 8 * (a >> 2) + 4 * e + (a & 3);
-      const f32x4 wf = *(const f32x4*)(w + (long)n * 16 + 4 * q);
-      const float wa[4] = {wf.x, wf.y, wf.z, wf.w};
-#pragma unroll
-      for (int i = 0; i < 4; ++i) {
-        wh[pr][e][i] = (half_t)wa[i];
-        wl[pr][e][i] = (half_t)(wa[i] - (float)wh[pr][e][i]);
-      }
-      bias[pr][e] = *(const f32x4*)(b + 256 * wv + 32 * pr + 8 * q + 4 * e);
-    }
+  PeFrag f;
+  patch_embed_load_frag(f, w, b, wv, a, q);
   for (int it = 0; it < tiles_per_block; ++it) {
     const long tile = (long)blockIdx.x * tiles_per_block + it;
     if (tile * 16 >= M) break;
@@ -126,65 +200,8 @@
     const float* xp = x + (((long)n_img * 4 + q) * R + (tok / grid) * 2) * R + (tok % grid) * 2;
     const f32x2 r0 = *(const f32x2*)xp, r1 = *(const f32x2*)(xp + R);
     const float xa[4] = {r0.x, r0.y, r1.x, r1.y};
-    half4v xh, xl;
-#pragma unroll
-    for (int i = 0; i < 4; ++i) {
-      xh[i] = (half_t)xa[i];
-      xl[i] = (half_t)(xa[i] - (float)xh[i]);
-    }
-    f32x4 val[8][2];
-    float sx = 0.f;
-    const float* prow = pos + (long)tok * D + 256 * wv + 8 * q;
-    float* xrow = X + m * D + 256 * wv + 8 * q;
-    const bool live = tile * 16 + a < M;
-#pragma unroll
-    for (int pr = 0; pr < 8; ++pr)
-#pragma unroll
-      for (int e = 0; e < 2; ++e) {
-        f32x4_t acc = {0.f, 0.f, 0.f, 0.f};
-        acc = __builtin_amdgcn_mfma_f32_16x16x16f16(wh[pr][e], xh, acc, 0, 0, 0);
-        acc = __builtin_amdgcn_mfma_f32_16x16x16f16(wl[pr][e], xh, acc, 0, 0, 0);
-        acc = __builtin_amdgcn_mfma_f32_16x16x16f16(wh[pr][e], xl, acc, 0, 0, 0);
-        const f32x4 v = (f32x4){acc[0], acc[1], acc[2], acc[3]} + bias[pr][e] + *(const f32x4*)(prow + 32 * pr + 4 * e);
-        val[pr][e] = v;
-        if (live) *(f32x4*)(xrow + 32 * pr + 4 * e) = v;
-        sx += (v.x + v.y) + (v.z + v.w);
-      }
-    if (!A) continue;
-    sx += __shfl_xor(sx, 16, 64);
-    sx += __shfl_xor(sx, 32, 64);
-    if (q == 0) red[0][wv][a] = sx;
-    __syncthreads();
-    float sum = 0.f;
-    for (int i = 0; i < (int)(blockDim.x >> 6); ++i) sum += red[0][i][a];
-    const float mean = sum / (float)D;
-    const float* srow = scale + (m / T) * mod_stride + 256 * wv + 8 * q;
-    half_t* arow = A + m * D + 256 * wv + 8 * q;
-    float sq = 0.f;
-#pragma unroll
-    for (int pr = 0; pr < 8; ++pr) {
-      const f32x4 d0 = val[pr][0] - mean, d1 = val[pr][1] - mean;
-      sq += (d0.x * d0.x + d0.y * d0.y) + (d0.z * d0.z + d0.w * d0.w) + (d1.x * d1.x + d1.y * d1.y) + (d1.z * d1.z + d1.w * d1.w);
-      const f32x4 o0 = d0 * (1.0f + *(const f32x4*)(srow + 32 * pr)), o1 = d1 * (1.0f + *(const f32x4*)(srow + 32 * pr + 4));
-      const half8_t h = {(half_t)o0.x, (half_t)o0.y, (half_t)o0.z, (half_t)o0.w, (half_t)o1.x, (half_t)o1.y, (half_t)o1.z, (half_t)o1.w};
-      if (live) *(half8_t*)(arow + 32 * pr) = h;
-    }
-    sq += __shfl_xor(sq, 16, 64);
-    sq += __shfl_xor(sq, 32, 64);
-    if (q == 0) red[1][wv][a] = sq;
-    __syncthreads();
-    if (wv == 0 && q == 0 && live) {
-      float qs = 0.f;
-      for (int i = 0; i < (int)(blockDim.x >> 6); ++i) qs += red[1][i][a];
-      float* pp = part + m * tiles_p * 2;
-      pp[0] = sum;
-      pp[1] = qs;
-      for (int t2 = 1; t2 < tiles_p; ++t2) {
-        pp[2 * t2] = 0.f;
-        pp[2 * t2 + 1] = 0.f;
-      }
-      cen[m] = mean;
-    }
+    patch_embed_ln_tile(f, xa, pos, X, m, tile * 16 + a < M, tok, D, A, scale + (m / T) * mod_stride, part, tiles_p, cen, red, wv, (int)(blockDim.x >> 6), true,
+                        false, a, q);
   }
 }
 
@@ -540,14 +557,10 @@
 }
 
 template <bool CFG, int NT>
-__global__ __launch_bounds__(256) void final_layer_mfma_kernel(const float* __restrict__ X, int M, int D, int tokens, const float* __restrict__ shift,
-                                                               const float* __restrict__ scale, long mod_stride, const float* __restrict__ Wf,
-                                                               const float* __restrict__ bf, int C, int R, int p, float cfg_scale, float* out,
-                                                               const float* base, const float* __restrict__ dt_ptr) {
-  __shared__ float st_s[4][16][3];
-  __shared__ float acc_s[4][NT][64][4];
+__device__ __forceinline__ void final_mfma_tile(const float* __restrict__ X, int M, int D, int tokens, const float* __restrict__ shift,
+                                                const float* __restrict__ scale, long mod_stride, const float* __restrict__ Wf, long tile,
+                                                float (*st_s)[16][3], float (*acc_s)[NT][64][4]) {
   const int lane = threadIdx.x & 63, wv = threadIdx.x >> 6, a = lane & 15, q = lane >> 4;
-  const long tile = blockIdx.x;
   const int Mh = CFG ? M / 2 : M;
   const long m = CFG ? tile * 8 + (a & 7) + (a >> 3) * (long)Mh : tile * 16 + a;
   const float* xr = X + m * D + 8 * q;
@@ -620,7 +633,12 @@
 #pragma unroll
   for (int t = 0; t < NT; ++t) *(f32x4_t*)acc_s[wv][t][lane] = acc[t];
   __syncthreads();
-  if (wv != 0) return;
+}
+template <bool CFG, int NT, class Also>
+__device__ __forceinline__ void final_mfma_out(long tile, int M, int tokens, float (*acc_s)[NT][64][4], const float* __restrict__ bf, int C, int R, int p,
+                                               float cfg_scale, float* out, const float* base, const float* __restrict__ dt_ptr, Also&& also) {
+  const int lane = threadIdx.x & 63, a = lane & 15, q = lane >> 4;
+  const int Mh = CFG ? M / 2 : M;
   const float dt = base ? *dt_ptr : 0.f;
   const int grid = R / p;
 #pragma unroll
@@ -642,9 +660,54 @@
       const long mr = CFG ? tile * 8 + (row & 7) + (row >> 3) * (long)Mh : tile * 16 + row;
       const int n = (int)(mr / tokens), tok = (int)(mr % tokens);
       const long off = (((long)n * C + c) * R + (tok / grid) * p + pp) * R + (tok % grid) * p + qq;
-      out[off] = base ? base[off] + dt * val : val;
-    }
-  }
+      const float res = base ? base[off] + dt * val : val;
+      out[off] = res;
+      also(row, o, res);
+    }
+  }
+}
+template <bool CFG, int NT>
+__global__ __launch_bounds__(256) void final_layer_mfma_kernel(const float* __restrict__ X, int M, int D, int tokens, const float* __restrict__ shift,
+                                                               const float* __restrict__ scale, long mod_stride, const float* __restrict__ Wf,
+                                                               const float* __restrict__ bf, int C, int R, int p, float cfg_scale, float* out,
+                                                               const float* base, const float* __restrict__ dt_ptr) {
+  __shared__ float st_s[4][16][3];
+  __shared__ float acc_s[4][NT][64][4];
+  final_mfma_tile<CFG, NT>(X, M, D, tokens, shift, scale, mod_stride, Wf, blockIdx.x, st_s, acc_s);
+  if (threadIdx.x >= 64) return;
+  final_mfma_out<CFG, NT>(blockIdx.x, M, tokens, acc_s, bf, C, R, p, cfg_scale, out, base, dt_ptr, [](int, int, float) {});
+}
+
+__global__ __launch_bounds__(256) void dit_seam_kernel(float* X, int M, int D, int tokens, const float* __restrict__ shift,
+                                                       const float* __restrict__ scale, const float* __restrict__ Wf, const float* __restrict__ bf, int R,
+                                                       float* lat, const float* __restrict__ dt_ptr, const float* __restrict__ pw,
+                                                       const float* __restrict__ pb, const float* __restrict__ pos, half_t* __restrict__ A,
+                                                       const float* __restrict__ table, long row_floats, const int* __restrict__ step, int next_offset,
+                                                       int rows, long scale_off, float* __restrict__ part, int tiles_p, float* __restrict__ cen) {
+  __shared__ float st_s[4][16][3];
+  __shared__ float acc_s[4][1][64][4];
+  __shared__ float lat_s[16][16];
+  __shared__ float red[2][5][16];
+  const int lane = threadIdx.x & 63, wv = threadIdx.x >> 6, a = lane & 15, q = lane >> 4;
+  const long tile = blockIdx.x;
+  final_mfma_tile<false, 1>(X, M, D, tokens, shift, scale, 0, Wf, tile, st_s, acc_s);
+  if (wv == 0)
+    final_mfma_out<false, 1>(tile, M, tokens, acc_s, bf, 4, R, 2, 1.0f, lat, lat, dt_ptr,
+                             [&](int row, int o, float v) { lat_s[row][4 * (o & 3) + 2 * (o >> 3) + ((o >> 2) & 1)] = v; });
+  const int nw = D >> 8;
+  const bool act = wv < nw;
+  const int wc = act ? wv : 0;
+  PeFrag f;
+  patch_embed_load_frag(f, pw, pb, wc, a, q);
+  __syncthreads();
+  const long m = tile * 16 + a;
+  const int tok = (int)(m % tokens);
+  const f32x4 l4 = *(const f32x4*)&lat_s[a][4 * q];
+  const float xa[4] = {l4.x, l4.y, l4.z, l4.w};
+  const long row = (long)*step + next_offset;
+  const bool has_row = rows <= 0 || (row >= 0 && row < rows);
+  patch_embed_ln_tile(f, xa, pos, X, m, true, tok, D, A, table + (has_row ? row : 0) * row_floats + scale_off, part, tiles_p, cen, red, wc, nw, act, !has_row, a,
+                      q);
 }
 
 __global__ __launch_bounds__(256) void cond_row_copy_kernel(const float* __restrict__ table, long row_floats, const int* __restrict__ step, int offset,
diff --git a/lfm_amd/hip.py b/lfm_amd/hip.py
--- a/lfm_amd/hip.py
+++ b/lfm_amd/hip.py
@@ -30,6 +30,13 @@
                 ("cfg", C.c_int), ("cfg_scale", C.c_float), ("out", C.c_void_p), ("axpy_base", C.c_void_p), ("axpy_dt", C.c_void_p),
                 ("cond_table", C.c_void_p), ("cond_step", C.c_void_p), ("cond_offset", C.c_int),
                 ("cond_rows", C.c_int), ("fold_ln", C.c_int), ("gemm_select", C.c_int)]
+
+
+class DitChain(C.Structure):
+    _fields_ = [("flags", C.c_int)]
+
+
+CHAIN_EMBEDDED, CHAIN_SEAM, CHAIN_EMBED_ONLY = 1, 2, 4
 
 
 class VaeResnet(C.Structure):
@@ -80,6 +87,8 @@
     L.lfm_dit_workspace_layout.argtypes = [C.POINTER(DitShape), C.c_int, C.POINTER(C.c_size_t), C.c_int]
     L.lfm_dit_forward.restype = C.c_int
     L.lfm_dit_forward.argtypes = [C.POINTER(DitShape), C.POINTER(DitWeights), C.c_void_p, C.c_size_t, C.POINTER(DitCall), C.c_void_p]
+    L.lfm_dit_forward_chained.restype = C.c_int
+    L.lfm_dit_forward_chained.argtypes = [C.POINTER(DitShape), C.POINTER(DitWeights), C.c_void_p, C.c_size_t, C.POINTER(DitCall), C.POINTER(DitChain), C.c_void_p]
     L.lfm_gemm_f16.restype = C.c_int
     L.lfm_gemm_f16.argtypes = [C.c_void_p, C.c_long, C.c_void_p, C.c_long, C.c_void_p, C.c_long, C.c_int, C.c_int, C.c_int,
                                C.c_void_p, C.c_int, C.c_void_p, C.c_long, C.c_int, C.c_void_p]
@@ -380,12 +389,13 @@
     return 2.0 * float(ticks.max()) / (ms * 1e3)
 
 
-PLAN_FOLDED_LN, PLAN_FUSED_QKV_ATTENTION = 1, 2
-
-
-def dit_plan(shape, batch, t_len=1, labels=False, fold_ln=0, gemm_select=0):
+PLAN_FOLDED_LN, PLAN_FUSED_QKV_ATTENTION, PLAN_CHAINED = 1, 2, 4
+
+
+def dit_plan(shape, batch, t_len=1, labels=False, fold_ln=0, gemm_select=0, cfg=False, cond_table=False, euler_update=False):
     call = DitCall()
     call.batch, call.t_len, call.y = int(batch), int(t_len), (1 if labels else None)
+    call.cfg, call.cond_table, call.axpy_base = (1 if cfg else 0), (1 if cond_table else None), (1 if euler_update else None)
     call.fold_ln, call.gemm_select = fold_ln, gemm_select
     plan = C.c_int(-1)
     check(lib().lfm_dit_plan(C.byref(shape), C.byref(call), C.byref(plan)), "lfm_dit_plan")
diff --git a/lfm_amd/models/DiT.py b/lfm_amd/models/DiT.py
--- a/lfm_amd/models/DiT.py
+++ b/lfm_amd/models/DiT.py
@@ -199,7 +199,7 @@
         return table
 
     @torch.no_grad()
-    def _run(self, t, x, y, cfg, cfg_scale, out=None, axpy_base=None, axpy_dt=None, cond=None, fold_ln=0, gemm_select=0):
+    def _run(self, t, x, y, cfg, cfg_scale, out=None, axpy_base=None, axpy_dt=None, cond=None, fold_ln=0, gemm_select=0, chain=0):
         hip.require_gpu(x, "DiT.forward")
         if self.training:
             raise hip.LfmHipError("the HIP DiT is inference-only: call .eval() (label dropout / autograd are training features)")
@@ -229,6 +229,11 @@
                            int(cond[2]) if cond is not None else 0,
                            int(cond[3]) if cond is not None and len(cond) > 3 else 0,
                            int(fold_ln), int(gemm_select))
+        if chain:
+            ch = hip.DitChain(int(chain))
+            rc = hip.lib().lfm_dit_forward_chained(C.byref(shape), C.byref(w), hip.ptr(ws), ws.numel(), C.byref(call), C.byref(ch), hip.stream_ptr(x.device))
+            hip.check(rc, "lfm_dit_forward_chained")
+            return out
         rc = hip.lib().lfm_dit_forward(C.byref(shape), C.byref(w), hip.ptr(ws), ws.numel(), C.byref(call), hip.stream_ptr(x.device))
         hip.check(rc, "lfm_dit_forward")
         return out
diff --git a/lfm_amd/solvers.py b/lfm_amd/solvers.py
--- a/lfm_amd/solvers.py
+++ b/lfm_amd/solvers.py
@@ -340,7 +340,7 @@
 
 class GraphedFixedGrid:
 
-    def __init__(self, model, batch, y=None, cfg_scale=1.0, use_cfg=False, graph=True, resolution=None):
+    def __init__(self, model, batch, y=None, cfg_scale=1.0, use_cfg=False, graph=True, resolution=None, chain=None):
         from .models.DiT import DiT
         from .models.EDM import DhariwalUNet
 
@@ -372,6 +372,7 @@
         self.graphs = {}
         self._graph_gen = -1
         self.use_cond_table = self.is_dit and self.y is None and not self.use_cfg and os.environ.get("LFM_COND_TABLE", "1") != "0"
+        self.use_chain = (os.environ.get("LFM_DIT_CHAIN", "1") != "0") if chain is None else bool(chain)
         self.cond_buf = None
         self._cond_rows = 0
         self._cond_key = None
@@ -437,10 +438,18 @@
             return out
         return v
 
-    def _euler(self):
+    def _chain_active(self):
+        if not (self.use_chain and self.is_dit and self._cond_active()):
+            return False
+        return bool(hip.dit_plan(self.model.shape_struct(), self.batch, cond_table=True, euler_update=True) & hip.PLAN_CHAINED)
+
+    _EULER_CHAIN = {"euler": 0, "euler_first": hip.CHAIN_SEAM, "euler_mid": hip.CHAIN_EMBEDDED | hip.CHAIN_SEAM, "euler_last": hip.CHAIN_EMBEDDED}
+
+    def _euler(self, chain=0):
         self._advance()
         if self.is_dit:
-            self.model._run(self.tcur, self.x, self.y, self.use_cfg, self.cfg_scale, out=self.x, axpy_base=self.x, axpy_dt=self.dt, cond=self._cond(-1))
+            self.model._run(self.tcur, self.x, self.y, self.use_cfg, self.cfg_scale, out=self.x, axpy_base=self.x, axpy_dt=self.dt, cond=self._cond(-1),
+                            chain=chain)
         else:
             hip.lincomb(self.x, self.x, [self._velocity(self.tcur, self.x)], self.c1, self.dt)
 
@@ -452,7 +461,7 @@
         hip.lincomb(self.x, self.x, [d1, d2], self.c2, self.dt)
 
     def _get(self, kind):
-        fn = self._euler if kind == "euler" else self._heun
+        fn = self._heun if kind == "heun" else (lambda c=self._EULER_CHAIN[kind]: self._euler(c))
         if not self.use_graph:
             return fn
         if self._graph_gen != getattr(self.model, "_gen", 0):
@@ -476,22 +485,23 @@
         return self.graphs[kind].replay
 
     @torch.no_grad()
-    def run(self, x0, heun_limit=0):
+    def run(self, x0, heun_limit=0, on_interval=None):
         assert self.n_intervals > 0, "set_grid first"
         n = self.n_intervals
         self._refresh_cond()
         self.x.copy_(x0)
         self.step.zero_()
         n_heun = max(0, min(n, heun_limit - 1)) if heun_limit else 0
-        self.last_plan = {"heun": n_heun, "euler": n - n_heun, "nfe": 2 * n_heun + (n - n_heun)}
-        if n_heun:
-            h = self._get("heun")
-            for _ in range(n_heun):
-                h()
-        if n - n_heun:
-            e = self._get("euler")
-            for _ in range(n - n_heun):
-                e()
+        n_euler = n - n_heun
+        chained = n_euler >= 2 and self._chain_active()
+        self.last_plan = {"heun": n_heun, "euler": n_euler, "nfe": 2 * n_heun + n_euler}
+        self.last_chained = chained
+        kinds = ["heun"] * n_heun + (["euler_first"] + ["euler_mid"] * (n_euler - 2) + ["euler_last"] if chained else ["euler"] * n_euler)
+        fns = {k: self._get(k) for k in dict.fromkeys(kinds)}
+        for i, k in enumerate(kinds):
+            fns[k]()
+            if on_interval is not None:
+                on_interval(i, k)
         return self.x
 
 
```

Result: slower. 117.8 images/sec (-3.6%).
